# microcosmAI/MuJoCo-RL-Environment-Wrapper

Measured on NVIDIA B200. Metric: agent-steps/sec, higher is better.
Workload: dtype f32

## Files before the change

include/mjb.h:

```cpp
#ifndef MJB_H_
#define MJB_H_

#include <stdint.h>

#include "mjb_blob.h"

#ifdef __cplusplus
extern "C" {
#endif

#define MJB_OK 0
#define MJB_ERR_PARSE -1
#define MJB_ERR_ARG -2
#define MJB_ERR_CUDA -3
#define MJB_ERR_LIMIT -4

typedef struct mjb_model mjb_model;
typedef struct mjb_batch mjb_batch;

typedef struct mjb_dims {
  int32_t nq, nv, nu, nbody, njnt, ngeom, nsite, nsensor, nsensordata, npair;
  int32_t integrator;
  int32_t ncam;
  double timestep;
} mjb_dims;

int mjb_model_create(const char* mjcf_text, mjb_model** out);
void mjb_model_destroy(mjb_model* m);
int mjb_model_dims(const mjb_model* m, mjb_dims* out);
const void* mjb_model_blob(const mjb_model* m, int64_t* nbytes);
int mjb_name2id(const mjb_model* m, int objtype, const char* name);
const char* mjb_id2name(const mjb_model* m, int objtype, int id);
const char* mjb_last_error(void);
const char* mjb_version(void);
typedef struct mjb_param_offsets {
  int32_t body_mass, body_inertia, geom_friction, actuator_gear, dof_damping;
  int32_t n_params;
} mjb_param_offsets;
int mjb_param_layout(const mjb_model* m, mjb_param_offsets* out);
int mjb_model_set_field(mjb_model* m, const char* name, const double* values, int32_t count);

enum {
  MJB_DYN_LANGUAGE = 1,
  MJB_DYN_PICKUP = 2
};
enum {
  MJB_REW_TAG_DISTANCE = 1,
  MJB_REW_ANT = 2
};
enum { MJB_DONE_DISTANCE_LE = 1  };

#define MJB_MAX_AGENTS 8
#define MJB_MAX_PLUGINS 4
#define MJB_MAX_TARGETS 16
#define MJB_MAX_EXTRA_PROBES 48

typedef struct mjb_plugin {
  int32_t kind;
  int32_t act_lo;
  int32_t act_hi;
  int32_t n_obs;
  float param[4];
} mjb_plugin;

typedef struct mjb_env_spec {
  int32_t n_agents;
  int32_t free_joint;
  int32_t skip_frames;
  int32_t max_steps;
  int32_t n_phys_act;
  int32_t act_dim;
  int32_t obs_dim[MJB_MAX_AGENTS];
  int32_t agent_body[MJB_MAX_AGENTS];
  const int32_t* act_index;
  const int32_t* obs_index;
  int32_t obs_adr[MJB_MAX_AGENTS + 1];
  int32_t n_dynamics, n_rewards, n_dones;
  mjb_plugin dynamics[MJB_MAX_PLUGINS];
  mjb_plugin rewards[MJB_MAX_PLUGINS];
  mjb_plugin dones[MJB_MAX_PLUGINS];
  int32_t n_targets;
  int32_t target_objtype[MJB_MAX_TARGETS];
  int32_t target_objid[MJB_MAX_TARGETS];
  uint64_t seed;
  int32_t solver_iterations;
  int32_t ls_iterations;
  int32_t flags;
  float reset_noise;
  int32_t n_extra_probes;
  int32_t extra_objtype[MJB_MAX_EXTRA_PROBES];
  int32_t extra_objid[MJB_MAX_EXTRA_PROBES];
  float act_low[64], act_high[64];
  float* final_obs;
  const float* start_qpos;
  const float* start_qvel;
  int32_t n_start;
  float* params;
  float param_lo[4], param_hi[4];
} mjb_env_spec;

enum {
  MJB_SPEC_NO_PACK = 1,
  MJB_SPEC_AUTORESET = 2,
  MJB_SPEC_RANDOMIZE = 4
};


typedef struct mjb_layout {
  int32_t num_envs;
  int32_t qpos_stride, qvel_stride, ctrl_stride, sensor_stride;
  int32_t act_stride;
  int32_t obs_stride;
  int32_t probe_count;
  int32_t maxcon;
  int32_t store_i32, store_f32;
} mjb_layout;

typedef struct mjb_buffers {
  float* qpos;
  float* qvel;
  float* ctrl;
  float* warmstart;
  float* sensordata;
  float* probe;
  float* actions;
  float* obs;
  float* reward;
  uint8_t* term;
  uint8_t* trunc;
  int32_t* timestep;
  int32_t* store_i;
  float* store_f;
  int32_t* ncon;
  int32_t* contact_geom;
  float* contact_dist;
  int32_t* niter;
  int32_t* nreset;
  float* probe_quat;
  int32_t* ncon_dropped;
} mjb_buffers;

enum { MJB_STORE_I_UTTERANCE = 0, MJB_STORE_I_HAS_UTTERANCE = 1, MJB_STORE_I_TARGET = 2, MJB_STORE_I_INVENTORY = 3,
       MJB_STORE_I_HAS_XPOS = 4, MJB_STORE_I_DRAWS = 5, MJB_STORE_I_COUNT = 8 };
enum { MJB_STORE_F_DISTANCE = 0, MJB_STORE_F_XPOS_BEFORE = 1, MJB_STORE_F_DISTANCE64 = 2, MJB_STORE_F_COUNT = 4 };

int mjb_batch_layout(const mjb_model* m, const mjb_env_spec* spec, int32_t num_envs, mjb_layout* out);
int mjb_batch_create(const mjb_model* m, const mjb_env_spec* spec, int32_t num_envs, int32_t device, void* stream,
                     const mjb_buffers* buffers, mjb_batch** out);
void mjb_batch_destroy(mjb_batch* b);
int mjb_reset(mjb_batch* b, const uint8_t* mask_dev);
int mjb_reset_rows(mjb_batch* b, const uint8_t* mask_dev);
int mjb_step(mjb_batch* b);
int mjb_physics(mjb_batch* b, int32_t skip_frames);
int mjb_forward(mjb_batch* b);
int mjb_sync(mjb_batch* b);
int mjb_step_host(mjb_batch* b, const float* actions, float* obs, float* reward, uint8_t* term, uint8_t* trunc);
int64_t mjb_launch_count(const mjb_batch* b);
int mjb_set_timing(mjb_batch* b, int32_t enable);
int mjb_kernel_time_ms(mjb_batch* b, double* total_ms, int64_t* launches);
int mjb_set_env_subset(mjb_batch* b, const int32_t* env_ids_dev, int32_t count);
int mjb_render(mjb_batch* b, const int32_t* cam_ids, int32_t ncams, int32_t width, int32_t height, uint8_t* rgb_dev);
int mjb_batch_geometry(const mjb_batch* b, int32_t* grid, int32_t* warps_per_cta, int64_t* smem_bytes);
int mjb_phase_cycles(uint64_t* out, int32_t n);
uint32_t mjb_draw_u32(uint64_t seed, uint32_t env, uint32_t agent, uint32_t counter);
float mjb_reset_action(uint64_t seed, uint32_t env, uint32_t agent, uint32_t dim, uint32_t ep, float low, float high);
uint32_t mjb_start_index(uint64_t seed, uint32_t env, uint32_t ep, int32_t n_start);
float mjb_param_scale(uint64_t seed, uint32_t env, int32_t family, uint32_t index, uint32_t ep, float lo, float hi);

#ifdef __cplusplus
}
#endif
#endif
```

include/mjb_blob.h:

```cpp
#ifndef MJB_BLOB_H_
#define MJB_BLOB_H_

#include <stdint.h>
#include <string.h>

#ifdef __cplusplus
extern "C" {
#endif

#define MJB_BLOB_MAGIC "MJBLOB1"
#define MJB_FIELD_NAME_LEN 32

enum { MJB_DTYPE_I32 = 0, MJB_DTYPE_F64 = 1 };

typedef struct mjb_blob_header {
  char magic[8];
  int32_t nfields;
  int32_t reserved;
  int64_t total_bytes;
} mjb_blob_header;

typedef struct mjb_blob_field {
  char name[MJB_FIELD_NAME_LEN];
  int32_t dtype;
  int32_t count;
  int64_t offset;
} mjb_blob_field;

enum { MJB_GEOM_PLANE = 0, MJB_GEOM_SPHERE = 2, MJB_GEOM_CAPSULE = 3, MJB_GEOM_BOX = 6 };
enum { MJB_JNT_FREE = 0, MJB_JNT_SLIDE = 2, MJB_JNT_HINGE = 3 };
enum { MJB_SENS_TOUCH = 0, MJB_SENS_ACCELEROMETER = 1, MJB_SENS_VELOCIMETER = 2, MJB_SENS_GYRO = 3,
       MJB_SENS_RANGEFINDER = 7, MJB_SENS_JOINTPOS = 9, MJB_SENS_JOINTVEL = 10, MJB_SENS_FRAMEPOS = 26,
       MJB_SENS_FRAMEQUAT = 27, MJB_SENS_FRAMEXAXIS = 28, MJB_SENS_FRAMEYAXIS = 29, MJB_SENS_FRAMEZAXIS = 30,
       MJB_SENS_FRAMELINVEL = 31, MJB_SENS_FRAMEANGVEL = 32 };
enum { MJB_DATA_REAL = 0, MJB_DATA_POSITIVE = 1, MJB_DATA_AXIS = 2, MJB_DATA_QUATERNION = 3 };
enum { MJB_OBJ_BODY = 1, MJB_OBJ_XBODY = 2, MJB_OBJ_JOINT = 3, MJB_OBJ_GEOM = 5, MJB_OBJ_SITE = 6, MJB_OBJ_CAMERA = 7,
       MJB_OBJ_ACTUATOR = 19, MJB_OBJ_SENSOR = 20 };
enum { MJB_INT_EULER = 0, MJB_INT_RK4 = 1 };

static inline const mjb_blob_field* mjb_blob_find(const void* blob, const char* name) {
  const mjb_blob_header* h = (const mjb_blob_header*)blob;
  const mjb_blob_field* f = (const mjb_blob_field*)((const char*)blob + sizeof(mjb_blob_header));
  for (int i = 0; i < h->nfields; i++)
    if (strncmp(f[i].name, name, MJB_FIELD_NAME_LEN) == 0) return &f[i];
  return 0;
}
static inline const int32_t* mjb_blob_i32(const void* blob, const char* name, int* count) {
  const mjb_blob_field* f = mjb_blob_find(blob, name);
  if (!f || f->dtype != MJB_DTYPE_I32) { if (count) *count = -1; return 0; }
  if (count) *count = f->count;
  return (const int32_t*)((const char*)blob + f->offset);
}
static inline const double* mjb_blob_f64(const void* blob, const char* name, int* count) {
  const mjb_blob_field* f = mjb_blob_find(blob, name);
  if (!f || f->dtype != MJB_DTYPE_F64) { if (count) *count = -1; return 0; }
  if (count) *count = f->count;
  return (const double*)((const char*)blob + f->offset);
}

#ifdef __cplusplus
}
#endif
#endif
```

mujoco_rl_environment_wrapper_b200/_lib.py:

```python
import ctypes
import os
import struct

import numpy as np

_HERE = os.path.dirname(os.path.abspath(__file__))
LIB_PATH = os.environ.get("MJB_LIB") or os.path.join(_HERE, "libmjb.so")

MAX_AGENTS, MAX_PLUGINS, MAX_TARGETS, MAX_EXTRA_PROBES = 8, 4, 16, 48
SPEC_NO_PACK, SPEC_AUTORESET, SPEC_RANDOMIZE = 1, 2, 4
PARAM_FIELDS = ("body_mass", "body_inertia", "geom_friction", "actuator_gear", "dof_damping")
PARAM_FAMILIES = ("body_mass", "geom_friction", "actuator_gear", "dof_damping")
OBJ_BODY, OBJ_XBODY, OBJ_JOINT, OBJ_GEOM, OBJ_SITE, OBJ_CAMERA, OBJ_ACTUATOR, OBJ_SENSOR = 1, 2, 3, 5, 6, 7, 19, 20
SENSOR_TYPE = {"touch": 0, "accelerometer": 1, "velocimeter": 2, "gyro": 3, "rangefinder": 7, "jointpos": 9, "jointvel": 10,
               "framepos": 26, "framequat": 27, "framexaxis": 28, "frameyaxis": 29, "framezaxis": 30, "framelinvel": 31,
               "frameangvel": 32}
DATA_REAL, DATA_POSITIVE, DATA_AXIS, DATA_QUATERNION = 0, 1, 2, 3
DYN_LANGUAGE, DYN_PICKUP = 1, 2
REW_TAG_DISTANCE, REW_ANT = 1, 2
DONE_DISTANCE_LE = 1
STORE_I = {"utterance": 0, "has_utterance": 1, "current_target": 2, "inventory": 3, "has_xpos": 4, "draws": 5}
STORE_I_COUNT = 8
STORE_F = {"distance": 0, "xpos_before": 1}
STORE_F_COUNT = 4
JNT_FREE, JNT_SLIDE, JNT_HINGE = 0, 2, 3


class Dims(ctypes.Structure):
    _fields_ = [(n, ctypes.c_int32) for n in
                ("nq", "nv", "nu", "nbody", "njnt", "ngeom", "nsite", "nsensor", "nsensordata", "npair",
                 "integrator", "ncam")] + [("timestep", ctypes.c_double)]


class Plugin(ctypes.Structure):
    _fields_ = [("kind", ctypes.c_int32), ("act_lo", ctypes.c_int32), ("act_hi", ctypes.c_int32),
                ("n_obs", ctypes.c_int32), ("param", ctypes.c_float * 4)]


class EnvSpec(ctypes.Structure):
    _fields_ = [
        ("n_agents", ctypes.c_int32), ("free_joint", ctypes.c_int32), ("skip_frames", ctypes.c_int32),
        ("max_steps", ctypes.c_int32), ("n_phys_act", ctypes.c_int32), ("act_dim", ctypes.c_int32),
        ("obs_dim", ctypes.c_int32 * MAX_AGENTS), ("agent_body", ctypes.c_int32 * MAX_AGENTS),
        ("act_index", ctypes.POINTER(ctypes.c_int32)), ("obs_index", ctypes.POINTER(ctypes.c_int32)),
        ("obs_adr", ctypes.c_int32 * (MAX_AGENTS + 1)),
        ("n_dynamics", ctypes.c_int32), ("n_rewards", ctypes.c_int32), ("n_dones", ctypes.c_int32),
        ("dynamics", Plugin * MAX_PLUGINS), ("rewards", Plugin * MAX_PLUGINS), ("dones", Plugin * MAX_PLUGINS),
        ("n_targets", ctypes.c_int32),
        ("target_objtype", ctypes.c_int32 * MAX_TARGETS), ("target_objid", ctypes.c_int32 * MAX_TARGETS),
        ("seed", ctypes.c_uint64),
        ("solver_iterations", ctypes.c_int32), ("ls_iterations", ctypes.c_int32), ("flags", ctypes.c_int32), ("reset_noise", ctypes.c_float),
        ("n_extra_probes", ctypes.c_int32), ("extra_objtype", ctypes.c_int32 * MAX_EXTRA_PROBES), ("extra_objid", ctypes.c_int32 * MAX_EXTRA_PROBES),
        ("act_low", ctypes.c_float * 64), ("act_high", ctypes.c_float * 64), ("final_obs", ctypes.c_void_p),
        ("start_qpos", ctypes.c_void_p), ("start_qvel", ctypes.c_void_p), ("n_start", ctypes.c_int32),
        ("params", ctypes.c_void_p), ("param_lo", ctypes.c_float * 4), ("param_hi", ctypes.c_float * 4),
    ]


class ParamOffsets(ctypes.Structure):
    _fields_ = [(n, ctypes.c_int32) for n in PARAM_FIELDS + ("n_params",)]


class Layout(ctypes.Structure):
    _fields_ = [(n, ctypes.c_int32) for n in
                ("num_envs", "qpos_stride", "qvel_stride", "ctrl_stride", "sensor_stride", "act_stride",
                 "obs_stride", "probe_count", "maxcon", "store_i32", "store_f32")]


class Buffers(ctypes.Structure):
    _fields_ = [(n, ctypes.c_void_p) for n in
                ("qpos", "qvel", "ctrl", "warmstart", "sensordata", "probe", "actions", "obs", "reward", "term",
                 "trunc", "timestep", "store_i", "store_f", "ncon", "contact_geom", "contact_dist", "niter", "nreset", "probe_quat", "ncon_dropped")]


_LIB = None


def load(build_if_missing=True):
    global _LIB
    if _LIB is not None:
        return _LIB
    if build_if_missing and not os.environ.get("MJB_LIB"):
        from . import build as _build
        try:
            if _build.needs_build():
                _build.build()
        except Exception:
            if not os.path.exists(LIB_PATH):
                raise
    if not os.path.exists(LIB_PATH):
        raise RuntimeError(f"{LIB_PATH} is missing: run `python -m mujoco_rl_environment_wrapper_b200.build` "
                           "(there is no CPU fallback for the step path)")
    lib = ctypes.CDLL(LIB_PATH)
    vp, i32, i64 = ctypes.c_void_p, ctypes.c_int32, ctypes.c_int64
    lib.mjb_last_error.restype = ctypes.c_char_p
    lib.mjb_version.restype = ctypes.c_char_p
    lib.mjb_model_create.argtypes = [ctypes.c_char_p, ctypes.POINTER(vp)]
    lib.mjb_model_destroy.argtypes = [vp]
    lib.mjb_model_destroy.restype = None
    lib.mjb_model_dims.argtypes = [vp, ctypes.POINTER(Dims)]
    lib.mjb_model_blob.restype = vp
    lib.mjb_model_blob.argtypes = [vp, ctypes.POINTER(i64)]
    lib.mjb_name2id.argtypes = [vp, ctypes.c_int, ctypes.c_char_p]
    lib.mjb_id2name.restype = ctypes.c_char_p
    lib.mjb_id2name.argtypes = [vp, ctypes.c_int, ctypes.c_int]
    lib.mjb_batch_layout.argtypes = [vp, ctypes.POINTER(EnvSpec), i32, ctypes.POINTER(Layout)]
    lib.mjb_batch_create.argtypes = [vp, ctypes.POINTER(EnvSpec), i32, i32, vp, ctypes.POINTER(Buffers),
                                     ctypes.POINTER(vp)]
    lib.mjb_batch_destroy.argtypes = [vp]
    lib.mjb_batch_destroy.restype = None
    lib.mjb_reset.argtypes = [vp, vp]
    lib.mjb_reset_rows.argtypes = [vp, vp]
    lib.mjb_step.argtypes = [vp]
    lib.mjb_physics.argtypes = [vp, i32]
    lib.mjb_forward.argtypes = [vp]
    lib.mjb_sync.argtypes = [vp]
    lib.mjb_step_host.argtypes = [vp, vp, vp, vp, vp, vp]
    lib.mjb_launch_count.restype = i64
    lib.mjb_launch_count.argtypes = [vp]
    lib.mjb_set_timing.argtypes = [vp, i32]
    lib.mjb_kernel_time_ms.argtypes = [vp, ctypes.POINTER(ctypes.c_double), ctypes.POINTER(i64)]
    lib.mjb_set_env_subset.argtypes = [vp, vp, ctypes.c_int32]
    lib.mjb_render.argtypes = [vp, ctypes.POINTER(ctypes.c_int32), ctypes.c_int32, ctypes.c_int32, ctypes.c_int32, vp]
    lib.mjb_batch_geometry.argtypes = [vp, ctypes.POINTER(i32), ctypes.POINTER(i32), ctypes.POINTER(i64)]
    lib.mjb_phase_cycles.argtypes = [ctypes.POINTER(ctypes.c_uint64), i32]
    lib.mjb_draw_u32.restype = ctypes.c_uint32
    lib.mjb_draw_u32.argtypes = [ctypes.c_uint64, ctypes.c_uint32, ctypes.c_uint32, ctypes.c_uint32]
    lib.mjb_reset_action.restype = ctypes.c_float
    lib.mjb_reset_action.argtypes = [ctypes.c_uint64, ctypes.c_uint32, ctypes.c_uint32, ctypes.c_uint32, ctypes.c_uint32,
                                     ctypes.c_float, ctypes.c_float]
    lib.mjb_start_index.restype = ctypes.c_uint32
    lib.mjb_start_index.argtypes = [ctypes.c_uint64, ctypes.c_uint32, ctypes.c_uint32, ctypes.c_int32]
    lib.mjb_param_layout.argtypes = [vp, ctypes.POINTER(ParamOffsets)]
    lib.mjb_model_set_field.argtypes = [vp, ctypes.c_char_p, ctypes.POINTER(ctypes.c_double), i32]
    lib.mjb_param_scale.restype = ctypes.c_float
    lib.mjb_param_scale.argtypes = [ctypes.c_uint64, ctypes.c_uint32, ctypes.c_int32, ctypes.c_uint32, ctypes.c_uint32,
                                    ctypes.c_float, ctypes.c_float]
    _LIB = lib
    return lib


def check(rc, what=""):
    if rc != 0:
        msg = load().mjb_last_error().decode(errors="replace")
        raise Exception(f"{what}: {msg}" if what else msg)


def parse_blob(raw: bytes):
    magic, nf, _, _tot = struct.unpack_from("8siiq", raw, 0)
    if not magic.startswith(b"MJBLOB1"):
        raise ValueError("bad model blob")
    out = {}
    for i in range(nf):
        name, dt, cnt, off = struct.unpack_from("32siiq", raw, 24 + i * 48)
        name = name.split(b"\0")[0].decode()
        out[name] = np.frombuffer(raw, dtype=np.int32 if dt == 0 else np.float64, count=cnt, offset=off).copy()
    return out


class Model:

    def __init__(self, xml_text: str):
        self._lib = load()
        h = ctypes.c_void_p()
        check(self._lib.mjb_model_create(xml_text.encode(), ctypes.byref(h)), "MJCF compile")
        self._h = h
        d = Dims()
        check(self._lib.mjb_model_dims(h, ctypes.byref(d)))
        self.dims = d
        self._read_blob()
        for k in ("nq", "nv", "nu", "nbody", "njnt", "ngeom", "nsite", "nsensor", "nsensordata", "npair", "ncam"):
            setattr(self, k, getattr(d, k))
        self.timestep = d.timestep

    def _read_blob(self):
        n = ctypes.c_int64()
        p = self._lib.mjb_model_blob(self._h, ctypes.byref(n))
        self.blob = bytes((ctypes.c_char * n.value).from_address(p))
        self.fields = parse_blob(self.blob)

    def set_field(self, name, values):
        v = np.ascontiguousarray(np.asarray(values, dtype=np.float64).reshape(-1))
        check(self._lib.mjb_model_set_field(self._h, name.encode(), v.ctypes.data_as(ctypes.POINTER(ctypes.c_double)), v.size),
              "set_field")
        self._read_blob()

    def param_layout(self):
        out = ParamOffsets()
        check(self._lib.mjb_param_layout(self._h, ctypes.byref(out)), "param layout")
        return out

    def nominal_params(self):
        lay, f = self.param_layout(), self.fields
        row = np.zeros(lay.n_params, np.float32)
        vals = {"body_mass": f["body_mass"], "body_inertia": f["body_inertia"], "geom_friction": f["geom_friction"][0::3],
                "actuator_gear": f["actuator_gear"], "dof_damping": f["dof_damping"]}
        for k, v in vals.items():
            o = getattr(lay, k)
            row[o:o + v.size] = v
        return row

    @classmethod
    def from_xml_path(cls, path):
        with open(path, "r") as f:
            return cls(f.read())

    def __del__(self):
        try:
            if getattr(self, "_h", None):
                self._lib.mjb_model_destroy(self._h)
                self._h = None
        except Exception:
            pass

    def name2id(self, objtype, name):
        return self._lib.mjb_name2id(self._h, objtype, name.encode())

    def id2name(self, objtype, idx):
        r = self._lib.mjb_id2name(self._h, objtype, idx)
        return None if r is None else r.decode()
```

mujoco_rl_environment_wrapper_b200/batch.py:

```python
import ctypes

import numpy as np
import torch

from . import _lib as L


class Batch:
    def __init__(self, model: "L.Model", spec: "L.EnvSpec", num_envs: int, device=None, keepalive=(), share=None, probe_quat=False,
                 start_states=None, params=False, param_ranges=None):
        self._lib = L.load()
        if not torch.cuda.is_available():
            raise RuntimeError("mujoco_rl_environment_wrapper_b200: no CUDA device — the step path is CUDA-only "
                               "(sm_100a); there is no CPU fallback")
        self.model, self.spec, self.num_envs = model, spec, int(num_envs)
        self._keep = keepalive
        self.device = torch.device("cuda", torch.cuda.current_device()) if device is None else torch.device(device)
        lay = L.Layout()
        L.check(self._lib.mjb_batch_layout(model._h, ctypes.byref(spec), self.num_envs, ctypes.byref(lay)), "batch layout")
        self.layout = lay
        if share is not None:
            same = all(getattr(lay, f) == getattr(share.layout, f) for f, _ in L.Layout._fields_)
            if not same or share.num_envs != self.num_envs or share.device != self.device:
                raise Exception("level variants must share one buffer layout (same sizes, sensors, agents and plugins)")
# ... 60 lines not shown
            if getattr(self, "_h", None):
                self._lib.mjb_batch_destroy(self._h)
                self._h = None
        except Exception:
            pass

    def __getattr__(self, k):
        buf = self.__dict__.get("buf")
        if buf is not None and k in buf:
            return buf[k]
        raise AttributeError(k)

    def _mask_ptr(self, mask):
        if mask is None:
            return None
        self._mask = mask.to(device=self.device, dtype=torch.uint8).contiguous()
        return ctypes.c_void_p(self._mask.data_ptr())

    def reset(self, mask=None):
        L.check(self._lib.mjb_reset(self._h, self._mask_ptr(mask)), "reset")

    def reset_rows(self, mask=None):
        L.check(self._lib.mjb_reset_rows(self._h, self._mask_ptr(mask)), "reset_rows")

    def step(self):
        L.check(self._lib.mjb_step(self._h), "step")

    def set_subset(self, env_ids=None):
        if env_ids is None:
            self._subset = None
            L.check(self._lib.mjb_set_env_subset(self._h, None, 0), "env subset")
            return
        ids = env_ids.to(device=self.device, dtype=torch.int32).contiguous()
        count = int(ids.numel())
        if count == 0:
            ids = torch.zeros(1, dtype=torch.int32, device=self.device)
        self._subset = ids
        L.check(self._lib.mjb_set_env_subset(self._h, ctypes.c_void_p(self._subset.data_ptr()), count), "env subset")

    def render(self, cam_ids, width=64, height=64, out=None):
        n = len(cam_ids)
        if out is None:
            out = torch.empty((self.num_envs, n, height, width, 3), dtype=torch.uint8, device=self.device)
        ids = (ctypes.c_int32 * n)(*cam_ids)
        L.check(self._lib.mjb_render(self._h, ids, n, int(width), int(height), ctypes.c_void_p(out.data_ptr())), "render")
        return out

    def physics(self, skip_frames=1):
        L.check(self._lib.mjb_physics(self._h, skip_frames), "physics")

    def forward(self):
        L.check(self._lib.mjb_forward(self._h), "forward")

    def sync(self):
        L.check(self._lib.mjb_sync(self._h), "sync")

    def step_host(self, actions: np.ndarray, obs: np.ndarray, reward: np.ndarray, term: np.ndarray, trunc: np.ndarray):
        L.check(self._lib.mjb_step_host(self._h, actions.ctypes.data, obs.ctypes.data, reward.ctypes.data,
                                        term.ctypes.data, trunc.ctypes.data), "step_host")

    def host_arrays(self, pinned=True):
        lay, A, N = self.layout, self.spec.n_agents, self.num_envs
        z = lambda shape, dt: torch.zeros(shape, dtype=dt, pin_memory=pinned)
        f32, u8 = torch.float32, torch.uint8
        self._host_keep = [z((N, A, lay.act_stride), f32), z((N, A, lay.obs_stride), f32), z((N, A), f32),
                           z((N, A + 1), u8), z((N, A + 1), u8)]
        return tuple(t.numpy() for t in self._host_keep)

    @property
    def launch_count(self):
        return int(self._lib.mjb_launch_count(self._h))

    def set_timing(self, enable=True):
        L.check(self._lib.mjb_set_timing(self._h, 1 if enable else 0))

    def kernel_time_ms(self):
        t, n = ctypes.c_double(), ctypes.c_int64()
        L.check(self._lib.mjb_kernel_time_ms(self._h, ctypes.byref(t), ctypes.byref(n)))
        return t.value, n.value

    def geometry(self):
        g, w, s = ctypes.c_int32(), ctypes.c_int32(), ctypes.c_int64()
        self._lib.mjb_batch_geometry(self._h, ctypes.byref(g), ctypes.byref(w), ctypes.byref(s))
        return {"grid": g.value, "warps_per_cta": w.value, "smem_bytes": s.value}
```

mujoco_rl_environment_wrapper_b200/build.py:

```python
import os
import subprocess
import sys

_HERE = os.path.dirname(os.path.abspath(__file__))
CSRC = os.path.join(_HERE, "csrc")
LIB_PATH = os.path.join(_HERE, "libmjb.so")
SOURCES = ["mjcf_compile.cpp", "mjb_model.cpp", "mjb_batch.cu"]
NVCC_FLAGS = [
    "-gencode", "arch=compute_100a,code=sm_100a", "-lineinfo", "-O3", "-std=c++17",
    "--use_fast_math",
    "-Xcompiler", "-fPIC", "-Xcompiler", "-Wall", "-shared",
]


def _nvcc():
    for cand in (os.environ.get("NVCC"), "/usr/local/cuda/bin/nvcc", "nvcc"):
        if cand and (os.path.isabs(cand) and os.path.exists(cand) or not os.path.isabs(cand)):
            return cand
    raise RuntimeError("nvcc not found")


def _deps():
    out = []
    for root in (CSRC, os.path.join(_HERE, "..", "include")):
        for f in os.listdir(root):
            if f.endswith((".h", ".cuh", ".cu", ".cpp")):
                out.append(os.path.join(root, f))
    return out


def needs_build():
    if not os.path.exists(LIB_PATH):
        return True
    t = os.path.getmtime(LIB_PATH)
    return any(os.path.getmtime(f) > t for f in _deps())


def build(force=False, verbose=False):
    if not force and not needs_build():
        return LIB_PATH
    cmd = [_nvcc()] + NVCC_FLAGS + os.environ.get("MJB_NVCC_FLAGS", "").split() + (["-Xptxas", "-v"] if verbose else []) + ["-o", LIB_PATH] + \
          [os.path.join(CSRC, s) for s in SOURCES]
    res = subprocess.run(cmd, capture_output=True, text=True)
    if verbose or res.returncode != 0:
        sys.stderr.write(res.stdout + res.stderr)
    if res.returncode != 0:
        raise RuntimeError("nvcc failed building libmjb.so")
    return LIB_PATH


if __name__ == "__main__":
    build(force="--force" in sys.argv, verbose="-v" in sys.argv)
    print(LIB_PATH)
```

mujoco_rl_environment_wrapper_b200/csrc/dev_model.h:

```cpp
#pragma once
#include <stdint.h>

#ifndef MJB_HD
#if defined(__CUDACC__)
#define MJB_HD __host__ __device__ __forceinline__
#else
#define MJB_HD inline
#endif
#endif

namespace mjb {

#define MJB_IMAGE_FIELDS(X)                                                                         \
  X(level_adr)       \
  X(mb_parent)       \
  X(mb_root)         \
  X(mb_jntadr)       \
  X(mb_jntnum)       \
  X(mb_dofadr)       \
  X(mb_dofnum)       \
  X(mb_childadr)     \
  X(mb_child)        \
  X(mb_dofmask)      \
  X(mb_pos)          \
  X(mb_quat)         \
  X(mb_ipos)         \
  X(mb_iquat)        \
  X(mb_mass)         \
  X(mb_inertia)      \
  X(mb_invweight)    \
  X(jnt_type)        \
  X(jnt_qposadr)     \
  X(jnt_dofadr)      \
  X(jnt_pos)         \
  X(jnt_axis)        \
  X(jnt_qpos0)       \
  X(lim_dof)         \
  X(lim_qposadr)     \
  X(lim_param)       \
  X(dof_mb)          \
  X(dof_parent)      \
  X(dof_kind)        \
  X(dof_t0)          \
  X(dof_t1)          \
  X(dof_lim)         \
  X(dof_armature)    \
  X(dof_damping)     \
  X(geom_type)       \
  X(geom_mb)         \
  X(geom_slot)       \
  X(geom_size)       \
  X(geom_rbound)     \
  X(geom_pos)        \
  X(geom_mat)        \
  X(geom_quat)       \
  X(geom_ray)        \
  X(pair_pack)       \
  X(pclass)          \
  X(bp_block)        \
  X(bp_passmask)     \
  X(site_mb)         \
  X(site_type)       \
  X(site_pos)        \
  X(site_quat)       \
  X(site_size)       \
  X(sensor_type)     \
  X(sensor_site)     \
  X(sensor_adr)      \
  X(sensor_dim)      \
  X(sensor_dtype)    \
  X(sensor_cutoff)   \
  X(act_dof)         \
  X(act_param)       \
  X(dof_actadr)      \
  X(dof_actnum)      \
  X(act_list)        \
  X(probe_kind)      \
  X(probe_id)        \
  X(probe_const)     \
  X(act_index)       \
  X(obs_index)       \
  X(tri_lut)         \
  X(qpos0)

enum ImageField {
#define X(n) IF_##n,
  MJB_IMAGE_FIELDS(X)
#undef X
      IF_COUNT
};

#define MJB_SMEM_FIELDS(X)                                                                          \
  X(qpos) X(qvel) X(qacc) X(ctrl) X(qfrc)  \
  X(xpos) X(xquat) X(xmat) X(xipos)        \
  X(cdof) X(cinert) X(crb) X(cvel) X(cacc)  \
  X(gpos) X(gmat) X(spos) X(smat)          \
  X(M) X(H)                                \
  X(cand)                                  \
  X(con)                                   \
  X(J)                                     \
  X(efcD) X(efcAref) X(efcJar) X(efcJv)    \
  X(vecA) X(vecB) X(vecC) X(vecD)          \
  X(rk)                                    \
  X(sens)

enum SmemField {
#define X(n) SF_##n,
  MJB_SMEM_FIELDS(X)
#undef X
      SF_COUNT
};

struct DevPlugin {
  int kind, act_lo, act_hi, n_obs;
  float param[4];
};

struct DevModel {
  int nq, nv, nu, nmb, njnt, nlim, ngeom, ngdyn, nsite, nsensor, nsensordata, npair, nclass, nlevel, nprobe;
  int maxcon, maxcand, maxefc, ldj, maxtree, nblock;
  int pack, a1, t1, nq1, nv1, nu1, ns1, np1, ngeom1, maxcon1;
  int integrator, has_damping, need_acc_sensors;
  float timestep, gravity[3];
  double timestep_d;
  int solver_iterations, ls_iterations;
  float solver_tol;
  float reset_noise;
  int njnt1;
  int n_agents, free_joint, skip_frames, max_steps, n_phys_act, act_dim;
  int obs_dim[8], obs_adr[9], agent_probe[8];
  int n_dynamics, n_rewards, n_dones, n_targets;
  DevPlugin dynamics[4], rewards[4], dones[4];
  int target_probe[16];
  unsigned long long seed;
  int off[IF_COUNT];
  int image_words;
  int soff[SF_COUNT];
  int env_words;
  int qpos_stride, qvel_stride, ctrl_stride, sensor_stride, act_stride, obs_stride, store_i32, store_f32;
  float* final_obs;
  int autoreset;
  float dyn_act_low[4], dyn_act_high[4];
  const float* start_qpos;
  const float* start_qvel;
  int n_start;
  int start_pad[3];
  float* params;
  int n_params, prm_n;
  int randomize, prm_soff, off_prm_map, off_prm_nominal;
  float prm_lo[4], prm_hi[4];
  int ext_sensors, off_sens_obj, ext_pad[2];
};
enum { SO_MB = 0, SO_POS = 1, SO_QUAT = 4, SO_STRIDE = 8 };
enum { KSENS_OBJ_AXIS = 64 };
MJB_HD int prm_inertia(const DevModel& dm) { return dm.nmb; }
MJB_HD int prm_damping(const DevModel& dm) { return 4 * dm.nmb; }
MJB_HD int prm_gear(const DevModel& dm) { return 4 * dm.nmb + dm.nv; }
MJB_HD int prm_friction(const DevModel& dm) { return 4 * dm.nmb + dm.nv + dm.nu; }

enum { CAM_MB = 0, CAM_MODE = 1, CAM_POS = 2, CAM_QUAT = 5, CAM_TANHALF = 9, CAM_STRIDE = 12 };
struct RenderHdr {
  int ncam, ngeom;
  int off_cam, off_rgba;
  int words;
};
enum { GL_POS = 0, GL_MAT = 3, GL_SIZE = 12, GL_TYPE = 15, GL_RBOUND = 16, GL_RGB = 17, GL_STRIDE = 20 };

enum { CON_DIST = 0, CON_POS = 1, CON_FRAME = 4, CON_PAIR = 13, CON_MU = 14, CON_MASK = 15, CON_DOFS = 16, CON_STRIDE = 20 };
enum { LIM_LO = 0, LIM_HI, LIM_MARGIN, LIM_K, LIM_B, LIM_INVW, LIM_SOLIMP, LIM_STRIDE = 12 };
enum { PC_MARGIN = 0, PC_INCMARGIN, PC_MU, PC_K, PC_B, PC_SOLIMP, PC_CONDIM = 10, PC_STRIDE = 12 };
enum { DOF_AXIS = 0, DOF_FREE_TRANS = 1, DOF_FREE_ROT = 2 };
enum { PROBE_BODY = 0, PROBE_GEOM = 1, PROBE_CONST = 2 };
enum { BP_ROOT_A = 0, BP_PARTNER = 1, BP_REACH = 2, BP_MARGIN = 3, BP_STRIDE = 4, BP_ALWAYS = 0x7fffffff };

}
```

mujoco_rl_environment_wrapper_b200/csrc/env_kernel.cuh:

```cuda
#pragma once
#include "step_kernel.cuh"
#if defined(MJB_HOST_EMU)
#define MJB_IMG_WAIT(c) ((void)0)
#else
#include "tma_prims.cuh"
#define MJB_IMG_WAIT(c) do { if ((c).img_bar) mbar_wait((c).img_bar, 0); } while (0)
#endif

namespace mjb {

enum { MODE_STEP = 0, MODE_PHYSICS = 1, MODE_FORWARD = 2, MODE_RESET = 3, MODE_RESET_ROWS = 4 };

#if defined(MJB_HOST_EMU)
#define MJB_AGENT_LOOP
#else
#define MJB_AGENT_LOOP _Pragma("unroll (AMAX <= 2 ? 2 : 1)")
#endif

MJB_HD uint32_t draw_u32(unsigned long long seed, uint32_t env, uint32_t agent, uint32_t counter) {
  unsigned long long z = seed + 0x9E3779B97F4A7C15ull * (1ull + env) + 0xBF58476D1CE4E5B9ull * agent +
                         0x94D049BB133111EBull * counter;
  z = (z ^ (z >> 30)) * 0xBF58476D1CE4E5B9ull;
  z = (z ^ (z >> 27)) * 0x94D049BB133111EBull;
  z ^= z >> 31;
  return (uint32_t)(z >> 32);
}

MJB_HD float reset_action(unsigned long long seed, uint32_t env, uint32_t agent, uint32_t dim, uint32_t ep, float low, float high) {
  const float u = (float)(draw_u32(seed ^ 0x5eedc0deULL, env, 0xC000u + agent * 64u + dim, ep) >> 8) * (1.f / 16777216.f);
#if defined(__CUDA_ARCH__)
  return __fadd_rn(low, __fmul_rn(u, high - low));
#else
  volatile float span = u * (high - low);
  return low + span;
#endif
}

MJB_HD uint32_t start_index(unsigned long long seed, uint32_t env, uint32_t ep, int n_start) {
  return n_start < 1 ? 0u : (uint32_t)(((unsigned long long)draw_u32(seed ^ 0x5eedc0deULL, env, 0xD000u, ep) * (uint32_t)n_start) >> 32);
}

MJB_HD float param_scale(unsigned long long seed, uint32_t env, uint32_t family, uint32_t index, uint32_t ep, float lo, float hi) {
  const float u = (float)(draw_u32(seed ^ 0x5eedc0deULL, env, 0x10000u + 0x1000u * family + index, ep) >> 8) * (1.f / 16777216.f);
#if defined(__CUDA_ARCH__)
  return __fadd_rn(lo, __fmul_rn(u, hi - lo));
#else
  volatile float span = u * (hi - lo);
  return lo + span;
#endif
}

MJB_DEV double probe_dist(const float* probe, int a, int b) {
  const double dx = (double)probe[4 * a] - (double)probe[4 * b], dy = (double)probe[4 * a + 1] - (double)probe[4 * b + 1],
               dz = (double)probe[4 * a + 2] - (double)probe[4 * b + 2];
#if defined(MJB_HOST_EMU)
  volatile double xx = dx * dx, yy = dy * dy, zz = dz * dz;
  return sqrt((xx + yy) + zz);
#else
  return sqrt(__dadd_rn(__dadd_rn(__dmul_rn(dx, dx), __dmul_rn(dy, dy)), __dmul_rn(dz, dz)));
#endif
}
MJB_DEV double ld_dist(const float* sfa) {
  union { double d; float f[2]; } u;
  u.f[0] = sfa[MJB_STORE_F_DISTANCE64]; u.f[1] = sfa[MJB_STORE_F_DISTANCE64 + 1];
  return u.d;
}
MJB_DEV void st_dist(float* sfa, double d) {
  union { double d; float f[2]; } u;
  u.d = d;
  sfa[MJB_STORE_F_DISTANCE64] = u.f[0]; sfa[MJB_STORE_F_DISTANCE64 + 1] = u.f[1];
  sfa[MJB_STORE_F_DISTANCE] = (float)d;
}

template <int AMAX>
MJB_DEV bool run_plugins(const DevModel& dm, const float* ctrl, float* obs, float* rew, uint8_t* term, uint8_t* trunc, int env, int copy,
                         bool is_reset, const float* probe, int* si, float* sf, const float* act, int* ts_io, const double* dtab = nullptr,
                         bool keep_flags = false) {
  const int A = dm.a1, ab = copy * dm.a1, tb = copy * dm.t1, n_targets = dm.t1;
  auto pdist = [&](int a, int t) { return dtab ? dtab[a * n_targets + t] : probe_dist(probe, dm.agent_probe[ab + a], dm.target_probe[tb + t]); };
  double reward[AMAX];
  bool done[AMAX];
  int opos[AMAX];
  if (is_reset)
    MJB_AGENT_LOOP
    for (int a = 0; a < AMAX; a++) if (a < A) {
      MJB_NOUNROLL
      for (int k = 0; k < dm.store_i32; k++) if (k != MJB_STORE_I_DRAWS) si[a * dm.store_i32 + k] = 0;
      MJB_NOUNROLL
      for (int k = 0; k < dm.store_f32; k++) sf[a * dm.store_f32 + k] = 0.f;
    }
  MJB_AGENT_LOOP
  for (int a = 0; a < AMAX; a++) if (a < A) { reward[a] = 0.0; done[a] = false; opos[a] = dm.obs_adr[ab + a + 1] - dm.obs_adr[ab + a]; }
  MJB_NOUNROLL
  for (int p = 0; p < dm.n_dynamics; p++) {
    const DevPlugin& dyn = dm.dynamics[p];
    MJB_AGENT_LOOP
    for (int a = 0; a < AMAX; a++) if (a < A) {
      int* sia = si + a * dm.store_i32;
      float* sfa = sf + a * dm.store_f32;
      float* oa = obs + a * dm.obs_stride;
      if (dyn.kind == MJB_DYN_LANGUAGE) {
        int utt = (int)act[a * dm.act_stride + dyn.act_lo];
        sia[MJB_STORE_I_UTTERANCE] = utt; sia[MJB_STORE_I_HAS_UTTERANCE] = 1;
        int other = a == 0 ? 1 : 0;
        float val = 0.f;
        if (other < A && si[other * dm.store_i32 + MJB_STORE_I_HAS_UTTERANCE]) val = (float)si[other * dm.store_i32 + MJB_STORE_I_UTTERANCE];
        oa[opos[a]++] = val;
      } else if (dyn.kind == MJB_DYN_PICKUP) {
        int tgt = sia[MJB_STORE_I_TARGET];
        if (tgt == 0 && n_targets > 0) {
          tgt = 1 + (int)(draw_u32(dm.seed, env, a, sia[MJB_STORE_I_DRAWS]++) % (uint32_t)n_targets);
          sia[MJB_STORE_I_TARGET] = tgt;
        }
        if (tgt > 0) {
          const double d = pdist(a, tgt - 1);
          if (d < (double)dyn.param[0]) {
            sia[MJB_STORE_I_INVENTORY] ^= 1;
            reward[a] += 1.0;
            tgt = 1 + (int)(draw_u32(dm.seed, env, a, sia[MJB_STORE_I_DRAWS]++) % (uint32_t)n_targets);
            sia[MJB_STORE_I_TARGET] = tgt;
            st_dist(sfa, pdist(a, tgt - 1));
          }
          const float* tp = probe + 4 * dm.target_probe[tb + tgt - 1];
          oa[opos[a]] = tp[0]; oa[opos[a] + 1] = tp[1]; oa[opos[a] + 2] = tp[2];
        } else {
          oa[opos[a]] = 0.f; oa[opos[a] + 1] = 0.f; oa[opos[a] + 2] = 0.f;
        }
        oa[opos[a] + 3] = (float)sia[MJB_STORE_I_INVENTORY];
        opos[a] += 4;
      }
    }
  }
  if (is_reset) {
    MJB_AGENT_LOOP
    for (int a = 0; a < AMAX; a++) if (a < A) {
      MJB_NOUNROLL
      for (int k = 0; k < dm.store_i32; k++) if (k != MJB_STORE_I_DRAWS) si[a * dm.store_i32 + k] = 0;
      MJB_NOUNROLL
      for (int k = 0; k < dm.store_f32; k++) sf[a * dm.store_f32 + k] = 0.f;
      if (!keep_flags) { rew[a] = 0.f; term[a] = 0; trunc[a] = 0; }
    }
    if (!keep_flags) { term[A] = 0; trunc[A] = 0; }
    *ts_io = 0;
    return false;
  }
  MJB_NOUNROLL
  for (int p = 0; p < dm.n_rewards; p++) {
    const DevPlugin& rf = dm.rewards[p];
    MJB_AGENT_LOOP
    for (int a = 0; a < AMAX; a++) if (a < A) {
      int* sia = si + a * dm.store_i32;
      float* sfa = sf + a * dm.store_f32;
      if (rf.kind == MJB_REW_TAG_DISTANCE) {
        int tgt = sia[MJB_STORE_I_TARGET];
        if (n_targets <= 0) continue;
        if (tgt == 0) {
          tgt = 1 + (int)(draw_u32(dm.seed, env, a, sia[MJB_STORE_I_DRAWS]++) % (uint32_t)n_targets);
          sia[MJB_STORE_I_TARGET] = tgt;
          st_dist(sfa, pdist(a, tgt - 1));
        } else {
          const double d = pdist(a, tgt - 1);
          reward[a] += (ld_dist(sfa) - d) * (double)rf.param[0];
          st_dist(sfa, d);
        }
      } else if (rf.kind == MJB_REW_ANT) {
        float x_after = probe[4 * dm.agent_probe[ab + a]];
        if (!sia[MJB_STORE_I_HAS_XPOS]) {
          sia[MJB_STORE_I_HAS_XPOS] = 1;
        } else {
          double cc = 0.0;
          MJB_NOUNROLL
          for (int u = 0; u < dm.nu1; u++) cc += (double)ctrl[u] * (double)ctrl[u];
          reward[a] += ((double)x_after - (double)sfa[MJB_STORE_F_XPOS_BEFORE]) / dm.timestep_d - 0.5 * cc;
        }
        sfa[MJB_STORE_F_XPOS_BEFORE] = x_after;
      }
    }
  }
  int ts = *ts_io;
  uint8_t tr = ts >= dm.max_steps ? 1 : 0;
  MJB_NOUNROLL
  for (int a = 0; a <= A; a++) trunc[a] = tr;
  bool all = false;
  MJB_NOUNROLL
  for (int p = 0; p < dm.n_dones && !all; p++) {
    const DevPlugin& df = dm.dones[p];
    MJB_AGENT_LOOP
    for (int a = 0; a < AMAX; a++) if (a < A)
      if (df.kind == MJB_DONE_DISTANCE_LE) done[a] = done[a] || (ld_dist(sf + a * dm.store_f32) <= (double)df.param[0]);
    MJB_AGENT_LOOP
    for (int a = 0; a < AMAX; a++) if (a < A) all = all || done[a];
  }
  MJB_AGENT_LOOP
  for (int a = 0; a < AMAX; a++) if (a < A) { rew[a] = (float)reward[a]; term[a] = done[a] ? 1 : 0; }
  term[A] = all ? 1 : 0;
  *ts_io = ts + 1;
  return all || tr;
}

MJB_DEV void split_copy(int i, int n1, int K, int& k, int& j) {
  if (K == 1) { k = 0; j = i; }
  else { k = i / n1; j = i - k * n1; }
}

template <bool PHYS, bool PACKED, bool EXT = true, bool PRM = false>
MJB_DEV void run_env(const Ctx& c_in, const mjb_buffers& B, int venv, int num_envs, int mode_in, int skip_frames,
                     const uint8_t* reset_mask) {
  uint32_t fin = 0;
pass:
  const bool auto_pass = fin != 0;
  const bool own_rows = EXT && mode_in == MODE_RESET_ROWS;
  const int mode = (auto_pass || own_rows) ? (int)MODE_RESET : mode_in;
  Ctx c = c_in;
  float* probe = c.probe;
  const DevModel& dm = *c.dm;
  const int lane = c.lane, K = PACKED ? dm.pack : 1, e0 = venv * K;
  c.probe_quat = (!PACKED && B.probe_quat) ? B.probe_quat + (size_t)e0 * dm.np1 * 4 : nullptr;
  uint32_t live = 0, upd = 0;
  for (int k = 0; k < K; k++)
    if (e0 + k < num_envs) {
      live |= 1u << k;
      if (!(mode == MODE_RESET && reset_mask && !reset_mask[e0 + k])) upd |= 1u << k;
    }
  if (auto_pass) {
    upd = fin;
    c.cta_threads = 0;
  }
  if (!upd) return;
  if (mode == MODE_RESET || live != (K >= 32 ? 0xffffffffu : (1u << K) - 1u)) MJB_IMG_WAIT(c);
  float *qpos = SF(qpos), *qvel = SF(qvel), *qacc = SF(qacc), *ctrl = SF(ctrl), *sens = SF(sens);
  auto fresh = [&](int k) { return mode == MODE_RESET && ((upd >> k) & 1u); };
  auto has = [&](int k) { return ((live >> k) & 1u) != 0; };
  auto reset_key = [&](uint32_t env) {
    return (uint32_t)B.timestep[env] ^ MJB_F2U(B.qpos[(size_t)env * dm.qpos_stride]) ^ (MJB_F2U(B.qvel[(size_t)env * dm.qvel_stride]) << 13);
  };
  const bool pool = EXT && mode == MODE_RESET && !own_rows && dm.n_start > 0, from_start = own_rows || pool;
  uint32_t pr[MJB_MAX_PACK] = {0, 0, 0, 0};
  if (pool) {
#pragma unroll
    for (int k = 0; k < MJB_MAX_PACK; k++)
      if (k < K && fresh(k)) pr[k] = start_index(dm.seed, (uint32_t)(e0 + k), reset_key((uint32_t)(e0 + k)), dm.n_start);
  }
  auto pool_row = [&](const float* base, int n1, int k) {
    return base + (size_t)(K == 1 || k == 0 ? pr[0] : k == 1 ? pr[1] : k == 2 ? pr[2] : pr[3]) * n1;
  };
  MJB_NOUNROLL
  for (int i = lane; i < dm.nq; i += 32) {
    int k, j;
    split_copy(i, dm.nq1, K, k, j);
    if (from_start && fresh(k)) MJB_G2S(&qpos[i], pool ? pool_row(dm.start_qpos, dm.nq1, k) + j : &B.qpos[(size_t)(e0 + k) * dm.qpos_stride + j]);
    else if (fresh(k) || !has(k)) qpos[i] = CF(qpos0)[i];
    else MJB_G2S(&qpos[i], &B.qpos[(size_t)(e0 + k) * dm.qpos_stride + j]);
  }
  MJB_NOUNROLL
  for (int i = lane; i < dm.nv; i += 32) {
    int k, j;
    split_copy(i, dm.nv1, K, k, j);
    bool z = fresh(k) || !has(k);
    if (from_start && fresh(k)) {
      MJB_G2S(&qvel[i], pool ? pool_row(dm.start_qvel, dm.nv1, k) + j : &B.qvel[(size_t)(e0 + k) * dm.qvel_stride + j]);
      qacc[i] = 0.f;
    } else if (z) { qvel[i] = 0.f; qacc[i] = 0.f; }
    else {
      MJB_G2S(&qvel[i], &B.qvel[(size_t)(e0 + k) * dm.qvel_stride + j]);
      MJB_G2S(&qacc[i], &B.warmstart[(size_t)(e0 + k) * dm.qvel_stride + j]);
    }
  }
  MJB_NOUNROLL
  for (int i = lane; i < dm.nu; i += 32) {
    int k, j;
    split_copy(i, dm.nu1, K, k, j);
    if (fresh(k) || !has(k)) ctrl[i] = 0.f;
    else MJB_G2S(&ctrl[i], &B.ctrl[(size_t)(e0 + k) * dm.ctrl_stride + j]);
  }
  MJB_NOUNROLL
  for (int i = lane; i < dm.nsensordata; i += 32) {
    int k, j;
    split_copy(i, dm.ns1, K, k, j);
    if (fresh(k) || !has(k)) sens[i] = 0.f;
    else MJB_G2S(&sens[i], &B.sensordata[(size_t)(e0 + k) * dm.sensor_stride + j]);
  }
  auto probe_slot = [&](int p, int& k, int& p1) {
    if (K == 1) { k = 0; p1 = p; }
    else if (p < K * dm.a1) { k = p / dm.a1; p1 = p - k * dm.a1; }
    else { int q = p - K * dm.a1; k = q / dm.t1; p1 = dm.a1 + (q - k * dm.t1); }
  };
  MJB_NOUNROLL
  for (int i = lane; i < 4 * dm.nprobe; i += 32) {
    int k, p1;
    probe_slot(i >> 2, k, p1);
    if (has(k)) MJB_G2S(&probe[i], &B.probe[((size_t)(e0 + k) * dm.np1 + p1) * 4 + (i & 3)]);
    else probe[i] = 0.f;
  }
  const bool epi = (mode == MODE_STEP || mode == MODE_RESET);
  int pre_si[2] = {0, 0}, pre_ts = 0;
  float pre_sf = 0.f, pre_act[2] = {0.f, 0.f};
  if (epi && K == 1) {
    const int* gsi = B.store_i + (size_t)e0 * dm.a1 * dm.store_i32;
// ... 200 lines not shown
    for (int i = lane; i < n; i += 32) {
      int e = CI(obs_index)[dm.obs_adr[av] + i], kind = e >> 24, adr = e & 0xffffff;
      oa[i] = kind == 0 ? sens[adr] : (kind == 1 ? qpos[adr] : qvel[adr]);
    }
  }
  MJB_PH(c, PH_EPI_OBS);
  int* s_si = (int*)SF(J);
  float* s_sf = SF(J) + MJB_MAX_AGENTS * MJB_STORE_I_COUNT;
  float* s_act = s_sf + MJB_MAX_AGENTS * MJB_STORE_F_COUNT;
  int* s_ts = (int*)(s_act + 64);
  double* s_dtab = (double*)(s_ts + 4);
  MJB_NOUNROLL
  for (int k = 0; k < K; k++) {
    if (!writes(k)) continue;
    const int env = e0 + k, A1 = dm.a1;
    int* gsi = B.store_i + (size_t)env * A1 * dm.store_i32;
    float* gsf = B.store_f + (size_t)env * A1 * dm.store_f32;
    const float* gact = B.actions + (size_t)env * A1 * dm.act_stride;
    MJB_SYNC();
    if (K == 1) {
      for (int r = 0; r < 2; r++) {
        int i = lane + 32 * r;
        if (i < A1 * dm.store_i32) s_si[i] = pre_si[r];
        if (i < A1 * dm.act_stride) s_act[i] = pre_act[r];
      }
      if (lane < A1 * dm.store_f32) s_sf[lane] = pre_sf;
      if (lane == 0) *s_ts = pre_ts;
    } else {
      for (int i = lane; i < A1 * dm.store_i32; i += 32) s_si[i] = gsi[i];
      for (int i = lane; i < A1 * dm.act_stride; i += 32) s_act[i] = gact[i];
      if (lane < A1 * dm.store_f32) s_sf[lane] = gsf[lane];
      if (lane == 0) *s_ts = B.timestep[env];
    }
    MJB_NOUNROLL
    for (int i = lane; i < A1 * dm.t1; i += 32) {
      const int a = i / dm.t1, t = i - a * dm.t1;
      s_dtab[i] = probe_dist(probe, dm.agent_probe[k * A1 + a], dm.target_probe[k * dm.t1 + t]);
    }
    MJB_SYNC();
    MJB_PH(c, PH_EPI_STAGE);
    const uint32_t ep = auto_pass ? MJB_SHFL(ep_k, k) : 0u;
    bool last_step = false;
    if (lane == 0) {
      if (auto_pass) {
        MJB_NOUNROLL
        for (int a = 0; a < A1; a++) {
          MJB_NOUNROLL
          for (int p = 0; p < dm.n_dynamics; p++) {
            const DevPlugin& dyn = dm.dynamics[p];
            if (dyn.act_hi > dyn.act_lo)
              s_act[a * dm.act_stride + dyn.act_lo] = reset_action(dm.seed, (uint32_t)env, (uint32_t)a, (uint32_t)dyn.act_lo, ep,
                                                                   dm.dyn_act_low[p], dm.dyn_act_high[p]);
          }
        }
      }
      if (MJB_LIKELY(A1 <= 2))
        last_step = run_plugins<2>(dm, SF(ctrl) + k * dm.nu1, B.obs + (size_t)env * A1 * dm.obs_stride, B.reward + (size_t)env * A1, B.term + (size_t)env * (A1 + 1),
                                   B.trunc + (size_t)env * (A1 + 1), env, k, mode == MODE_RESET, probe, s_si, s_sf, s_act, s_ts, s_dtab, auto_pass);
      else
        last_step = run_plugins<MJB_MAX_AGENTS>(dm, SF(ctrl) + k * dm.nu1, B.obs + (size_t)env * A1 * dm.obs_stride, B.reward + (size_t)env * A1,
                                                B.term + (size_t)env * (A1 + 1), B.trunc + (size_t)env * (A1 + 1), env, k, mode == MODE_RESET, probe, s_si,
                                                s_sf, s_act, s_ts, s_dtab, auto_pass);
    }
    MJB_SYNC();
    MJB_PH(c, PH_EPI_PLUG);
    for (int i = lane; i < A1 * dm.store_i32; i += 32) gsi[i] = s_si[i];
    if (lane < A1 * dm.store_f32) gsf[lane] = s_sf[lane];
    if (lane == 0) B.timestep[env] = *s_ts;
    if (EXT && PHYS && mode == MODE_STEP && dm.autoreset && MJB_SHFL((int)last_step, 0)) {
      ended |= 1u << k;
      const size_t o = (size_t)env * A1 * dm.obs_stride;
      MJB_NOUNROLL
      for (int i = lane; i < A1 * dm.obs_stride; i += 32) dm.final_obs[o + i] = B.obs[o + i];
    }
  }
  MJB_PH(c, PH_EPILOGUE);
  if (MJB_UNLIKELY(ended)) {
    MJB_SYNC();
    fin = ended;
    goto pass;
  }
}

}
```

mujoco_rl_environment_wrapper_b200/csrc/mjb_batch.cu:

```cuda
#include <cuda_runtime.h>

#include <cmath>
#include <cstdio>
#include <cstring>
#include <map>
#include <mutex>
#include <string>
#include <vector>

#include "../../include/mjb.h"
#include "dev_model_build.h"
#include "env_kernel.cuh"
#include "render_kernel.cuh"
#include "tma_prims.cuh"
#include "lite_kernel.cuh"
#include "mjb_internal.h"

#ifndef MJB_MAX_THREADS
#define MJB_MAX_THREADS 512
#endif

namespace mjb {

template <bool PHYS, bool PACKED, bool EXT = false, bool PRM = false>
__global__ void __launch_bounds__(PHYS ? MJB_MAX_THREADS : 512, PHYS ? 1 : 4) k_env(const __grid_constant__ DevModel dm, const uint32_t* __restrict__ image, const mjb_buffers B,
                      int num_envs, int mode, int skip_frames, const uint8_t* __restrict__ mask,
                      const int* __restrict__ env_ids, int active, int env_base) {
  extern __shared__ __align__(128) uint32_t smem[];
  uint64_t* bar = reinterpret_cast<uint64_t*>(smem);
  uint32_t* img = smem + 4;
  const int warps = blockDim.x >> 5, warp = threadIdx.x >> 5, lane = threadIdx.x & 31;
  if (threadIdx.x == 0) {
    mbar_init(bar, 1);
    mbar_fence_init();
  }
  __syncthreads();
  if (threadIdx.x == 0) {
    uint32_t bytes = (uint32_t)dm.image_words * 4u;
    mbar_expect_tx(bar, bytes);
    bulk_g2s(img, image, bytes, bar);
  }
  float* scratch = reinterpret_cast<float*>(img + dm.image_words) + (size_t)warp * (dm.env_words + 4 * ((dm.nprobe + 3) & ~3));
  float* probe = scratch + dm.env_words;
  Ctx c{&dm, img, scratch, lane, probe, 0};
#if defined(MJB_PHASE_PROF)
  long long t_last = clock64();
  c.t_last = &t_last;
#endif
  const int stride = gridDim.x * warps;
  const int pack = PACKED ? dm.pack : 1;
  const int nvirt = (active + pack - 1) / pack;
  const int rounds = (nvirt - blockIdx.x * warps + stride - 1) / stride;
  int env = blockIdx.x * warps + warp;
  for (int r = 0; r < rounds; r++) {
    if (PHYS) {
      int busy = nvirt - (blockIdx.x * warps + r * stride);
      c.cta_threads = (mask == nullptr ? 32 : 0) * (busy > warps ? warps : (busy < 0 ? 0 : busy));
    }
    c.img_bar = r == 0 ? bar : nullptr;
    if (env < nvirt) run_env<PHYS, PACKED, EXT, PRM>(c, B, env_ids ? env_ids[env] : env + env_base, num_envs, mode, skip_frames, mask);
    if (r == 0) mbar_wait(bar, 0);
    if (!PHYS) __syncthreads();
    MJB_PH(c, PH_BARRIER);
    env += stride;
  }
}

}

struct mjb_batch {
  mjb::PackedModel packed;
  mjb::DevImage img;
  mjb::DevImage lite;
  bool has_lite = false;
  int lite_warps = 0, lite_grid = 0;
  size_t lite_smem = 0;
  mjb::LiteLayout tile{};
  int tile_grid = 0;
  size_t tile_smem = 0;
  int* d_lite_tab = nullptr;
  mjb::DevModel* d_lite_dm = nullptr;
  mjb_buffers B;
  int num_envs = 0, device = 0, warps = 0, grid = 0;
  size_t smem_bytes = 0;
  cudaStream_t stream = nullptr;
  cudaStream_t stream2 = nullptr;
  cudaEvent_t ev_fork = nullptr, ev_join = nullptr;
  uint32_t* d_image = nullptr;
  mjb::DevImage rimg;
  uint32_t *d_rimage = nullptr, *d_rtab = nullptr;
  const int* subset = nullptr;
  int subset_count = -1;
  int64_t launches = 0;
  bool timing = false;
  std::vector<std::pair<cudaEvent_t, cudaEvent_t>> events;
  float *h_act = nullptr, *h_obs = nullptr, *h_rew = nullptr;
  uint8_t *h_term = nullptr, *h_trunc = nullptr;
  const void* pin_cache[5] = {nullptr, nullptr, nullptr, nullptr, nullptr};
};

namespace {
#define CUDA_TRY(expr)                                                                      \
  do {                                                                                      \
    cudaError_t e_ = (expr);                                                                \
    if (e_ != cudaSuccess) {                                                                \
      mjb::set_error(std::string(#expr) + ": " + cudaGetErrorString(e_));                   \
      return MJB_ERR_CUDA;                                                                  \
    }                                                                                       \
  } while (0)

int launch(mjb_batch* b, int mode, int skip_frames, const uint8_t* mask, cudaStream_t stream = nullptr, int base = 0, int count = -1,
           const mjb_buffers* out_buffers = nullptr) {
  if (b->subset && b->subset_count == 0) return MJB_OK;
  if (!stream) stream = b->stream;
  const int active = b->subset ? b->subset_count : (count >= 0 ? count : b->num_envs);
  const mjb_buffers& B = out_buffers ? *out_buffers : b->B;
  cudaEvent_t e0 = nullptr, e1 = nullptr;
  if (b->timing) {
    CUDA_TRY(cudaEventCreate(&e0));
    CUDA_TRY(cudaEventCreate(&e1));
    CUDA_TRY(cudaEventRecord(e0, stream));
  }
  if (mode == mjb::MODE_STEP && b->has_lite && !b->subset) {
    const int ntiles = (active + b->tile.tile - 1) / b->tile.tile;
    const mjb::LiteLayout& T = b->tile;
    mjb::LiteIssue I{};
    int k = 0;
    auto row = [&](const void* basep, int words, int off_words) {
      if (words <= 0) return;
      I.c[k].base = (const char*)basep; I.c[k].row_bytes = 4u * words; I.c[k].fixed = 0; I.c[k].dst_off = 4u * off_words; k++;
      I.sum_row_bytes += 4u * words;
    };
    auto fixed = [&](const void* basep, int bytes, int off_words) {
      I.c[k].base = (const char*)basep; I.c[k].row_bytes = 0; I.c[k].fixed = bytes; I.c[k].dst_off = 4u * off_words; k++;
      I.first_bytes += bytes;
    };
    row(B.qpos, T.qs, T.o_qpos); row(B.qvel, T.vs, T.o_qvel); row(B.actions, T.as, T.o_act);
    row(B.store_i, T.sis, T.o_si); row(B.store_f, T.sfs, T.o_sf);
    if (T.use_ctrl) row(B.ctrl, T.cs, T.o_ctrl);
    if (T.use_sens) row(B.sensordata, T.ss, T.o_sens);
    if (T.use_probe) row(B.probe, T.ps, T.o_probe);
    fixed(b->d_lite_tab, 4 * T.table_words, T.o_gather);
    fixed(b->d_lite_dm, T.dm_bytes, T.o_dm);
    I.ncopy = k; I.tile = T.tile; I.active = active; I.env_base = base; I.profile = T.profile;
    mjb::k_lite<<<std::min(ntiles, b->tile_grid), LITE_THREADS, b->tile_smem, stream>>>(I, B, T);
  } else if (mode == mjb::MODE_STEP && b->has_lite) {
    mjb::k_env<false, false><<<b->lite_grid, b->lite_warps * 32, b->lite_smem, stream>>>(b->lite.dm, b->d_image, B, b->num_envs, mode,
                                                                                   skip_frames, mask, b->subset, active, base);
  } else {
    const bool ext = b->img.dm.autoreset || mode == mjb::MODE_RESET_ROWS || (mode == mjb::MODE_RESET && b->img.dm.n_start > 0);
    auto kern = b->img.dm.prm_n > 0 ? (b->img.dm.pack > 1 ? mjb::k_env<true, true, true, true> : mjb::k_env<true, false, true, true>)
              : ext ? (b->img.dm.pack > 1 ? mjb::k_env<true, true, true> : mjb::k_env<true, false, true>)
                    : (b->img.dm.pack > 1 ? mjb::k_env<true, true> : mjb::k_env<true, false>);
    const int pack = b->img.dm.pack;
    const int need = ((active + pack - 1) / pack + b->warps - 1) / b->warps;
    kern<<<std::min(b->grid, std::max(1, need)), b->warps * 32, b->smem_bytes, stream>>>(
        b->img.dm, b->d_image, B, b->num_envs, mode, skip_frames, mask, b->subset, active, base / pack);
  }
  CUDA_TRY(cudaGetLastError());
  if (b->timing) {
    CUDA_TRY(cudaEventRecord(e1, stream));
    b->events.emplace_back(e0, e1);
  }
  b->launches++;
  return MJB_OK;
}
}

extern "C" {

uint32_t mjb_draw_u32(uint64_t seed, uint32_t env, uint32_t agent, uint32_t counter) {
  return mjb::draw_u32(seed, env, agent, counter);
}

float mjb_reset_action(uint64_t seed, uint32_t env, uint32_t agent, uint32_t dim, uint32_t ep, float low, float high) {
  return mjb::reset_action(seed, env, agent, dim, ep, low, high);
}

uint32_t mjb_start_index(uint64_t seed, uint32_t env, uint32_t ep, int32_t n_start) {
  return mjb::start_index(seed, env, ep, n_start);
}

float mjb_param_scale(uint64_t seed, uint32_t env, int32_t family, uint32_t index, uint32_t ep, float lo, float hi) {
  return mjb::param_scale(seed, env, (uint32_t)family, index, ep, lo, hi);
}

int mjb_batch_layout(const mjb_model* m, const mjb_env_spec* spec, int32_t num_envs, mjb_layout* out) {
  if (!m || !spec || !out || num_envs < 1) { mjb::set_error("mjb_batch_layout: bad argument"); return MJB_ERR_ARG; }
  if (const char* e = mjb::param_spec_error(*spec)) { mjb::set_error(std::string("mjb_batch_layout: ") + e); return MJB_ERR_ARG; }
  try {
    mjb::ModelView mv(m->host.blob.data());
    mjb::DevImage img;
    mjb::build_dev_model(mv, *spec, img);
    mjb::fill_layout(img.dm, num_envs, *out);
    return MJB_OK;
  } catch (const std::exception& e) {
    mjb::set_error(e.what());
    return MJB_ERR_LIMIT;
  }
}

int mjb_batch_create(const mjb_model* m, const mjb_env_spec* spec, int32_t num_envs, int32_t device, void* stream,
                     const mjb_buffers* buffers, mjb_batch** out) {
  if (!m || !spec || !buffers || !out || num_envs < 1) { mjb::set_error("mjb_batch_create: bad argument"); return MJB_ERR_ARG; }
  *out = nullptr;
  if (spec->flags & MJB_SPEC_AUTORESET) {
    if (spec->skip_frames == 0) {
      mjb::set_error("mjb_batch_create: MJB_SPEC_AUTORESET needs skip_frames >= 1 (the physics-free step has no forward pass to reset with)");
      return MJB_ERR_ARG;
    }
    if (!spec->final_obs) { mjb::set_error("mjb_batch_create: MJB_SPEC_AUTORESET needs spec.final_obs"); return MJB_ERR_ARG; }
    for (int d = 0; d < spec->act_dim && d < 64; d++)
      if (!(spec->act_low[d] <= spec->act_high[d]) || !std::isfinite(spec->act_low[d]) || !std::isfinite(spec->act_high[d])) {
        mjb::set_error("mjb_batch_create: MJB_SPEC_AUTORESET needs finite act_low <= act_high");
        return MJB_ERR_ARG;
      }
  }
  if (spec->n_start < 0) { mjb::set_error("mjb_batch_create: spec.n_start < 0"); return MJB_ERR_ARG; }
  if (spec->n_start > 0 && (!spec->start_qpos || !spec->start_qvel)) {
    mjb::set_error("mjb_batch_create: spec.n_start > 0 needs spec.start_qpos and spec.start_qvel");
    return MJB_ERR_ARG;
  }
  if (const char* e = mjb::param_spec_error(*spec)) { mjb::set_error(std::string("mjb_batch_create: ") + e); return MJB_ERR_ARG; }
  int ndev = 0;
  if (cudaGetDeviceCount(&ndev) != cudaSuccess || ndev < 1) {
    mjb::set_error("mjb_batch_create: no CUDA device (the step path has no CPU fallback)");
    return MJB_ERR_CUDA;
  }
  mjb_batch* b = new mjb_batch();
  try {
    const int K = mjb::choose_pack(m->host, *spec, num_envs);
    mjb::make_packed(m->host, *spec, K, b->packed);
    mjb::ModelView mv(K > 1 ? b->packed.rep.blob.data() : m->host.blob.data());
    mjb::build_dev_model(mv, b->packed.vspec, b->img, false, K);
    mjb::ModelView mv1(m->host.blob.data());
    if (mv1.ncam > 0) mjb::build_dev_model(mv1, *spec, b->rimg, false, 1);
  } catch (const std::exception& e) {
    mjb::set_error(e.what());
    delete b;
    return MJB_ERR_LIMIT;
  }
  b->B = *buffers;
  b->num_envs = num_envs; b->device = device; b->stream = (cudaStream_t)stream;
  const mjb::DevModel& dm = b->img.dm;
  for (const void* p : {(const void*)b->B.qpos, (const void*)b->B.qvel, (const void*)b->B.ctrl, (const void*)b->B.warmstart,
                        (const void*)b->B.sensordata, (const void*)b->B.probe, (const void*)b->B.actions, (const void*)b->B.obs,
                        (const void*)b->B.reward, (const void*)b->B.term, (const void*)b->B.trunc, (const void*)b->B.timestep,
                        (const void*)b->B.store_i, (const void*)b->B.store_f})
    if (!p) { mjb::set_error("mjb_batch_create: a required buffer is NULL"); delete b; return MJB_ERR_ARG; }
  auto fail = [&](int rc) { mjb_batch_destroy(b); return rc; };
  if (cudaSetDevice(device) != cudaSuccess) { mjb::set_error("cudaSetDevice failed"); return fail(MJB_ERR_CUDA); }
  cudaDeviceProp prop;
  if (cudaGetDeviceProperties(&prop, device) != cudaSuccess) { mjb::set_error("cudaGetDeviceProperties failed"); return fail(MJB_ERR_CUDA); }
  size_t max_smem = prop.sharedMemPerBlockOptin;
  size_t fixed = 16 + (size_t)dm.image_words * 4;
  size_t per_env = ((size_t)dm.env_words + 4 * ((dm.nprobe + 3) & ~3)) * 4;
  size_t cta_budget = std::min(max_smem, prop.sharedMemPerMultiprocessor - 1024);
  int warps = cta_budget > fixed ? (int)((cta_budget - fixed) / per_env) : 0;
  int cap = std::min(MJB_MAX_THREADS / 32, mjb::env_int("MJB_WARPS", MJB_MAX_THREADS / 32));
  if (warps > cap) warps = cap;
  if (warps < 1) { mjb::set_error("model needs more shared memory per environment than one SM has"); return fail(MJB_ERR_LIMIT); }
  int sms = prop.multiProcessorCount;
  const int nvirt = (num_envs + dm.pack - 1) / dm.pack;
  int rounds = (nvirt + sms * warps - 1) / (sms * warps);
  int even = (nvirt + sms * rounds - 1) / (sms * rounds);
  if (even < warps) warps = even < 1 ? 1 : even;
  b->warps = warps;
  b->grid = (nvirt + warps - 1) / warps;
  if (b->grid > sms) b->grid = sms;
  b->smem_bytes = fixed + per_env * warps;
  static std::mutex smem_attr_mu;
  static std::map<int, size_t> smem_attr;
  std::lock_guard<std::mutex> smem_attr_lock(smem_attr_mu);
  if (b->smem_bytes > smem_attr[device] && (cudaFuncSetAttribute(mjb::k_env<true, false>, cudaFuncAttributeMaxDynamicSharedMemorySize, (int)b->smem_bytes) != cudaSuccess ||
      cudaFuncSetAttribute(mjb::k_env<true, true>, cudaFuncAttributeMaxDynamicSharedMemorySize, (int)b->smem_bytes) != cudaSuccess ||
      cudaFuncSetAttribute(mjb::k_env<true, false, true>, cudaFuncAttributeMaxDynamicSharedMemorySize, (int)b->smem_bytes) != cudaSuccess ||
      cudaFuncSetAttribute(mjb::k_env<true, true, true>, cudaFuncAttributeMaxDynamicSharedMemorySize, (int)b->smem_bytes) != cudaSuccess ||
      cudaFuncSetAttribute(mjb::k_env<true, false, true, true>, cudaFuncAttributeMaxDynamicSharedMemorySize, (int)b->smem_bytes) != cudaSuccess ||
      cudaFuncSetAttribute(mjb::k_env<true, true, true, true>, cudaFuncAttributeMaxDynamicSharedMemorySize, (int)b->smem_bytes) != cudaSuccess)) {
    mjb::set_error(std::string("cudaFuncSetAttribute(max dynamic smem) failed: ") + cudaGetErrorString(cudaGetLastError()));
    return fail(MJB_ERR_CUDA);
  }
  smem_attr[device] = std::max(smem_attr[device], b->smem_bytes);
  if (spec->skip_frames == 0) {
    try {
      mjb::ModelView mv(m->host.blob.data());
      mjb::build_dev_model(mv, *spec, b->lite, true);
    } catch (const std::exception& e) { mjb::set_error(e.what()); return fail(MJB_ERR_LIMIT); }
    size_t lite_env = ((size_t)b->lite.dm.env_words + 4 * ((b->lite.dm.nprobe + 3) & ~3)) * 4;
    b->lite_warps = 16;
    b->lite_smem = fixed + lite_env * b->lite_warps;
    int per_sm = 1;
    if (cudaFuncSetAttribute(mjb::k_env<false, false>, cudaFuncAttributeMaxDynamicSharedMemorySize, (int)b->lite_smem) != cudaSuccess ||
        cudaOccupancyMaxActiveBlocksPerMultiprocessor(&per_sm, mjb::k_env<false, false>, b->lite_warps * 32, b->lite_smem) != cudaSuccess || per_sm < 1) {
      mjb::set_error("lite step kernel configuration failed");
      return fail(MJB_ERR_CUDA);
    }
    b->lite_grid = std::min((num_envs + b->lite_warps - 1) / b->lite_warps, prop.multiProcessorCount * per_sm);
    b->has_lite = true;
    int tile = std::max(16, mjb::env_int("MJB_LITE_TILE", 64) / 16 * 16);
    for (;;) {
      b->tile = mjb::make_lite_layout(b->lite.dm, tile);
      b->tile.profile = mjb::env_int("MJB_LITE_PROFILE", 0);
      b->tile_smem = 16 + (size_t)b->tile.words * 4;
      if (b->tile_smem <= 48 * 1024 || tile <= 16) break;
      tile /= 2;
    }
    int tile_per_sm = 1;
    if (b->tile_smem > max_smem || cudaFuncSetAttribute(mjb::k_lite, cudaFuncAttributeMaxDynamicSharedMemorySize, (int)b->tile_smem) != cudaSuccess ||
        cudaOccupancyMaxActiveBlocksPerMultiprocessor(&tile_per_sm, mjb::k_lite, LITE_THREADS, b->tile_smem) != cudaSuccess || tile_per_sm < 1) {
      mjb::set_error("tile step kernel configuration failed (rows of one env too large for shared memory)");
      return fail(MJB_ERR_CUDA);
    }
    b->tile_grid = prop.multiProcessorCount * tile_per_sm;
    {
      std::vector<int> tab = mjb::lite_tables(b->lite.dm, b->tile, b->img.words.data());
      std::vector<char> hdr(b->tile.dm_bytes, 0);
      memcpy(hdr.data(), &b->lite.dm, sizeof(mjb::DevModel));
      if (cudaMalloc(&b->d_lite_tab, tab.size() * 4) != cudaSuccess ||
          cudaMemcpy(b->d_lite_tab, tab.data(), tab.size() * 4, cudaMemcpyHostToDevice) != cudaSuccess ||
          cudaMalloc(&b->d_lite_dm, hdr.size()) != cudaSuccess ||
          cudaMemcpy(b->d_lite_dm, hdr.data(), hdr.size(), cudaMemcpyHostToDevice) != cudaSuccess) {
        mjb::set_error("tile kernel table upload failed");
        return fail(MJB_ERR_CUDA);
      }
    }
  }
  if (cudaMalloc(&b->d_image, (size_t)dm.image_words * 4) != cudaSuccess ||
      cudaMemcpy(b->d_image, b->img.words.data(), (size_t)dm.image_words * 4, cudaMemcpyHostToDevice) != cudaSuccess) {
    mjb::set_error("device image upload failed");
    return fail(MJB_ERR_CUDA);
  }
  if (cudaStreamCreateWithFlags(&b->stream2, cudaStreamNonBlocking) != cudaSuccess ||
      cudaEventCreateWithFlags(&b->ev_fork, cudaEventDisableTiming) != cudaSuccess ||
      cudaEventCreateWithFlags(&b->ev_join, cudaEventDisableTiming) != cudaSuccess) {
    mjb::set_error("mjb_batch_create: stream / event creation failed");
    return fail(MJB_ERR_CUDA);
  }
  const int A = dm.a1;
  if (cudaMallocHost(&b->h_act, sizeof(float) * (size_t)num_envs * A * dm.act_stride + 16) != cudaSuccess ||
      cudaMallocHost(&b->h_obs, sizeof(float) * (size_t)num_envs * A * dm.obs_stride + 16) != cudaSuccess ||
      cudaMallocHost(&b->h_rew, sizeof(float) * (size_t)num_envs * A + 16) != cudaSuccess ||
      cudaMallocHost(&b->h_term, (size_t)num_envs * (A + 1) + 16) != cudaSuccess ||
      cudaMallocHost(&b->h_trunc, (size_t)num_envs * (A + 1) + 16) != cudaSuccess) {
    mjb::set_error("pinned staging allocation failed");
    return fail(MJB_ERR_CUDA);
  }
  *out = b;
  return MJB_OK;
}

void mjb_batch_destroy(mjb_batch* b) {
  if (!b) return;
  for (auto& ev : b->events) { cudaEventDestroy(ev.first); cudaEventDestroy(ev.second); }
  if (b->d_image) cudaFree(b->d_image);
  if (b->stream2) cudaStreamDestroy(b->stream2);
  for (cudaEvent_t e : {b->ev_fork, b->ev_join}) if (e) cudaEventDestroy(e);
  if (b->d_rimage) cudaFree(b->d_rimage);
  if (b->d_rtab) cudaFree(b->d_rtab);
  if (b->d_lite_tab) cudaFree(b->d_lite_tab);
  if (b->d_lite_dm) cudaFree(b->d_lite_dm);
  if (b->h_act) cudaFreeHost(b->h_act);
  if (b->h_obs) cudaFreeHost(b->h_obs);
  if (b->h_rew) cudaFreeHost(b->h_rew);
  if (b->h_term) cudaFreeHost(b->h_term);
  if (b->h_trunc) cudaFreeHost(b->h_trunc);
// ... 106 lines not shown
  if (!b || !total_ms || !launches) { mjb::set_error("mjb_kernel_time_ms: null argument"); return MJB_ERR_ARG; }
  CUDA_TRY(cudaStreamSynchronize(b->stream));
  double tot = 0;
  for (auto& ev : b->events) {
    float ms = 0;
    CUDA_TRY(cudaEventElapsedTime(&ms, ev.first, ev.second));
    tot += ms;
    cudaEventDestroy(ev.first); cudaEventDestroy(ev.second);
  }
  *total_ms = tot; *launches = (int64_t)b->events.size();
  b->events.clear();
  return MJB_OK;
}

int mjb_render(mjb_batch* b, const int32_t* cam_ids, int32_t ncams, int32_t width, int32_t height, uint8_t* rgb_dev) {
  if (!b || !cam_ids || !rgb_dev) { mjb::set_error("mjb_render: null argument"); return MJB_ERR_ARG; }
  const mjb::RenderHdr& rh = b->rimg.rhdr;
  if (rh.ncam == 0) { mjb::set_error("mjb_render: the model has no <camera>"); return MJB_ERR_ARG; }
  if (ncams < 1 || ncams > RENDER_MAX_CAMS || width < 1 || height < 1 || width > 4096 || height > 4096) {
    mjb::set_error("mjb_render: 1.." + std::to_string(RENDER_MAX_CAMS) + " cameras, 1..4096 pixels per side");
    return MJB_ERR_ARG;
  }
  mjb::RenderCams cams{};
  cams.n = ncams;
  for (int k = 0; k < ncams; k++) {
    if (cam_ids[k] < 0 || cam_ids[k] >= rh.ncam) { mjb::set_error("mjb_render: camera id out of range"); return MJB_ERR_ARG; }
    if (b->rimg.render[rh.off_cam + cam_ids[k] * mjb::CAM_STRIDE + mjb::CAM_MODE] != 0) {
      mjb::set_error("mjb_render: only mode=\"fixed\" cameras can be rendered");
      return MJB_ERR_ARG;
    }
    cams.id[k] = cam_ids[k];
  }
  CUDA_TRY(cudaSetDevice(b->device));
  const mjb::DevModel& dm = b->rimg.dm;
  const size_t smem = ((size_t)dm.image_words + dm.env_words + rh.words + (size_t)dm.ngeom * mjb::GL_STRIDE + 12 * RENDER_MAX_CAMS) * 4 +
                      (size_t)RENDER_TILE_BATCH * ((dm.ngeom + 2) & ~1) * 2;
  if (!b->d_rimage) {
    CUDA_TRY(cudaMalloc(&b->d_rimage, b->rimg.words.size() * 4));
    CUDA_TRY(cudaMalloc(&b->d_rtab, b->rimg.render.size() * 4));
    CUDA_TRY(cudaMemcpy(b->d_rimage, b->rimg.words.data(), b->rimg.words.size() * 4, cudaMemcpyHostToDevice));
    CUDA_TRY(cudaMemcpy(b->d_rtab, b->rimg.render.data(), b->rimg.render.size() * 4, cudaMemcpyHostToDevice));
    CUDA_TRY(cudaFuncSetAttribute(mjb::k_render, cudaFuncAttributeMaxDynamicSharedMemorySize, (int)smem));
  }
  int sms = 148;
  cudaDeviceGetAttribute(&sms, cudaDevAttrMultiProcessorCount, b->device);
  const int per_sm = (int)std::max<size_t>(1, std::min<size_t>(8, (200 * 1024) / (smem + 1024)));
  const int grid = std::min(b->num_envs, sms * per_sm);
  mjb::k_render<<<grid, 256, smem, b->stream>>>(dm, b->d_rimage, rh, b->d_rtab, b->B.qpos, b->num_envs, cams, width, height, rgb_dev);
  CUDA_TRY(cudaGetLastError());
  b->launches++;
  return MJB_OK;
}

int mjb_set_env_subset(mjb_batch* b, const int32_t* env_ids_dev, int32_t count) {
  if (!b) { mjb::set_error("mjb_set_env_subset: null batch"); return MJB_ERR_ARG; }
  if (b->img.dm.autoreset) {
    mjb::set_error("mjb_set_env_subset: level variants cannot auto-reset (a reset draws the env's level on the host)");
    return MJB_ERR_ARG;
  }
  if (!env_ids_dev) { b->subset = nullptr; b->subset_count = -1; return MJB_OK; }
  if (count < 0 || count > b->num_envs) { mjb::set_error("mjb_set_env_subset: count out of range"); return MJB_ERR_ARG; }
  if (b->img.dm.pack != 1) {
    mjb::set_error("mjb_set_env_subset: the batch packs several envs per warp; create it with MJB_SPEC_NO_PACK");
    return MJB_ERR_ARG;
  }
  b->subset = env_ids_dev; b->subset_count = count;
  return MJB_OK;
}

int mjb_phase_cycles(uint64_t* out, int32_t n) {
#if defined(MJB_PHASE_PROF)
  unsigned long long h[32];
  if (cudaMemcpyFromSymbol(h, mjb::g_phase_cycles, sizeof(h)) != cudaSuccess) return -1;
  for (int i = 0; i < n && i < 32; i++) out[i] = h[i];
  memset(h, 0, sizeof(h));
  cudaMemcpyToSymbol(mjb::g_phase_cycles, h, sizeof(h));
  return mjb::PH_COUNT;
#else
  (void)out; (void)n;
  return 0;
#endif
}

int mjb_batch_geometry(const mjb_batch* b, int32_t* grid, int32_t* warps_per_cta, int64_t* smem_bytes) {
  if (!b) return MJB_ERR_ARG;
  if (grid) *grid = b->grid;
  if (warps_per_cta) *warps_per_cta = b->warps;
  if (smem_bytes) *smem_bytes = (int64_t)b->smem_bytes;
  return MJB_OK;
}

}
```

mujoco_rl_environment_wrapper_b200/csrc/step_kernel.cuh:

```cuda
#pragma once
#include "../../include/mjb.h"
#include "dev_model.h"
#include "warp_prims.cuh"

namespace mjb {

#define MJB_MINVAL 1e-15f
#define MJB_MAX_PACK 4
#define MJB_BIG 1e30f

struct f3 { float x, y, z; };
struct q4 { float w, x, y, z; };
MJB_DEV f3 mk3(float x, float y, float z) { f3 r; r.x = x; r.y = y; r.z = z; return r; }
MJB_DEV f3 operator+(f3 a, f3 b) { return mk3(a.x + b.x, a.y + b.y, a.z + b.z); }
MJB_DEV f3 operator-(f3 a, f3 b) { return mk3(a.x - b.x, a.y - b.y, a.z - b.z); }
MJB_DEV f3 operator*(f3 a, float s) { return mk3(a.x * s, a.y * s, a.z * s); }
MJB_DEV float dot(f3 a, f3 b) { return a.x * b.x + a.y * b.y + a.z * b.z; }
MJB_DEV f3 cross(f3 a, f3 b) { return mk3(a.y * b.z - a.z * b.y, a.z * b.x - a.x * b.z, a.x * b.y - a.y * b.x); }
MJB_DEV f3 ld3(const float* p) { return mk3(p[0], p[1], p[2]); }
MJB_DEV void st3(float* p, f3 v) { p[0] = v.x; p[1] = v.y; p[2] = v.z; }
MJB_DEV float comp(f3 v, int i) { return i == 0 ? v.x : (i == 1 ? v.y : v.z); }
MJB_DEV q4 ldq(const float* p) { q4 q; q.w = p[0]; q.x = p[1]; q.y = p[2]; q.z = p[3]; return q; }
MJB_DEV q4 qmul(q4 a, q4 b) {
  q4 r;
  r.w = a.w * b.w - a.x * b.x - a.y * b.y - a.z * b.z;
  r.x = a.w * b.x + a.x * b.w + a.y * b.z - a.z * b.y;
  r.y = a.w * b.y - a.x * b.z + a.y * b.w + a.z * b.x;
  r.z = a.w * b.z + a.x * b.y - a.y * b.x + a.z * b.w;
  return r;
}
MJB_DEV q4 qnorm(q4 q) {
  float n2 = q.w * q.w + q.x * q.x + q.y * q.y + q.z * q.z;
  if (n2 < 1e-30f) { q.w = 1; q.x = q.y = q.z = 0; return q; }
  float inv = 1.0f / sqrtf(n2);
  q.w *= inv; q.x *= inv; q.y *= inv; q.z *= inv;
  return q;
}
MJB_DEV void q2m(q4 q, float* m) {
  float ww = q.w * q.w, xx = q.x * q.x, yy = q.y * q.y, zz = q.z * q.z;
  m[0] = ww + xx - yy - zz; m[4] = ww - xx + yy - zz; m[8] = ww - xx - yy + zz;
  m[1] = 2 * (q.x * q.y - q.w * q.z); m[2] = 2 * (q.x * q.z + q.w * q.y);
  m[3] = 2 * (q.x * q.y + q.w * q.z); m[5] = 2 * (q.y * q.z - q.w * q.x);
  m[6] = 2 * (q.x * q.z - q.w * q.y); m[7] = 2 * (q.y * q.z + q.w * q.x);
}
MJB_DEV f3 mulv(const float* m, f3 v) {
  return mk3(m[0] * v.x + m[1] * v.y + m[2] * v.z, m[3] * v.x + m[4] * v.y + m[5] * v.z, m[6] * v.x + m[7] * v.y + m[8] * v.z);
}
MJB_DEV f3 mulTv(const float* m, f3 v) {
  return mk3(m[0] * v.x + m[3] * v.y + m[6] * v.z, m[1] * v.x + m[4] * v.y + m[7] * v.z, m[2] * v.x + m[5] * v.y + m[8] * v.z);
}
MJB_DEV f3 colv(const float* m, int c) { return mk3(m[c], m[3 + c], m[6 + c]); }
MJB_DEV f3 qrot(q4 q, f3 v) {
  f3 u = mk3(q.x, q.y, q.z);
  f3 t = cross(u, v) * 2.0f;
  return v + t * q.w + cross(u, t);
}
MJB_DEV q4 axisangle(f3 ax, float ang) {
  float s, c;
  sincosf(0.5f * ang, &s, &c);
  q4 q; q.w = c; q.x = ax.x * s; q.y = ax.y * s; q.z = ax.z * s;
  return q;
}

struct Ctx {
  const DevModel* dm;
  const uint32_t* img;
  float* s;
  int lane;
  float* probe;
  int cta_threads;
  float* probe_quat;
  uint64_t* img_bar;
#if defined(MJB_PHASE_PROF)
  long long* t_last;
#endif
};
enum { PH_LOAD, PH_FK, PH_CRB, PH_RNE, PH_COLLIDE, PH_SENS, PH_CONSTR, PH_NEWTON_INIT, PH_NEWTON_GRAD, PH_NEWTON_HESS, PH_NEWTON_FACTOR,
       PH_NEWTON_LS, PH_INTEGRATE, PH_STORE, PH_EPILOGUE, PH_BARRIER, PH_ALIGN, PH_LS_ROWSMUL, PH_LS_MV, PH_LS_LOOP, PH_EPI_OBS, PH_EPI_STAGE, PH_EPI_PLUG, PH_COUNT };
#if defined(MJB_PHASE_PROF) && !defined(MJB_HOST_EMU)
__device__ unsigned long long g_phase_cycles[32];
__device__ __forceinline__ void mjb_phase(long long* t_last, int lane, int id) {
  __syncwarp();
  if (lane == 0) { long long t = clock64(); atomicAdd(&g_phase_cycles[id], (unsigned long long)(t - *t_last)); *t_last = t; }
}
#define MJB_PH(c, id) mjb_phase((c).t_last, (c).lane, (id))
#define MJB_COUNT(c, slot, n) do { if ((c).lane == 0) atomicAdd(&g_phase_cycles[slot], (unsigned long long)(n)); } while (0)
#else
#define MJB_PH(c, id) ((void)0)
#define MJB_COUNT(c, slot, n) ((void)0)
#endif
#define CI(f) ((const int*)(c.img + c.dm->off[IF_##f]))
#define CU(f) ((const uint32_t*)(c.img + c.dm->off[IF_##f]))
#define CF(f) ((const float*)(c.img + c.dm->off[IF_##f]))
#define SF(f) (c.s + c.dm->soff[SF_##f])
#define SI(f) ((int*)(c.s + c.dm->soff[SF_##f]))
#define PF(f, blk) (PRM ? c.s + c.dm->prm_soff + (blk) : CF(f))

MJB_DEV int tri(int i, int j) { return ((i * (i + 1)) >> 1) + j; }

MJB_DEV void inertia_mul(const float* I, f3 w, f3 v, f3& n, f3& f) {
  f3 h = mk3(I[1], I[2], I[3]);
  f = v * I[0] + cross(w, h);
  f3 Iw = mk3(I[4] * w.x + I[7] * w.y + I[8] * w.z, I[7] * w.x + I[5] * w.y + I[9] * w.z, I[8] * w.x + I[9] * w.y + I[6] * w.z);
  n = Iw + cross(h, v);
}

MJB_DEV void fk(const Ctx& c) {
  const DevModel& dm = *c.dm;
  const int* level_adr = CI(level_adr);
  float* qpos = SF(qpos);
  float *xpos = SF(xpos), *xquat = SF(xquat), *xmat = SF(xmat), *xipos = SF(xipos), *cdof = SF(cdof);
  MJB_NOUNROLL
  for (int l = 0; l < dm.nlevel; l++) {
    MJB_NOUNROLL
    for (int b = level_adr[l] + c.lane; b < level_adr[l + 1]; b += 32) {
      int p = CI(mb_parent)[b], root = CI(mb_root)[b];
      f3 pos = ld3(CF(mb_pos) + 3 * b);
      q4 quat = ldq(CF(mb_quat) + 4 * b);
      if (p >= 0) {
        pos = ld3(xpos + 3 * p) + mulv(xmat + 9 * p, pos);
        quat = qmul(ldq(xquat + 4 * p), quat);
      }
      int ja = CI(mb_jntadr)[b], jn = CI(mb_jntnum)[b];
      MJB_NOUNROLL
      for (int j = ja; j < ja + jn; j++) {
        int type = CI(jnt_type)[j], qa = CI(jnt_qposadr)[j], da = CI(jnt_dofadr)[j];
        if (type == MJB_JNT_FREE) {
          pos = ld3(qpos + qa);
          quat = qnorm(ldq(qpos + qa + 3));
          qpos[qa + 3] = quat.w; qpos[qa + 4] = quat.x; qpos[qa + 5] = quat.y; qpos[qa + 6] = quat.z;
        } else {
          f3 jpos = ld3(CF(jnt_pos) + 3 * j), jax = ld3(CF(jnt_axis) + 3 * j);
          f3 anchor = pos + qrot(quat, jpos), axis = qrot(quat, jax);
          float q = qpos[qa] - CF(jnt_qpos0)[j];
          st3(cdof + 6 * da, axis); st3(cdof + 6 * da + 3, anchor);
          if (type == MJB_JNT_HINGE) {
            quat = qmul(quat, axisangle(jax, q));
            pos = anchor - qrot(quat, jpos);
          } else {
            pos = pos + axis * q;
          }
        }
      }
      quat = qnorm(quat);
      float R[9];
      q2m(quat, R);
      st3(xpos + 3 * b, pos);
      xquat[4 * b] = quat.w; xquat[4 * b + 1] = quat.x; xquat[4 * b + 2] = quat.y; xquat[4 * b + 3] = quat.z;
#pragma unroll
      for (int i = 0; i < 9; i++) xmat[9 * b + i] = R[i];
      st3(xipos + 3 * b, pos + mulv(R, ld3(CF(mb_ipos) + 3 * b)));
      f3 o = (root == b) ? pos : ld3(xpos + 3 * root);
      MJB_NOUNROLL
      for (int j = ja; j < ja + jn; j++) {
        int type = CI(jnt_type)[j], da = CI(jnt_dofadr)[j];
        if (type == MJB_JNT_FREE) {
          for (int i = 0; i < 3; i++) {
            st3(cdof + 6 * (da + i), mk3(0, 0, 0));
            st3(cdof + 6 * (da + i) + 3, mk3(i == 0, i == 1, i == 2));
            f3 ax = colv(R, i);
            st3(cdof + 6 * (da + 3 + i), ax);
            st3(cdof + 6 * (da + 3 + i) + 3, cross(ax, o - pos));
          }
        } else if (type == MJB_JNT_HINGE) {
          f3 axis = ld3(cdof + 6 * da), anchor = ld3(cdof + 6 * da + 3);
          st3(cdof + 6 * da + 3, cross(axis, o - anchor));
        } else {
          f3 axis = ld3(cdof + 6 * da);
          st3(cdof + 6 * da, mk3(0, 0, 0)); st3(cdof + 6 * da + 3, axis);
        }
      }
    }
    MJB_SYNC();
  }
  float* cinert = SF(cinert);
  MJB_NOUNROLL
  for (int b = c.lane; b < dm.nmb; b += 32) {
    float R[9];
    q2m(qmul(ldq(xquat + 4 * b), ldq(CF(mb_iquat) + 4 * b)), R);
    f3 I = ld3(CF(mb_inertia) + 3 * b);
    float m = CF(mb_mass)[b];
    f3 cc = ld3(xipos + 3 * b) - ld3(xpos + 3 * CI(mb_root)[b]);
    float* o = cinert + 10 * b;
    o[0] = m; o[1] = m * cc.x; o[2] = m * cc.y; o[3] = m * cc.z;
    o[4] = R[0] * R[0] * I.x + R[1] * R[1] * I.y + R[2] * R[2] * I.z + m * (cc.y * cc.y + cc.z * cc.z);
    o[5] = R[3] * R[3] * I.x + R[4] * R[4] * I.y + R[5] * R[5] * I.z + m * (cc.x * cc.x + cc.z * cc.z);
    o[6] = R[6] * R[6] * I.x + R[7] * R[7] * I.y + R[8] * R[8] * I.z + m * (cc.x * cc.x + cc.y * cc.y);
    o[7] = R[0] * R[3] * I.x + R[1] * R[4] * I.y + R[2] * R[5] * I.z - m * cc.x * cc.y;
    o[8] = R[0] * R[6] * I.x + R[1] * R[7] * I.y + R[2] * R[8] * I.z - m * cc.x * cc.z;
    o[9] = R[3] * R[6] * I.x + R[4] * R[7] * I.y + R[5] * R[8] * I.z - m * cc.y * cc.z;
  }
  float *gpos = SF(gpos), *gmat = SF(gmat);
  MJB_NOUNROLL
  for (int g = c.lane; g < dm.ngeom; g += 32) {
    int slot = CI(geom_slot)[g];
    if (slot < 0) continue;
    int b = CI(geom_mb)[g];
    st3(gpos + 3 * slot, ld3(xpos + 3 * b) + mulv(xmat + 9 * b, ld3(CF(geom_pos) + 3 * g)));
    q2m(qmul(ldq(xquat + 4 * b), ldq(CF(geom_quat) + 4 * g)), gmat + 9 * slot);
  }
  float *spos = SF(spos), *smat = SF(smat);
  MJB_NOUNROLL
  for (int t = c.lane; t < dm.nsite; t += 32) {
    int b = CI(site_mb)[t];
    f3 lp = ld3(CF(site_pos) + 3 * t);
    q4 lq = ldq(CF(site_quat) + 4 * t);
    if (b >= 0) { lp = ld3(xpos + 3 * b) + mulv(xmat + 9 * b, lp); lq = qmul(ldq(xquat + 4 * b), lq); }
    st3(spos + 3 * t, lp);
    q2m(lq, smat + 9 * t);
  }
  MJB_SYNC();
}

MJB_DEV void crb_mass(const Ctx& c) {
  const DevModel& dm = *c.dm;
  const int* level_adr = CI(level_adr);
  float *cinert = SF(cinert), *crb = SF(crb), *M = SF(M), *cdof = SF(cdof);
  MJB_NOUNROLL
  for (int i = c.lane; i < 10 * dm.nmb; i += 32) crb[i] = cinert[i];
  MJB_NOUNROLL
  for (int i = c.lane; i < (dm.nv * (dm.nv + 1)) / 2; i += 32) M[i] = 0.f;
  MJB_SYNC();
  MJB_NOUNROLL
  for (int l = dm.nlevel - 2; l >= 0; l--) {
    MJB_NOUNROLL
    for (int b = level_adr[l] + c.lane; b < level_adr[l + 1]; b += 32) {
      int ca = CI(mb_childadr)[b], ce = CI(mb_childadr)[b + 1];
      if (ce > ca) {
        float acc[10];
#pragma unroll
        for (int i = 0; i < 10; i++) acc[i] = crb[10 * b + i];
        MJB_NOUNROLL
        for (int k = ca; k < ce; k++) {
          int ch = CI(mb_child)[k];
#pragma unroll
          for (int i = 0; i < 10; i++) acc[i] += crb[10 * ch + i];
        }
#pragma unroll
        for (int i = 0; i < 10; i++) crb[10 * b + i] = acc[i];
      }
    }
    MJB_SYNC();
  }
  MJB_NOUNROLL
  for (int i = c.lane; i < dm.nv; i += 32) {
    int b = CI(dof_mb)[i];
    f3 n, f;
    inertia_mul(crb + 10 * b, ld3(cdof + 6 * i), ld3(cdof + 6 * i + 3), n, f);
    for (int j = i; j >= 0; j = CI(dof_parent)[j]) {
      float v = dot(ld3(cdof + 6 * j), n) + dot(ld3(cdof + 6 * j + 3), f);
      if (j == i) v += CF(dof_armature)[i];
      M[tri(i, j)] = v;
    }
  }
  MJB_SYNC();
}

MJB_DEV void rne_pass(const Ctx& c, bool with_acc) {
  const DevModel& dm = *c.dm;
  const int* level_adr = CI(level_adr);
  float *cdof = SF(cdof), *cvel = SF(cvel), *cacc = SF(cacc), *qvel = SF(qvel), *qacc = SF(qacc);
  float *cinert = SF(cinert), *cfrc = SF(crb);
  MJB_NOUNROLL
  for (int l = 0; l < dm.nlevel; l++) {
    MJB_NOUNROLL
    for (int b = level_adr[l] + c.lane; b < level_adr[l + 1]; b += 32) {
      int p = CI(mb_parent)[b];
      f3 w = mk3(0, 0, 0), v = mk3(0, 0, 0), aw = mk3(0, 0, 0);
      f3 av = mk3(-dm.gravity[0], -dm.gravity[1], -dm.gravity[2]);
      if (p >= 0) { w = ld3(cvel + 6 * p); v = ld3(cvel + 6 * p + 3); aw = ld3(cacc + 6 * p); av = ld3(cacc + 6 * p + 3); }
      int da = CI(mb_dofadr)[b], dn = CI(mb_dofnum)[b];
      f3 wb = w, vb = v;
      MJB_NOUNROLL
      for (int d = da; d < da + dn; d++) {
        int kind = CI(dof_kind)[d];
        f3 sw = ld3(cdof + 6 * d), sv = ld3(cdof + 6 * d + 3);
        float qd = qvel[d];
        if (kind == DOF_FREE_ROT && d == da + 3) { wb = w; vb = v; }
        if (kind != DOF_FREE_TRANS) {
          f3 uw = kind == DOF_FREE_ROT ? wb : w, uv = kind == DOF_FREE_ROT ? vb : v;
          aw = aw + cross(uw, sw) * qd;
          av = av + (cross(uw, sv) + cross(uv, sw)) * qd;
        }
        if (with_acc) { aw = aw + sw * qacc[d]; av = av + sv * qacc[d]; }
        w = w + sw * qd; v = v + sv * qd;
      }
      st3(cvel + 6 * b, w); st3(cvel + 6 * b + 3, v);
      st3(cacc + 6 * b, aw); st3(cacc + 6 * b + 3, av);
      if (!with_acc) {
        f3 n1, f1, n2, f2;
        inertia_mul(cinert + 10 * b, aw, av, n1, f1);
        inertia_mul(cinert + 10 * b, w, v, n2, f2);
        st3(cfrc + 10 * b, n1 + cross(w, n2) + cross(v, f2));
        st3(cfrc + 10 * b + 3, f1 + cross(w, f2));
      }
    }
    MJB_SYNC();
  }
  if (with_acc) return;
  MJB_NOUNROLL
  for (int l = dm.nlevel - 2; l >= 0; l--) {
    MJB_NOUNROLL
    for (int b = level_adr[l] + c.lane; b < level_adr[l + 1]; b += 32) {
      int ca = CI(mb_childadr)[b], ce = CI(mb_childadr)[b + 1];
      MJB_NOUNROLL
      for (int k = ca; k < ce; k++) {
        int ch = CI(mb_child)[k];
#pragma unroll
        for (int i = 0; i < 6; i++) cfrc[10 * b + i] += cfrc[10 * ch + i];
      }
    }
    MJB_SYNC();
  }
  float *qfrc = SF(qfrc), *ctrl = SF(ctrl);
  MJB_NOUNROLL
  for (int d = c.lane; d < dm.nv; d += 32) {
    int b = CI(dof_mb)[d];
    float bias = dot(ld3(cdof + 6 * d), ld3(cfrc + 10 * b)) + dot(ld3(cdof + 6 * d + 3), ld3(cfrc + 10 * b + 3));
    float f = -CF(dof_damping)[d] * qvel[d] - bias;
    MJB_NOUNROLL
    for (int k = CI(dof_actadr)[d]; k < CI(dof_actadr)[d] + CI(dof_actnum)[d]; k++) {
      int u = CI(act_list)[k];
      const float* ap = CF(act_param) + 4 * u;
      float cv = ctrl[u];
      if (ap[1] != 0.f) cv = fminf(ap[3], fmaxf(ap[2], cv));
      f += ap[0] * cv;
    }
    qfrc[d] = f;
  }
  MJB_SYNC();
}

template <bool PRM = false>
MJB_DEV void kin_forward(const Ctx& c) {
  const DevModel& dm = *c.dm;
  const int* level_adr = CI(level_adr);
  float *qpos = SF(qpos), *qvel = SF(qvel);
  float *xpos = SF(xpos), *xquat = SF(xquat), *xmat = SF(xmat), *xipos = SF(xipos), *cdof = SF(cdof);
  float *cinert = SF(cinert), *cfrc = SF(crb), *cvel = SF(cvel), *cacc = SF(cacc);
  MJB_NOUNROLL
  for (int l = 0; l < dm.nlevel; l++) {
    MJB_NOUNROLL
    for (int b = level_adr[l] + c.lane; b < level_adr[l + 1]; b += 32) {
      const int p = CI(mb_parent)[b], root = CI(mb_root)[b];
      f3 pos = ld3(CF(mb_pos) + 3 * b);
      q4 quat = ldq(CF(mb_quat) + 4 * b);
      if (p >= 0) {
        pos = ld3(xpos + 3 * p) + mulv(xmat + 9 * p, pos);
        quat = qmul(ldq(xquat + 4 * p), quat);
      }
      const int ja = CI(mb_jntadr)[b], jn = CI(mb_jntnum)[b];
      MJB_NOUNROLL
      for (int j = ja; j < ja + jn; j++) {
        int type = CI(jnt_type)[j], qa = CI(jnt_qposadr)[j], da = CI(jnt_dofadr)[j];
        if (type == MJB_JNT_FREE) {
          pos = ld3(qpos + qa);
          quat = qnorm(ldq(qpos + qa + 3));
          qpos[qa + 3] = quat.w; qpos[qa + 4] = quat.x; qpos[qa + 5] = quat.y; qpos[qa + 6] = quat.z;
        } else {
          f3 jpos = ld3(CF(jnt_pos) + 3 * j), jax = ld3(CF(jnt_axis) + 3 * j);
          f3 anchor = pos + qrot(quat, jpos), axis = qrot(quat, jax);
          float q = qpos[qa] - CF(jnt_qpos0)[j];
          st3(cdof + 6 * da, axis); st3(cdof + 6 * da + 3, anchor);
          if (type == MJB_JNT_HINGE) {
            quat = qmul(quat, axisangle(jax, q));
            pos = anchor - qrot(quat, jpos);
          } else {
            pos = pos + axis * q;
          }
        }
      }
      quat = qnorm(quat);
      float R[9];
      q2m(quat, R);
      st3(xpos + 3 * b, pos);
      xquat[4 * b] = quat.w; xquat[4 * b + 1] = quat.x; xquat[4 * b + 2] = quat.y; xquat[4 * b + 3] = quat.z;
#pragma unroll
      for (int i = 0; i < 9; i++) xmat[9 * b + i] = R[i];
      const f3 ipos = pos + mulv(R, ld3(CF(mb_ipos) + 3 * b));
      st3(xipos + 3 * b, ipos);
      const f3 o = (root == b) ? pos : ld3(xpos + 3 * root);
      MJB_NOUNROLL
      for (int j = ja; j < ja + jn; j++) {
        int type = CI(jnt_type)[j], da = CI(jnt_dofadr)[j];
        if (type == MJB_JNT_FREE) {
          for (int i = 0; i < 3; i++) {
            st3(cdof + 6 * (da + i), mk3(0, 0, 0));
            st3(cdof + 6 * (da + i) + 3, mk3(i == 0, i == 1, i == 2));
            f3 ax = colv(R, i);
            st3(cdof + 6 * (da + 3 + i), ax);
            st3(cdof + 6 * (da + 3 + i) + 3, cross(ax, o - pos));
          }
        } else if (type == MJB_JNT_HINGE) {
          f3 axis = ld3(cdof + 6 * da), anchor = ld3(cdof + 6 * da + 3);
          st3(cdof + 6 * da + 3, cross(axis, o - anchor));
        } else {
          f3 axis = ld3(cdof + 6 * da);
          st3(cdof + 6 * da, mk3(0, 0, 0)); st3(cdof + 6 * da + 3, axis);
        }
      }
      f3 w = mk3(0, 0, 0), v = mk3(0, 0, 0), aw = mk3(0, 0, 0);
      f3 av = mk3(-dm.gravity[0], -dm.gravity[1], -dm.gravity[2]);
      if (p >= 0) { w = ld3(cvel + 6 * p); v = ld3(cvel + 6 * p + 3); aw = ld3(cacc + 6 * p); av = ld3(cacc + 6 * p + 3); }
      const int da = CI(mb_dofadr)[b], dn = CI(mb_dofnum)[b];
      if (p < 0 && root == b && dn == 6 && CI(dof_kind)[da] == DOF_FREE_TRANS) {
        v = ld3(qvel + da);
        w = mulv(R, ld3(qvel + da + 3));
        av = av + cross(v, w);
      } else {
        f3 wb = w, vb = v;
        MJB_NOUNROLL
        for (int d = da; d < da + dn; d++) {
          const int kind = CI(dof_kind)[d];
          const f3 sw = ld3(cdof + 6 * d), sv = ld3(cdof + 6 * d + 3);
          const float qd = qvel[d];
          if (kind == DOF_FREE_ROT && d == da + 3) { wb = w; vb = v; }
          if (kind != DOF_FREE_TRANS) {
            const f3 uw = kind == DOF_FREE_ROT ? wb : w, uv = kind == DOF_FREE_ROT ? vb : v;
            aw = aw + cross(uw, sw) * qd;
            av = av + (cross(uw, sv) + cross(uv, sw)) * qd;
          }
          w = w + sw * qd; v = v + sv * qd;
        }
      }
      st3(cvel + 6 * b, w); st3(cvel + 6 * b + 3, v);
      st3(cacc + 6 * b, aw); st3(cacc + 6 * b + 3, av);
    }
    MJB_SYNC();
  }
  MJB_NOUNROLL
  for (int b = c.lane; b < level_adr[dm.nlevel]; b += 32) {
    const f3 ipos = ld3(xipos + 3 * b), o = ld3(xpos + 3 * CI(mb_root)[b]);
    float I[10];
    {
      float Ri[9];
      q2m(qmul(ldq(xquat + 4 * b), ldq(CF(mb_iquat) + 4 * b)), Ri);
      const f3 In = ld3(PF(mb_inertia, prm_inertia(dm)) + 3 * b);
      const float m = PF(mb_mass, 0)[b];
      const f3 cc = ipos - o;
      I[0] = m; I[1] = m * cc.x; I[2] = m * cc.y; I[3] = m * cc.z;
      I[4] = Ri[0] * Ri[0] * In.x + Ri[1] * Ri[1] * In.y + Ri[2] * Ri[2] * In.z + m * (cc.y * cc.y + cc.z * cc.z);
      I[5] = Ri[3] * Ri[3] * In.x + Ri[4] * Ri[4] * In.y + Ri[5] * Ri[5] * In.z + m * (cc.x * cc.x + cc.z * cc.z);
      I[6] = Ri[6] * Ri[6] * In.x + Ri[7] * Ri[7] * In.y + Ri[8] * Ri[8] * In.z + m * (cc.x * cc.x + cc.y * cc.y);
      I[7] = Ri[0] * Ri[3] * In.x + Ri[1] * Ri[4] * In.y + Ri[2] * Ri[5] * In.z - m * cc.x * cc.y;
      I[8] = Ri[0] * Ri[6] * In.x + Ri[1] * Ri[7] * In.y + Ri[2] * Ri[8] * In.z - m * cc.x * cc.z;
      I[9] = Ri[3] * Ri[6] * In.x + Ri[4] * Ri[7] * In.y + Ri[5] * Ri[8] * In.z - m * cc.y * cc.z;
#pragma unroll
      for (int i = 0; i < 10; i++) cinert[10 * b + i] = I[i];
    }
    const f3 w = ld3(cvel + 6 * b), v = ld3(cvel + 6 * b + 3), aw = ld3(cacc + 6 * b), av = ld3(cacc + 6 * b + 3);
    f3 n1, f1, n2, f2;
    inertia_mul(I, aw, av, n1, f1);
    inertia_mul(I, w, v, n2, f2);
    st3(cfrc + 10 * b, n1 + cross(w, n2) + cross(v, f2));
    st3(cfrc + 10 * b + 3, f1 + cross(w, f2));
  }
  float *gpos = SF(gpos), *gmat = SF(gmat);
  MJB_NOUNROLL
  for (int g = c.lane; g < dm.ngeom; g += 32) {
    int slot = CI(geom_slot)[g];
    if (slot < 0) continue;
    int b = CI(geom_mb)[g];
    st3(gpos + 3 * slot, ld3(xpos + 3 * b) + mulv(xmat + 9 * b, ld3(CF(geom_pos) + 3 * g)));
    q2m(qmul(ldq(xquat + 4 * b), ldq(CF(geom_quat) + 4 * g)), gmat + 9 * slot);
  }
  float *spos = SF(spos), *smat = SF(smat);
  MJB_NOUNROLL
  for (int t = c.lane; t < dm.nsite; t += 32) {
    int b = CI(site_mb)[t];
    f3 lp = ld3(CF(site_pos) + 3 * t);
    q4 lq = ldq(CF(site_quat) + 4 * t);
    if (b >= 0) { lp = ld3(xpos + 3 * b) + mulv(xmat + 9 * b, lp); lq = qmul(ldq(xquat + 4 * b), lq); }
    st3(spos + 3 * t, lp);
    q2m(lq, smat + 9 * t);
  }
  {
    struct alignas(16) W4 { float a, b, c, d; };
    W4* m4 = (W4*)SF(M);
    const W4 z = {0.f, 0.f, 0.f, 0.f};
    MJB_NOUNROLL
    for (int i = c.lane; i < ((dm.nv * (dm.nv + 1)) / 2 + 3) / 4; i += 32) m4[i] = z;
  }
  MJB_SYNC();
}

template <bool PRM = false>
MJB_DEV void dyn_backward(const Ctx& c) {
  const DevModel& dm = *c.dm;
  const int* level_adr = CI(level_adr);
  float *crb = SF(cinert), *cfrc = SF(crb), *M = SF(M), *cdof = SF(cdof), *qvel = SF(qvel);
  MJB_NOUNROLL
  for (int l = dm.nlevel - 2; l >= 0; l--) {
    MJB_NOUNROLL
    for (int b = level_adr[l] + c.lane; b < level_adr[l + 1]; b += 32) {
      const int ca = CI(mb_childadr)[b], ce = CI(mb_childadr)[b + 1];
      if (ce > ca) {
        float acc[16];
#pragma unroll
        for (int i = 0; i < 10; i++) acc[i] = crb[10 * b + i];
#pragma unroll
        for (int i = 0; i < 6; i++) acc[10 + i] = cfrc[10 * b + i];
        MJB_NOUNROLL
        for (int k = ca; k < ce; k++) {
          const int ch = CI(mb_child)[k];
#pragma unroll
          for (int i = 0; i < 10; i++) acc[i] += crb[10 * ch + i];
#pragma unroll
          for (int i = 0; i < 6; i++) acc[10 + i] += cfrc[10 * ch + i];
        }
#pragma unroll
        for (int i = 0; i < 10; i++) crb[10 * b + i] = acc[i];
#pragma unroll
        for (int i = 0; i < 6; i++) cfrc[10 * b + i] = acc[10 + i];
      }
    }
    MJB_SYNC();
  }
  float *qfrc = SF(qfrc), *ctrl = SF(ctrl);
  MJB_NOUNROLL
  for (int i = c.lane; i < dm.nv; i += 32) {
    const int b = CI(dof_mb)[i];
    const f3 sw = ld3(cdof + 6 * i), sv = ld3(cdof + 6 * i + 3);
    f3 n, f;
    inertia_mul(crb + 10 * b, sw, sv, n, f);
    MJB_NOUNROLL
    for (int j = i; j >= 0; j = CI(dof_parent)[j]) {
      float v = dot(ld3(cdof + 6 * j), n) + dot(ld3(cdof + 6 * j + 3), f);
      if (j == i) v += CF(dof_armature)[i];
      M[tri(i, j)] = v;
    }
    const float bias = dot(sw, ld3(cfrc + 10 * b)) + dot(sv, ld3(cfrc + 10 * b + 3));
    float fq = -PF(dof_damping, prm_damping(dm))[i] * qvel[i] - bias;
    MJB_NOUNROLL
    for (int k = CI(dof_actadr)[i]; k < CI(dof_actadr)[i] + CI(dof_actnum)[i]; k++) {
      int u = CI(act_list)[k];
      const float* ap = CF(act_param) + 4 * u;
      float cv = ctrl[u];
      if (ap[1] != 0.f) cv = fminf(ap[3], fmaxf(ap[2], cv));
      fq += (PRM ? c.s[dm.prm_soff + prm_gear(dm) + u] : ap[0]) * cv;
    }
    qfrc[i] = fq;
  }
  MJB_SYNC();
}

struct GeomW { f3 pos; const float* mat; const float* size; int type; };
MJB_DEV GeomW geom_world(const Ctx& c, int g) {
  GeomW r;
  int slot = CI(geom_slot)[g];
  r.type = CI(geom_type)[g];
  r.size = CF(geom_size) + 3 * g;
  if (slot >= 0) { r.pos = ld3(SF(gpos) + 3 * slot); r.mat = SF(gmat) + 9 * slot; }
  else { r.pos = ld3(CF(geom_pos) + 3 * g); r.mat = CF(geom_mat) + 9 * g; }
  return r;
}
struct ConOut { float dist; f3 pos, n, t; };

MJB_DEV int plane_sphere(f3 pp, f3 n, f3 cs, float r, float margin, ConOut& o) {
  float dist = dot(cs - pp, n) - r;
  if (dist > margin) return 0;
  o.dist = dist; o.pos = cs - n * (r + 0.5f * dist); o.n = n; o.t = mk3(0, 0, 0);
  return 1;
}
MJB_DEV int sphere_sphere(f3 c1, float r1, f3 c2, float r2, float margin, ConOut& o) {
  f3 d = c2 - c1;
  float cd = sqrtf(dot(d, d)), dist = cd - r1 - r2;
  if (dist > margin) return 0;
  f3 n = cd < MJB_MINVAL ? mk3(1, 0, 0) : d * (1.0f / cd);
  o.dist = dist; o.pos = c1 + n * (r1 + 0.5f * dist); o.n = n; o.t = mk3(0, 0, 0);
  return 1;
}
// ... 143 lines not shown
  }
  const bool ref1 = fax < 3;
  const int ri = ref1 ? fax : fax - 3;
  const GeomW& A = ref1 ? a : b;
  const GeomW& B = ref1 ? b : a;
  f3 nA = colv(A.mat, ri);
  if (dot(nA, B.pos - A.pos) < 0.f) nA = nA * -1.f;
  const f3 nb = mulTv(B.mat, nA);
  int bj = 0;
  if (fabsf(nb.y) > fabsf(nb.x)) bj = 1;
  if (fabsf(nb.z) > fabsf(comp(nb, bj))) bj = 2;
  const f3 mB = colv(B.mat, bj) * (comp(nb, bj) > 0.f ? -1.f : 1.f);
  const int bu = bj == 2 ? 0 : bj + 1, bw = bu == 2 ? 0 : bu + 1, au = ri == 2 ? 0 : ri + 1, aw = au == 2 ? 0 : au + 1;
  const f3 Bu = colv(B.mat, bu) * B.size[bu], Bw = colv(B.mat, bw) * B.size[bw], Au = colv(A.mat, au), Aw = colv(A.mat, aw);
  const f3 fc = B.pos + mB * B.size[bj];
  const float su = A.size[au], sw = A.size[aw];
  auto s0 = [](int q) { return (q == 0 || q == 3) ? 1.f : -1.f; };
  auto s1 = [](int q) { return q < 2 ? 1.f : -1.f; };
  bool hit = false;
  f3 x = mk3(0, 0, 0);
  if (lane < 4) {
    x = fc + Bu * s0(lane) + Bw * s1(lane);
    const f3 rel = x - A.pos;
    hit = fabsf(dot(rel, Au)) <= su && fabsf(dot(rel, Aw)) <= sw;
  } else if (lane < 8) {
    const int q = lane - 4;
    const float U = s0(q) * su, W = s1(q) * sw;
    int pos_ = 0, neg_ = 0;
#pragma unroll
    for (int e = 0; e < 4; e++) {
      const f3 p0 = fc + Bu * s0(e) + Bw * s1(e) - A.pos, p1 = fc + Bu * s0((e + 1) & 3) + Bw * s1((e + 1) & 3) - A.pos;
      const float u0 = dot(p0, Au), w0 = dot(p0, Aw), u1 = dot(p1, Au), w1 = dot(p1, Aw);
      const float cr = (u1 - u0) * (W - w0) - (w1 - w0) * (U - u0);
      pos_ += cr > 0.f; neg_ += cr < 0.f;
    }
    if (pos_ == 4 || neg_ == 4) {
      const f3 x0 = A.pos + nA * A.size[ri] + Au * U + Aw * W;
      const float t = dot(mB, fc - x0) / dot(mB, nA);
      x = x0 + nA * t;
      hit = true;
    }
  } else if (lane < 24) {
    const int e = (lane - 8) >> 2, side = (lane - 8) & 3;
    const f3 p0 = fc + Bu * s0(e) + Bw * s1(e), p1 = fc + Bu * s0((e + 1) & 3) + Bw * s1((e + 1) & 3);
    const f3 ax_ = side < 2 ? Au : Aw, ot_ = side < 2 ? Aw : Au;
    const float sg = (side & 1) ? -1.f : 1.f, lim_ = side < 2 ? su : sw, olim = side < 2 ? sw : su;
    const float f0 = sg * dot(p0 - A.pos, ax_) - lim_, f1 = sg * dot(p1 - A.pos, ax_) - lim_;
    if ((f0 < 0.f && f1 > 0.f) || (f0 > 0.f && f1 < 0.f)) {
      x = p0 + (p1 - p0) * (f0 / (f0 - f1));
      hit = fabsf(dot(x - A.pos, ot_)) <= olim;
    }
  }
  if (hit) {
    const float dist = dot(x - A.pos, nA) - A.size[ri];
    if (dist > margin) hit = false;
    o.dist = dist; o.pos = x - nA * (0.5f * dist); o.n = ref1 ? nA : nA * -1.f;
  }
  return hit;
}

MJB_DEV void make_frame(f3 n, f3 t, float* fr) {
  float nn = sqrtf(dot(n, n));
  n = n * (1.0f / nn);
  if (dot(t, t) < 0.25f) {
    t = mk3(0, 0, 0);
    if (n.y < 0.5f && n.y > -0.5f) t.y = 1; else t.z = 1;
  }
  t = t - n * dot(n, t);
  t = t * (1.0f / sqrtf(dot(t, t)));
  st3(fr, n); st3(fr + 3, t); st3(fr + 6, cross(n, t));
}

MJB_DEV void store_contact(const Ctx& c, int idx, const ConOut& o, int pair, float mu) {
  float* r = SF(con) + CON_STRIDE * idx;
  r[CON_DIST] = o.dist;
  st3(r + CON_POS, o.pos);
  make_frame(o.n, o.t, r + CON_FRAME);
  ((int*)r)[CON_PAIR] = pair;
  r[CON_MU] = mu;
}

template <bool PRM = false>
MJB_DEV int collide(const Ctx& c, int* tot) {
  const DevModel& dm = *c.dm;
  const uint32_t* pairs = CU(pair_pack);
  int* cand = SI(cand);
  int ncand = 0;
  uint32_t act_lo = 0xffffffffu, act_hi = 0xffffffffu;
  MJB_NOUNROLL
  for (int b0 = 0; b0 < dm.nblock; b0 += 32) {
    const int bi = b0 + c.lane;
    bool on = false;
    if (bi < dm.nblock) {
      const int* rec = CI(bp_block) + BP_STRIDE * bi;
      const int partner = rec[BP_PARTNER];
      if (partner == BP_ALWAYS) on = true;
      else {
        const float reach = CF(bp_block)[BP_STRIDE * bi + BP_REACH] + CF(bp_block)[BP_STRIDE * bi + BP_MARGIN];
        const f3 ca = ld3(SF(xpos) + 3 * rec[BP_ROOT_A]);
        if (partner >= 0) {
          f3 d = ld3(SF(xpos) + 3 * partner) - ca;
          on = dot(d, d) <= reach * reach;
        } else {
          const int g = -1 - partner;
          const f3 gp = ld3(CF(geom_pos) + 3 * g);
          const float* gm = CF(geom_mat) + 9 * g;
          const int type = CI(geom_type)[g];
          if (type == MJB_GEOM_PLANE) on = dot(ca - gp, colv(gm, 2)) <= reach;
          else if (type == MJB_GEOM_BOX) on = point_box_dist(mulTv(gm, ca - gp), CF(geom_size) + 3 * g) <= reach;
          else { f3 d = gp - ca; float rr = reach + CF(geom_rbound)[g]; on = dot(d, d) <= rr * rr; }
        }
      }
    }
    const uint32_t bal = MJB_BALLOT(on);
    if (b0 == 0) act_lo = bal; else act_hi = bal;
  }
  if (dm.nblock > 0 && dm.nblock <= 32) act_hi = 0;
  const int npass = (dm.npair + 31) >> 5;
  MJB_NOUNROLL
  for (int pb = 0; pb < npass; pb += 32) {
  uint32_t live = 0;
  {
    const int ps = pb + c.lane;
    bool on = false;
    if (ps < npass) { const uint32_t* pm = CU(bp_passmask) + 2 * ps; on = ((pm[0] & act_lo) | (pm[1] & act_hi)) != 0u; }
    live = MJB_BALLOT(on);
  }
  MJB_NOUNROLL
  while (live) {
    const int base = (pb + MJB_FFS(live) - 1) << 5;
    live &= live - 1u;
    int p = base + c.lane;
    bool keep = false;
    if (p < dm.npair) {
      uint32_t pk = pairs[p];
      int g1 = pk & 0xfff, g2 = (pk >> 12) & 0xfff;
      float margin = CF(pclass)[PC_STRIDE * (pk >> 24) + PC_MARGIN];
      GeomW a = geom_world(c, g1), b = geom_world(c, g2);
      float rb2 = CF(geom_rbound)[g2];
      if (a.type == MJB_GEOM_PLANE) keep = dot(b.pos - a.pos, colv(a.mat, 2)) <= rb2 + margin;
      else if (b.type == MJB_GEOM_BOX) {
        keep = point_box_dist(mulTv(b.mat, a.pos - b.pos), b.size) <= CF(geom_rbound)[g1] + margin;
      } else {
        float rr = CF(geom_rbound)[g1] + rb2 + margin;
        f3 d = b.pos - a.pos;
        keep = dot(d, d) <= rr * rr;
      }
    }
    uint32_t bal = MJB_BALLOT(keep);
    int idx = ncand + MJB_POPC(bal & ((1u << c.lane) - 1u));
    if (keep && idx < dm.maxcand) cand[idx] = p;
    ncand += MJB_POPC(bal);
  }
  }
  if (ncand > dm.maxcand) ncand = dm.maxcand;
  MJB_SYNC();
  int ncon = 0;
  MJB_NOUNROLL
  for (int base = 0; base < ncand; base += 32) {
    int i = base + c.lane;
    int n = 0, p = -1;
    ConOut o[2];
    float mu = 0.f;
    if (i < ncand) {
      p = cand[i];
      uint32_t pk = pairs[p];
      int g1 = pk & 0xfff, g2 = (pk >> 12) & 0xfff;
// ... 41 lines not shown
    }
  }
  MJB_NOUNROLL
  for (int cb = 0; cb < ncand; cb += 32) {
  uint32_t multi = 0;
  {
    const int i = cb + c.lane;
    bool is_multi = false;
    if (i < ncand) {
      const uint32_t pk = pairs[cand[i]];
      const int t1 = CI(geom_type)[pk & 0xfff], t2 = CI(geom_type)[(pk >> 12) & 0xfff];
      is_multi = t2 == MJB_GEOM_BOX && (t1 == MJB_GEOM_PLANE || t1 == MJB_GEOM_BOX);
    }
    multi = MJB_BALLOT(is_multi);
  }
  MJB_NOUNROLL
  while (multi) {
    const int i = cb + MJB_FFS(multi) - 1;
    multi &= multi - 1u;
    int p = cand[i];
    uint32_t pk = pairs[p];
    int g1 = pk & 0xfff, g2 = (pk >> 12) & 0xfff;
    int t1 = CI(geom_type)[g1];
    const float* pc = CF(pclass) + PC_STRIDE * (pk >> 24);
    float margin = pc[PC_MARGIN], mu = PRM ? fmaxf(c.s[dm.prm_soff + prm_friction(dm) + g1], c.s[dm.prm_soff + prm_friction(dm) + g2]) : pc[PC_MU];
    GeomW a = geom_world(c, g1), b = geom_world(c, g2);
    bool hit = false;
    ConOut o;
    o.t = mk3(0, 0, 0);
    int lim = 4;
    if (t1 == MJB_GEOM_PLANE) {
      if (c.lane < 8) {
        f3 nrm = colv(a.mat, 2);
        float dist0 = dot(b.pos - a.pos, nrm);
        f3 vec = mk3(b.size[0] * ((c.lane & 1) ? 1.f : -1.f), b.size[1] * ((c.lane & 2) ? 1.f : -1.f), b.size[2] * ((c.lane & 4) ? 1.f : -1.f));
        f3 corner = mulv(b.mat, vec);
        float ld = dot(nrm, corner);
        if (!(dist0 + ld > margin || ld > 0)) {
          hit = true; o.dist = dist0 + ld; o.pos = corner + b.pos - nrm * (0.5f * o.dist); o.n = nrm;
        }
      }
    } else {
      lim = 8;
      hit = box_box_lane(c.lane, a, b, margin, o);
    }
    uint32_t bal = MJB_BALLOT(hit);
    int rank = MJB_POPC(bal & ((1u << c.lane) - 1u));
    int add = MJB_POPC(bal);
    if (add > lim) add = lim;
    const int copy = dm.pack > 1 ? g1 / dm.ngeom1 : 0;
    int room = 0;
#pragma unroll
    for (int cp = 0; cp < MJB_MAX_PACK; cp++)
      if (cp == copy) { room = dm.maxcon1 - tot[cp]; tot[cp] += add; }
    if (room < 0) room = 0;
    if (add > room) add = room;
    if (hit && rank < add) store_contact(c, ncon + rank, o, p, mu);
    ncon += add;
  }
  }
  MJB_SYNC();
  return ncon;
}

MJB_DEV_NOINLINE float impedance_pow(float x, float mid, float power) {
  if (x <= mid) return powf(x, power) / powf(mid, power - 1.f);
  return 1.f - powf(1.f - x, power) / powf(1.f - mid, power - 1.f);
}
MJB_DEV float impedance(const float* solimp, float pos, float margin) {
  float dmin = solimp[0], dmax = solimp[1], width = solimp[2], mid = solimp[3], power = solimp[4];
  if (dmin == dmax || width <= MJB_MINVAL) return 0.5f * (dmin + dmax);
  float x = fabsf((pos - margin) / width);
  if (x >= 1.f) return dmax;
  if (x <= 0.f) return dmin;
  float y;
  if (power == 1.f) y = x;
  else if (power == 2.f) y = x <= mid ? x * x / mid : 1.f - (1.f - x) * (1.f - x) / (1.f - mid);
  else y = impedance_pow(x, mid, power);
  return dmin + y * (dmax - dmin);
}

template <bool PRM = false>
MJB_DEV void make_constraints(const Ctx& c, int ncon) {
  const DevModel& dm = *c.dm;
  float *efcD = SF(efcD), *efcAref = SF(efcAref), *qpos = SF(qpos), *qvel = SF(qvel);
  MJB_NOUNROLL
  for (int k = c.lane; k < dm.nlim; k += 32) {
    const float* lp = CF(lim_param) + LIM_STRIDE * k;
    float q = qpos[CI(lim_qposadr)[k]], v = qvel[CI(lim_dof)[k]];
#pragma unroll
    for (int side = 0; side < 2; side++) {
      float dist = side == 0 ? q - lp[LIM_LO] : lp[LIM_HI] - q;
      float D = 0.f, aref = 0.f;
      if (dist < lp[LIM_MARGIN]) {
        float imp = impedance(lp + LIM_SOLIMP, dist, lp[LIM_MARGIN]);
        float R = fmaxf(MJB_MINVAL, (1.f - imp) * lp[LIM_INVW] / imp);
        D = 1.f / R;
        float vel = side == 0 ? v : -v;
        aref = -lp[LIM_B] * vel - lp[LIM_K] * imp * (dist - lp[LIM_MARGIN]);
      }
      efcD[2 * k + side] = D; efcAref[2 * k + side] = aref;
    }
  }
  float *J = SF(J), *con = SF(con), *cdof = SF(cdof), *xpos = SF(xpos);
  const uint32_t* pairs = CU(pair_pack);
  MJB_NOUNROLL
  for (int k = c.lane; k < ncon; k += 32) {
    float* r = con + CON_STRIDE * k;
    uint32_t pk = pairs[((const int*)r)[CON_PAIR]];
    int b1 = CI(geom_mb)[pk & 0xfff], b2 = CI(geom_mb)[(pk >> 12) & 0xfff];
    uint32_t mask = (b1 >= 0 ? CU(mb_dofmask)[2 * b1] : 0u) ^ (b2 >= 0 ? CU(mb_dofmask)[2 * b2] : 0u);
    ((uint32_t*)r)[CON_MASK] = mask;
#pragma unroll
    for (int wi = 0; wi < 4; wi++) {
      uint32_t word = 0u;
#pragma unroll
      for (int bi = 0; bi < 4; bi++) {
        if (mask) { word |= (uint32_t)(MJB_FFS(mask) - 1) << (8 * bi); mask &= mask - 1; }
      }
      ((uint32_t*)r)[CON_DOFS + wi] = word;
    }
  }
  MJB_SYNC();
  MJB_NOUNROLL
  for (int d = c.lane; d < dm.nv; d += 32) {
    f3 sw = ld3(cdof + 6 * d), sv = ld3(cdof + 6 * d + 3);
    int root = CI(mb_root)[CI(dof_mb)[d]];
    f3 o = ld3(xpos + 3 * root);
    uint32_t bit = 1u << d;
    MJB_NOUNROLL
    for (int k = 0; k < ncon; k++) {
      const float* r = con + CON_STRIDE * k;
      uint32_t mask = ((const uint32_t*)r)[CON_MASK];
      if (!(mask & bit)) continue;
      uint32_t pk = pairs[((const int*)r)[CON_PAIR]];
      int b2 = CI(geom_mb)[(pk >> 12) & 0xfff];
      float sgn = (b2 >= 0 && (CU(mb_dofmask)[2 * b2] & bit)) ? 1.f : -1.f;
      f3 vel = (sv + cross(sw, ld3(r + CON_POS) - o)) * sgn;
      int idx = MJB_POPC(mask & (bit - 1u));
      J[(3 * k) * dm.ldj + idx] = dot(ld3(r + CON_FRAME), vel);
      J[(3 * k + 1) * dm.ldj + idx] = dot(ld3(r + CON_FRAME + 3), vel);
      J[(3 * k + 2) * dm.ldj + idx] = dot(ld3(r + CON_FRAME + 6), vel);
    }
  }
  MJB_SYNC();
  int base = 2 * dm.nlim;
  MJB_NOUNROLL
  for (int k = c.lane; k < ncon; k += 32) {
    const float* r = con + CON_STRIDE * k;
    uint32_t pk = pairs[((const int*)r)[CON_PAIR]];
    const float* pc = CF(pclass) + PC_STRIDE * (pk >> 24);
    int b1 = CI(geom_mb)[pk & 0xfff], b2 = CI(geom_mb)[(pk >> 12) & 0xfff];
    float tran = (b1 >= 0 ? CF(mb_invweight)[b1] : 0.f) + (b2 >= 0 ? CF(mb_invweight)[b2] : 0.f);
    float mu = PRM ? r[CON_MU] : pc[PC_MU], dist = r[CON_DIST], inc = pc[PC_INCMARGIN];
    float imp = impedance(pc + PC_SOLIMP, dist, inc);
    float vn = 0.f, v1 = 0.f, v2 = 0.f;
    {
      uint32_t mm = ((const uint32_t*)r)[CON_MASK];
      int m = 0;
      MJB_NOUNROLL
      while (mm) {
        float qd = qvel[MJB_FFS(mm) - 1];
        mm &= mm - 1;
        vn += J[(3 * k) * dm.ldj + m] * qd; v1 += J[(3 * k + 1) * dm.ldj + m] * qd; v2 += J[(3 * k + 2) * dm.ldj + m] * qd;
        m++;
      }
    }
// ... 120 lines not shown
  MJB_SYNC();
  const int nrow = t1 - t0, lq = own ? li : NBT;
  const float* lp = Lout + tri(t0 + NBT - 1, 0) + lane;
#pragma unroll
  for (int kk = NBT - 1; kk >= 1; kk--) {
    const int k = t0 + kk;
    const float xk = MJB_SHFL(x, k);
    const bool in = lq < kk && kk < nrow;
    const float lk = *(in ? lp : Lout);
    x = in ? x - lk * xk : x;
    lp -= k;
  }
  return x;
}
MJB_DEV float factor_solve_reg(const float* A, float* Lout, int lane, int t0, int t1, int nb, float diag_add, float b) {
  if (nb <= 6) return factor_solve_regT<6>(A, Lout, lane, t0, t1, diag_add, b);
  if (nb <= 14) return factor_solve_regT<14>(A, Lout, lane, t0, t1, diag_add, b);
  return factor_solve_regT<MJB_NB>(A, Lout, lane, t0, t1, diag_add, b);
}
template <int NBT>
MJB_DEV_NOINLINE float chol_solve_regT(const float* A, float* Lout, int lane, int n, float diag_add, float b) {
  float l[NBT];
  const bool own = lane < n;
  const int rowoff = own ? tri(lane, 0) : 0;
#pragma unroll
  for (int k = 0; k < NBT; k++) {
    float v = (own && k <= lane) ? A[rowoff + k] : 0.f;
    l[k] = (k == lane) ? v + diag_add : v;
  }
  float rinv = 1.f;
#pragma unroll
  for (int j = 0; j < NBT; j++) {
    float s0 = l[j], s1 = 0.f;
#pragma unroll
    for (int k = 0; k < j; k++) {
      const float ljk = MJB_SHFL(l[k], j);
      if (k & 1) s1 -= l[k] * ljk; else s0 -= l[k] * ljk;
    }
    const float s = s0 + s1;
    const float inv = MJB_RSQRT(fmaxf(MJB_SHFL(s, j), 1e-20f));
    l[j] = s * inv;
    if (lane == j) rinv = inv;
  }
  MJB_SYNC();
#pragma unroll
  for (int k = 0; k < NBT; k++)
    if (own && k <= lane) Lout[rowoff + k] = l[k];
  float x = b;
#pragma unroll
  for (int k = 0; k < NBT; k++) {
    const float yk = MJB_SHFL(x * rinv, k);
    x = lane > k ? x - l[k] * yk : x;
  }
  x *= rinv;
  MJB_SYNC();
#pragma unroll
  for (int k = NBT - 1; k >= 1; k--) {
    const float zk = MJB_SHFL(x * rinv, k);
    const bool in = lane < k && k < n;
    const float lk = Lout[in ? tri(k, 0) + lane : 0];
    x = in ? x - lk * zk : x;
  }
  return x * rinv;
}

MJB_DEV float factor_solve(const float* A, float* L, int lane, int t0, int t1, int nb, float diag_add, float b, int nv) {
  if (MJB_LIKELY(nb <= MJB_NB)) return factor_solve_reg(A, L, lane, t0, t1, nb, diag_add, b);
  if (nb == nv) {
    if (nv <= 28) return chol_solve_regT<28>(A, L, lane, nv, diag_add, b);
    return chol_solve_regT<32>(A, L, lane, nv, diag_add, b);
  }
  if (A != L) {
    MJB_NOUNROLL
    for (int i = lane; i < (nv * (nv + 1)) / 2; i += 32) L[i] = A[i];
    MJB_SYNC();
  }
  if (lane < t1 && diag_add != 0.f) L[tri(lane, lane)] += diag_add;
  MJB_SYNC();
  float invd = cholesky(L, lane, t0, t1, nb);
  return chol_solve(L, lane, t0, t1, nb, invd, b);
}

MJB_DEV void rows_mul(const Ctx& c, int ncon, const float* x, float* out, const float* sub) {
  const DevModel& dm = *c.dm;
  MJB_NOUNROLL
  for (int k = c.lane; k < dm.nlim; k += 32) {
    float v = x[CI(lim_dof)[k]];
    out[2 * k] = v - (sub ? sub[2 * k] : 0.f);
    out[2 * k + 1] = -v - (sub ? sub[2 * k + 1] : 0.f);
  }
  const float* J = SF(J);
  const float* con = SF(con);
  const int base = 2 * dm.nlim;
  MJB_NOUNROLL
  for (int k0 = 0; k0 < ncon; k0 += 4) {
    const int k = k0 + (c.lane >> 3), l8 = c.lane & 7;
    float sn = 0.f, s1 = 0.f, s2 = 0.f;
    if (k < ncon) {
      const uint32_t* rec = (const uint32_t*)(con + CON_STRIDE * k);
      const int nb = MJB_POPC(rec[CON_MASK]);
      const float *Jn = J + (3 * k) * dm.ldj, *J1 = Jn + dm.ldj, *J2 = J1 + dm.ldj;
      MJB_NOUNROLL
      for (int m = l8; m < nb; m += 8) {
        const float xv = x[(rec[CON_DOFS + (m >> 2)] >> (8 * (m & 3))) & 0xff];
        sn += Jn[m] * xv; s1 += J1[m] * xv; s2 += J2[m] * xv;
      }
    }
#pragma unroll
    for (int o = 4; o > 0; o >>= 1) { sn += MJB_SHFL_XOR(sn, o); s1 += MJB_SHFL_XOR(s1, o); s2 += MJB_SHFL_XOR(s2, o); }
    if (k < ncon && l8 < 4) {
      const float mu = con[CON_STRIDE * k + CON_MU];
      const float v = sn + ((l8 & 1) ? -mu : mu) * (l8 < 2 ? s1 : s2);
      out[base + 4 * k + l8] = v - (sub ? sub[base + 4 * k + l8] : 0.f);
    }
  }
  MJB_SYNC();
}

MJB_DEV float jt_mul(const Ctx& c, int ncon, int base, int mylim, const float* w) {
  const DevModel& dm = *c.dm;
  const float* J = SF(J);
  const float* con = SF(con);
  float out = mylim >= 0 ? w[2 * mylim] - w[2 * mylim + 1] : 0.f;
  MJB_NOUNROLL
  for (int k = 0; k < ncon; k++) {
    const uint32_t mask = ((const uint32_t*)(con + CON_STRIDE * k))[CON_MASK];
    if (!((mask >> c.lane) & 1u)) continue;
    const float mu = con[CON_STRIDE * k + CON_MU];
    const float w0 = w[base + 4 * k], w1 = w[base + 4 * k + 1], w2 = w[base + 4 * k + 2], w3 = w[base + 4 * k + 3];
    const int idx = MJB_POPC(mask & ((1u << c.lane) - 1u));
    out += J[(3 * k) * dm.ldj + idx] * ((w0 + w1) + (w2 + w3)) + J[(3 * k + 1) * dm.ldj + idx] * (mu * (w0 - w1)) +
           J[(3 * k + 2) * dm.ldj + idx] * (mu * (w2 - w3));
  }
  return out;
}
MJB_DEV void jt_mul2(const Ctx& c, int ncon, int base, int mylim, const float* w, const float* v, float& ow, float& ov) {
  const DevModel& dm = *c.dm;
  const float* J = SF(J);
  const float* con = SF(con);
  ow = mylim >= 0 ? w[2 * mylim] - w[2 * mylim + 1] : 0.f;
  ov = mylim >= 0 ? v[2 * mylim] - v[2 * mylim + 1] : 0.f;
  MJB_NOUNROLL
  for (int k = 0; k < ncon; k++) {
    const uint32_t mask = ((const uint32_t*)(con + CON_STRIDE * k))[CON_MASK];
    if (!((mask >> c.lane) & 1u)) continue;
    const float mu = con[CON_STRIDE * k + CON_MU];
    const float w0 = w[base + 4 * k], w1 = w[base + 4 * k + 1], w2 = w[base + 4 * k + 2], w3 = w[base + 4 * k + 3];
    const float v0 = v[base + 4 * k], v1 = v[base + 4 * k + 1], v2 = v[base + 4 * k + 2], v3 = v[base + 4 * k + 3];
    const int idx = MJB_POPC(mask & ((1u << c.lane) - 1u));
    const float jn = J[(3 * k) * dm.ldj + idx], j1 = J[(3 * k + 1) * dm.ldj + idx], j2 = J[(3 * k + 2) * dm.ldj + idx];
    ow += jn * ((w0 + w1) + (w2 + w3)) + j1 * (mu * (w0 - w1)) + j2 * (mu * (w2 - w3));
    ov += jn * ((v0 + v1) + (v2 + v3)) + j1 * (mu * (v0 - v1)) + j2 * (mu * (v2 - v3));
  }
}

MJB_DEV int newton(const Ctx& c, int ncon) {
  const DevModel& dm = *c.dm;
  const int nv = dm.nv, lane = c.lane;
  const int t0 = CI(dof_t0)[lane], t1 = CI(dof_t1)[lane];
  float *M = SF(M), *H = SF(H), *a = SF(qacc), *sv = SF(vecC);
  float *D = SF(efcD), *frc = SF(efcAref), *jar = SF(efcJar), *jv = SF(efcJv);
  const float* J = SF(J);
  const float* con = SF(con);
  const uint32_t* pairs = CU(pair_pack);
  const int base = 2 * dm.nlim, nrow = base + 4 * ncon;
  float *qfrc = SF(qfrc), *tot = SF(vecA);
  {
    float x = factor_solve(M, H, lane, t0, t1, dm.maxtree, 0.f, lane < nv ? qfrc[lane] : 0.f, nv);
    if (lane < nv) a[lane] = x;
    MJB_SYNC();
  }
  rows_mul(c, ncon, a, jar, frc);
  MJB_NOUNROLL
  for (int r = lane; r < nrow; r += 32) { const float x = jar[r]; frc[r] = x < 0.f ? -D[r] * x : 0.f; }
  MJB_SYNC();
  float g = 0.f;
  if (lane < nv) {
    const float q = jt_mul(c, ncon, base, CI(dof_lim)[lane], frc);
    g = -q;
    tot[lane] = qfrc[lane] + q;
  }
  MJB_PH(c, PH_NEWTON_INIT);
  int it = 0;
  float last_step = 0.f;
  MJB_NOUNROLL
  for (;;) {
    const float qf = lane < nv ? qfrc[lane] : 0.f, ma = lane < nv ? tot[lane] + g : 0.f;
    const float gn = wsum(g * g), fn = wsum(qf * qf + ma * ma);
    const float amax = wmax(lane < nv ? fabsf(a[lane]) : 0.f), smax = wmax(last_step);
    const bool stalled = it > 0 && smax <= 1e-7f * (1.f + amax);
    const bool done = gn <= dm.solver_tol * dm.solver_tol * (fn + 1e-12f) || it >= dm.solver_iterations || stalled;
    MJB_PH(c, PH_NEWTON_GRAD);
    if (done) break;
    it++;
    {
      struct alignas(16) W4 { float a, b, c, d; };
      const W4* src = (const W4*)M;
      W4* dst = (W4*)H;
      MJB_NOUNROLL
      for (int i = lane; i < ((nv * (nv + 1)) / 2 + 3) / 4; i += 32) dst[i] = src[i];
    }
    MJB_SYNC();
    float hdiag = 0.f;
    {
      const int mylim = CI(dof_lim)[lane];
      if (mylim >= 0) hdiag = (jar[2 * mylim] < 0 ? D[2 * mylim] : 0.f) + (jar[2 * mylim + 1] < 0 ? D[2 * mylim + 1] : 0.f);
    }
    bool coupled = false;
    MJB_NOUNROLL
    for (int k = 0; k < ncon; k++) {
      uint32_t pk = pairs[((const int*)(con + CON_STRIDE * k))[CON_PAIR]];
      int b1 = CI(geom_mb)[pk & 0xfff], b2 = CI(geom_mb)[(pk >> 12) & 0xfff];
      uint32_t mask = ((const uint32_t*)(con + CON_STRIDE * k))[CON_MASK];
      float mu = con[CON_STRIDE * k + CON_MU];
      float w0 = jar[base + 4 * k] < 0 ? D[base + 4 * k] : 0.f, w1 = jar[base + 4 * k + 1] < 0 ? D[base + 4 * k + 1] : 0.f;
      float w2 = jar[base + 4 * k + 2] < 0 ? D[base + 4 * k + 2] : 0.f, w3 = jar[base + 4 * k + 3] < 0 ? D[base + 4 * k + 3] : 0.f;
      float cnn = w0 + w1 + w2 + w3;
      if (cnn == 0.f) continue;
      if (b1 >= 0 && b2 >= 0 && CI(mb_root)[b1] != CI(mb_root)[b2]) coupled = true;
      float cn1 = mu * (w0 - w1), c11 = mu * mu * (w0 + w1), cn2 = mu * (w2 - w3), c22 = mu * mu * (w2 + w3);
      const int nb = MJB_POPC(mask), npairs = (nb * (nb + 1)) >> 1;
      const uint32_t* dofs = (const uint32_t*)(con + CON_STRIDE * k) + CON_DOFS;
      const float *Jn = J + (3 * k) * dm.ldj, *J1 = Jn + dm.ldj, *J2 = J1 + dm.ldj;
      MJB_NOUNROLL
      for (int p = lane; p < npairs; p += 32) {
        uint32_t rc = CU(tri_lut)[p];
        int mi = rc & 0xff, mj = rc >> 8;
        int di = (dofs[mi >> 2] >> (8 * (mi & 3))) & 0xff, dj = (dofs[mj >> 2] >> (8 * (mj & 3))) & 0xff;
        float ni = Jn[mi], ai = J1[mi], bi = J2[mi], nj = Jn[mj], aj = J1[mj], bj = J2[mj];
        H[tri(di, dj)] += ni * (cnn * nj + cn1 * aj + cn2 * bj) + ai * (cn1 * nj + c11 * aj) + bi * (cn2 * nj + c22 * bj);
      }
      MJB_SYNC();
    }
    MJB_SYNC();
    const int h0 = coupled ? 0 : t0, h1 = coupled ? (lane < nv ? nv : 0) : t1, hb = coupled ? nv : dm.maxtree;
    MJB_PH(c, PH_NEWTON_HESS);
    float s = factor_solve(H, H, lane, h0, h1, hb, hdiag, -g, nv);
    if (lane < nv) sv[lane] = s; else s = 0.f;
    MJB_SYNC();
    MJB_PH(c, PH_NEWTON_FACTOR);
// ... 43 lines not shown
#endif
    }
#if defined(MJB_PHASE_PROF) && !defined(MJB_HOST_EMU)
    if (lane == 0 && alpha == 1.f) atomicAdd(&g_phase_cycles[31], 1ull);
#endif
    MJB_SYNC();
    if (lane < nv) {
      float gu, q;
      jt_mul2(c, ncon, base, CI(dof_lim)[lane], jv, frc, gu, q);
      g = (1.f - alpha) * g - gu;
      tot[lane] = qfrc[lane] + q;
    }
    MJB_PH(c, PH_NEWTON_LS);
  }
  if (lane < nv) SF(vecB)[lane] = g;
  MJB_SYNC();
  return it;
}

MJB_DEV int quad_roots(float a, float b, float cc, float* x) {
  if (a < MJB_MINVAL) return 0;
  float det = b * b - a * cc;
  if (det < 0) return 0;
  float sq = sqrtf(det);
  x[0] = (-b - sq) / a; x[1] = (-b + sq) / a;
  return 2;
}
MJB_DEV float ray_geom(f3 pos, const float* R, const float* size, f3 pnt, f3 vec, int type) {
  if (type == MJB_GEOM_SPHERE) {
    f3 d = pnt - pos;
    float x[2];
    if (!quad_roots(dot(vec, vec), dot(vec, d), dot(d, d) - size[0] * size[0], x)) return -1.f;
    return x[0] >= 0 ? x[0] : (x[1] >= 0 ? x[1] : -1.f);
  }
  f3 lp = mulTv(R, pnt - pos), lv = mulTv(R, vec);
  if (type == MJB_GEOM_PLANE) {
    if (lv.z > -MJB_MINVAL) return -1.f;
    float x = -lp.z / lv.z;
    if (x < 0) return -1.f;
    float p0 = lp.x + x * lv.x, p1 = lp.y + x * lv.y;
    if ((size[0] <= 0 || fabsf(p0) <= size[0]) && (size[1] <= 0 || fabsf(p1) <= size[1])) return x;
    return -1.f;
  }
  float best = -1.f;
  if (type == MJB_GEOM_CAPSULE) {
    float r = size[0], h = size[1], x[2];
    if (quad_roots(lv.x * lv.x + lv.y * lv.y, lp.x * lv.x + lp.y * lv.y, lp.x * lp.x + lp.y * lp.y - r * r, x))
      for (int i = 0; i < 2; i++)
        if (fabsf(lp.z + x[i] * lv.z) <= h && x[i] >= 0 && (best < 0 || x[i] < best)) best = x[i];
    for (int sg = -1; sg <= 1; sg += 2) {
      f3 d = lp - mk3(0, 0, sg * h);
      if (quad_roots(dot(lv, lv), dot(lv, d), dot(d, d) - r * r, x))
        for (int i = 0; i < 2; i++)
          if (sg * (lp.z + x[i] * lv.z) >= h && x[i] >= 0 && (best < 0 || x[i] < best)) best = x[i];
    }
    return best;
  }
  float tn = -MJB_BIG, tf = MJB_BIG;
#pragma unroll
  for (int a = 0; a < 3; a++) {
    const float p = comp(lp, a), v = comp(lv, a), sz = size[a];
    if (fabsf(v) < MJB_MINVAL) {
      if (fabsf(p) > sz) return -1.f;
    } else {
      const float inv = 1.f / v, t1 = (-sz - p) * inv, t2 = (sz - p) * inv;
      tn = fmaxf(tn, fminf(t1, t2));
      tf = fminf(tf, fmaxf(t1, t2));
    }
  }
  if (tn > tf || tf < 0.f) return -1.f;
  return tn >= 0.f ? tn : tf;
}

MJB_DEV float cutoff(const Ctx& c, int i, float x) {
  float cut = CF(sensor_cutoff)[i];
  if (cut <= 0) return x;
  int dt = CI(sensor_dtype)[i];
  if (dt == 0) return fminf(cut, fmaxf(-cut, x));
  if (dt == 1) return fminf(cut, x);
  return x;
}

MJB_DEV void sensors_pos(const Ctx& c) {
  const DevModel& dm = *c.dm;
  float* sens = SF(sens);
  MJB_NOUNROLL
  for (int i = 0; i < dm.nsensor; i++) {
    int type = CI(sensor_type)[i], t = CI(sensor_site)[i], adr = CI(sensor_adr)[i];
    if (type == MJB_SENS_RANGEFINDER) {
      f3 pnt = ld3(SF(spos) + 3 * t), vec = colv(SF(smat) + 9 * t, 2);
      int bex = CI(site_mb)[t];
      float best = MJB_BIG;
      MJB_NOUNROLL
      for (int g = c.lane; g < dm.ngeom; g += 32) {
        int gb = CI(geom_mb)[g];
        if ((gb >= 0 && gb == bex) || !CI(geom_ray)[g]) continue;
        GeomW gw = geom_world(c, g);
        if (gw.type != MJB_GEOM_PLANE) {
          f3 mvec = gw.pos - pnt;
          float rb = CF(geom_rbound)[g], tca = dot(mvec, vec), mm = dot(mvec, mvec);
          if (mm - tca * tca > rb * rb || (tca < 0.f && mm > rb * rb)) continue;
        }
        float x = ray_geom(gw.pos, gw.mat, gw.size, pnt, vec, gw.type);
        if (x >= 0 && x < best) best = x;
      }
      best = wmin(best);
      if (c.lane == 0) sens[adr] = cutoff(c, i, best >= MJB_BIG ? -1.f : best);
    } else if (type >= MJB_SENS_FRAMEXAXIS && type <= MJB_SENS_FRAMEZAXIS) {
      if (c.lane < 3) sens[adr + c.lane] = cutoff(c, i, SF(smat)[9 * t + 3 * c.lane + (type - MJB_SENS_FRAMEXAXIS)]);
    }
  }
  MJB_SYNC();
}

MJB_DEV void sensors_acc(const Ctx& c, int ncon) {
  const DevModel& dm = *c.dm;
  if (!dm.need_acc_sensors) return;
  float* sens = SF(sens);
  bool did_rne = false;
  const uint32_t* pairs = CU(pair_pack);
  const int base = 2 * dm.nlim;
  MJB_NOUNROLL
  for (int i = 0; i < dm.nsensor; i++) {
    int type = CI(sensor_type)[i], t = CI(sensor_site)[i], adr = CI(sensor_adr)[i];
    if (type == MJB_SENS_TOUCH) {
      int body = CI(site_mb)[t];
      float total = 0.f;
      MJB_NOUNROLL
      for (int k = c.lane; k < ncon; k += 32) {
        const float* r = SF(con) + CON_STRIDE * k;
        uint32_t pk = pairs[((const int*)r)[CON_PAIR]];
        int b1 = CI(geom_mb)[pk & 0xfff], b2 = CI(geom_mb)[(pk >> 12) & 0xfff];
        if (body < 0 || (b1 != body && b2 != body)) continue;
        float fn = 0.f;
        for (int e = 0; e < 4; e++) {
          float x = SF(efcJar)[base + 4 * k + e];
          if (x < 0) fn -= SF(efcD)[base + 4 * k + e] * x;
        }
        if (fn <= MJB_MINVAL) continue;
        f3 ray = ld3(r + CON_FRAME);
        if (b2 == body) ray = ray * -1.f;
        if (ray_geom(ld3(SF(spos) + 3 * t), SF(smat) + 9 * t, CF(site_size) + 3 * t, ld3(r + CON_POS), ray, CI(site_type)[t]) >= 0)
          total += fn;
      }
      total = wsum(total);
      if (c.lane == 0) sens[adr] = cutoff(c, i, total);
    } else if (type == MJB_SENS_ACCELEROMETER) {
      if (!did_rne) { rne_pass(c, true); did_rne = true; }
      int b = CI(site_mb)[t];
      if (c.lane == 0) {
        f3 acc = mk3(-dm.gravity[0], -dm.gravity[1], -dm.gravity[2]);
        if (b >= 0) {
          f3 w = ld3(SF(cvel) + 6 * b), v = ld3(SF(cvel) + 6 * b + 3), aw = ld3(SF(cacc) + 6 * b), av = ld3(SF(cacc) + 6 * b + 3);
          f3 r = ld3(SF(spos) + 3 * t) - ld3(SF(xpos) + 3 * CI(mb_root)[b]);
          acc = av + cross(aw, r) + cross(w, v + cross(w, r));
        }
        f3 loc = mulTv(SF(smat) + 9 * t, acc);
        sens[adr] = cutoff(c, i, loc.x); sens[adr + 1] = cutoff(c, i, loc.y); sens[adr + 2] = cutoff(c, i, loc.z);
      }
    }
  }
  MJB_SYNC();
}

MJB_DEV void sensors_frame(const Ctx& c) {
  const DevModel& dm = *c.dm;
  float* sens = SF(sens);
  const float *xpos = SF(xpos), *xquat = SF(xquat), *xmat = SF(xmat), *cvel = SF(cvel);
  MJB_NOUNROLL
  for (int i = c.lane; i < dm.nsensor; i += 32) {
    const int type = CI(sensor_type)[i], adr = CI(sensor_adr)[i];
    if (type == MJB_SENS_JOINTPOS || type == MJB_SENS_JOINTVEL) {
      const int a = CI(sensor_site)[i];
      sens[adr] = cutoff(c, i, type == MJB_SENS_JOINTPOS ? SF(qpos)[a] : SF(qvel)[a]);
      continue;
    }
    const bool axis = type >= KSENS_OBJ_AXIS;
    if (!axis && type != MJB_SENS_VELOCIMETER && type != MJB_SENS_GYRO && type != MJB_SENS_FRAMEPOS && type != MJB_SENS_FRAMEQUAT &&
        type != MJB_SENS_FRAMELINVEL && type != MJB_SENS_FRAMEANGVEL)
      continue;
    const float* rec = (const float*)(c.img + dm.off_sens_obj + SO_STRIDE * i);
    const int b = ((const int*)rec)[SO_MB];
    f3 p = ld3(rec + SO_POS), w = mk3(0, 0, 0), v = mk3(0, 0, 0);
    q4 q = ldq(rec + SO_QUAT);
    if (b >= 0) {
      p = ld3(xpos + 3 * b) + mulv(xmat + 9 * b, p);
      q = qmul(ldq(xquat + 4 * b), q);
      w = ld3(cvel + 6 * b);
      v = ld3(cvel + 6 * b + 3) + cross(w, p - ld3(xpos + 3 * CI(mb_root)[b]));
    }
    if (type == MJB_SENS_FRAMEQUAT) {
      q = qnorm(q);
      sens[adr] = q.w; sens[adr + 1] = q.x; sens[adr + 2] = q.y; sens[adr + 3] = q.z;
      continue;
    }
    f3 r = type == MJB_SENS_FRAMEPOS ? p : (type == MJB_SENS_FRAMEANGVEL ? w : v);
    if (axis) {
      const int a = type - KSENS_OBJ_AXIS;
      r = qrot(q, mk3(a == 0, a == 1, a == 2));
    } else if (type == MJB_SENS_GYRO || type == MJB_SENS_VELOCIMETER) {
      q4 qc = q;
      qc.x = -q.x; qc.y = -q.y; qc.z = -q.z;
      r = qrot(qc, type == MJB_SENS_GYRO ? w : v);
    }
    sens[adr] = cutoff(c, i, r.x); sens[adr + 1] = cutoff(c, i, r.y); sens[adr + 2] = cutoff(c, i, r.z);
  }
  MJB_SYNC();
}

template <bool PRM = false>
MJB_DEV int forward(const Ctx& c, bool sensors, bool probes, int* iters_out, int* found) {
  MJB_PH(c, PH_INTEGRATE);
  kin_forward<PRM>(c);
  if (probes) {
    const DevModel& dm = *c.dm;
    MJB_NOUNROLL
    for (int p = c.lane; p < dm.nprobe; p += 32) {
      int kind = CI(probe_kind)[p], id = CI(probe_id)[p];
      f3 v = kind == PROBE_BODY ? ld3(SF(xipos) + 3 * id) : (kind == PROBE_GEOM ? ld3(SF(gpos) + 3 * id) : ld3(CF(probe_const) + 3 * p));
      c.probe[4 * p] = v.x; c.probe[4 * p + 1] = v.y; c.probe[4 * p + 2] = v.z; c.probe[4 * p + 3] = 0.f;
      if (c.probe_quat && kind != PROBE_CONST) {
        q4 q;
        if (kind == PROBE_BODY) q = ldq(SF(xquat) + 4 * id);
        else {
          int g = 0;
          MJB_NOUNROLL
          for (int k = 0; k < dm.ngeom; k++) if (CI(geom_slot)[k] == id) g = k;
          q = qnorm(qmul(ldq(SF(xquat) + 4 * CI(geom_mb)[g]), ldq(CF(geom_quat) + 4 * g)));
        }
        c.probe_quat[4 * p] = q.w; c.probe_quat[4 * p + 1] = q.x; c.probe_quat[4 * p + 2] = q.y; c.probe_quat[4 * p + 3] = q.z;
      }
    }
    MJB_SYNC();
  }
  MJB_PH(c, PH_FK);
  dyn_backward<PRM>(c);
  MJB_PH(c, PH_RNE);
  if (sensors && c.dm->ext_sensors) sensors_frame(c);
  int tot[MJB_MAX_PACK] = {0, 0, 0, 0};
  int ncon = collide<PRM>(c, tot);
  MJB_PH(c, PH_COLLIDE);
  if (found) {
#pragma unroll
    for (int cp = 0; cp < MJB_MAX_PACK; cp++) found[cp] += tot[cp] > c.dm->maxcon1 ? tot[cp] - c.dm->maxcon1 : 0;
  }
  if (sensors) sensors_pos(c);
  MJB_PH(c, PH_SENS);
  make_constraints<PRM>(c, ncon);
  MJB_PH(c, PH_CONSTR);
  int it = newton(c, ncon);
  MJB_CTA_SYNC(c.cta_threads);
  MJB_PH(c, PH_ALIGN);
  if (iters_out) *iters_out = it;
  if (sensors) sensors_acc(c, ncon);
  MJB_PH(c, PH_SENS);
  return ncon;
}

MJB_DEV void integrate_pos(const Ctx& c, float* qpos, const float* v, float h) {
  const DevModel& dm = *c.dm;
  MJB_NOUNROLL
  for (int j = c.lane; j < dm.njnt; j += 32) {
    int qa = CI(jnt_qposadr)[j], da = CI(jnt_dofadr)[j];
    if (CI(jnt_type)[j] == MJB_JNT_FREE) {
      for (int i = 0; i < 3; i++) qpos[qa + i] += h * v[da + i];
      f3 w = ld3(v + da + 3);
      float nw = sqrtf(dot(w, w)), ang = nw * h;
      if (ang > 0.f) {
        q4 q = qnorm(qmul(ldq(qpos + qa + 3), axisangle(w * (1.0f / nw), ang)));
        qpos[qa + 3] = q.w; qpos[qa + 4] = q.x; qpos[qa + 5] = q.y; qpos[qa + 6] = q.z;
      }
    } else {
      qpos[qa] += h * v[da];
    }
  }
}

template <bool PRM = false>
MJB_DEV int substep(const Ctx& c, bool sensors, bool integrate, int* iters_out, int* dropped) {
  const DevModel& dm = *c.dm;
  const int nv = dm.nv, lane = c.lane;
  float *qpos = SF(qpos), *qvel = SF(qvel), *qacc = SF(qacc);
  const float h = dm.timestep;
  const bool rk4 = integrate && dm.integrator == MJB_INT_RK4;
  const int nstage = rk4 ? 4 : 1;
  float* rk = SF(rk);
  float *q0 = rk, *v0 = rk + dm.nq, *dq = rk + dm.nq + nv, *dv = rk + dm.nq + 2 * nv;
  int ncon = 0;
  MJB_NOUNROLL
  for (int st = 0; st < nstage; st++) {
    if (st > 0) {
      const float A = st == 3 ? 1.0f : 0.5f;
      float vprev = lane < nv ? qvel[lane] : 0.f, aprev = lane < nv ? qacc[lane] : 0.f;
      MJB_SYNC();
      if (lane < nv) SF(vecC)[lane] = A * vprev;
      MJB_NOUNROLL
      for (int i = lane; i < dm.nq; i += 32) qpos[i] = q0[i];
      MJB_SYNC();
      integrate_pos(c, qpos, SF(vecC), h);
      if (lane < nv) qvel[lane] = v0[lane] + h * A * aprev;
      MJB_SYNC();
    }
    ncon = forward<PRM>(c, sensors && st == 0, sensors && st == nstage - 1, st == 0 ? iters_out : nullptr, dropped);
    if (rk4) {
      const float Bw = (st == 0 || st == 3) ? (1.f / 6) : (1.f / 3);
      if (st == 0) {
        MJB_NOUNROLL
        for (int i = lane; i < dm.nq; i += 32) q0[i] = qpos[i];
        if (lane < nv) { v0[lane] = qvel[lane]; dq[lane] = 0.f; dv[lane] = 0.f; }
      }
      if (lane < nv) { dq[lane] += Bw * qvel[lane]; dv[lane] += Bw * qacc[lane]; }
      MJB_SYNC();
    }
  }
  if (!integrate) return ncon;
  if (rk4) {
    if (lane < nv) qvel[lane] = v0[lane] + h * dv[lane];
    MJB_NOUNROLL
    for (int i = lane; i < dm.nq; i += 32) qpos[i] = q0[i];
    MJB_SYNC();
    integrate_pos(c, qpos, dq, h);
    MJB_SYNC();
    return ncon;
  }
  float acc = lane < nv ? qacc[lane] : 0.f;
  if (PRM || dm.has_damping) {
    float *M = SF(M), *H = SF(H);
    const int t0 = CI(dof_t0)[lane], t1 = CI(dof_t1)[lane];
    float rhs = lane < nv ? SF(vecA)[lane] : 0.f;
    MJB_SYNC();
    acc = factor_solve(M, H, lane, t0, t1, dm.maxtree, lane < nv ? h * PF(dof_damping, prm_damping(dm))[lane] : 0.f, rhs, nv);
  }
  if (lane < nv) qvel[lane] += h * acc;
  MJB_SYNC();
  integrate_pos(c, qpos, qvel, h);
  MJB_SYNC();
  return ncon;
}

}
```

mujoco_rl_environment_wrapper_b200/csrc/tma_prims.cuh:

```cuda
#pragma once
#include <stdint.h>

namespace mjb {

__device__ __forceinline__ uint32_t smem_u32(const void* p) { return (uint32_t)__cvta_generic_to_shared(p); }
__device__ __forceinline__ void mbar_init(uint64_t* bar, int count) {
  asm volatile("mbarrier.init.shared::cta.b64 [%0], %1;" ::"r"(smem_u32(bar)), "r"(count));
}
__device__ __forceinline__ void mbar_fence_init() { asm volatile("fence.mbarrier_init.release.cluster;" ::: "memory"); }
__device__ __forceinline__ void mbar_expect_tx(uint64_t* bar, uint32_t bytes) {
  asm volatile("mbarrier.arrive.expect_tx.shared::cta.b64 _, [%0], %1;" ::"r"(smem_u32(bar)), "r"(bytes) : "memory");
}
__device__ __forceinline__ void bulk_g2s(void* dst, const void* src, uint32_t bytes, uint64_t* bar) {
  asm volatile("cp.async.bulk.shared::cluster.global.mbarrier::complete_tx::bytes [%0], [%1], %2, [%3];" ::"r"(smem_u32(dst)),
               "l"(src), "r"(bytes), "r"(smem_u32(bar))
               : "memory");
}
__device__ __forceinline__ void mbar_wait(uint64_t* bar, uint32_t parity) {
  asm volatile(
      "{\n"
      ".reg .pred p;\n"
      "WAIT_LOOP:\n"
      "mbarrier.try_wait.parity.shared::cta.b64 p, [%0], %1;\n"
      "@p bra WAIT_DONE;\n"
      "bra WAIT_LOOP;\n"
      "WAIT_DONE:\n"
      "}\n" ::"r"(smem_u32(bar)),
      "r"(parity)
      : "memory");
}

}
```

mujoco_rl_environment_wrapper_b200/csrc/warp_prims.cuh:

```cuda
#pragma once
#include <math.h>
#include <stdint.h>
#include <string.h>

#if defined(MJB_HOST_EMU)
#include "../../tests/emu/simt_emu.h"
#define MJB_DEV inline
#define MJB_DEV_NOINLINE inline
#define MJB_NOUNROLL
#define MJB_LANE() (simt::lane())
#define MJB_SYNC() simt::barrier()
#define MJB_SHFL(v, src) simt::shfl((v), (src))
#define MJB_SHFL_XOR(v, m) simt::shfl_xor((v), (m))
#define MJB_BALLOT(p) simt::ballot(p)
#define MJB_POPC(x) __builtin_popcount(x)
#define MJB_FFS(x) __builtin_ffs(x)
#define MJB_RSQRT(x) (1.0f / sqrtf(x))
inline uint32_t mjb_f2u(float x) { uint32_t u; memcpy(&u, &x, 4); return u; }
#define MJB_F2U(x) mjb_f2u(x)
#define MJB_G2S(dst, src) (*(dst) = *(src))
#define MJB_G2S_WAIT() ((void)0)
#define MJB_CTA_SYNC(nthreads) ((void)0)
#else
#define MJB_DEV __device__ __forceinline__
#define MJB_DEV_NOINLINE __device__ __noinline__
#define MJB_NOUNROLL _Pragma("unroll 1")
#define MJB_LANE() ((int)(threadIdx.x & 31))
#define MJB_SYNC() __syncwarp()
#define MJB_SHFL(v, src) __shfl_sync(0xffffffffu, (v), (src))
#define MJB_SHFL_XOR(v, m) __shfl_xor_sync(0xffffffffu, (v), (m))
#define MJB_BALLOT(p) __ballot_sync(0xffffffffu, (p))
#define MJB_POPC(x) __popc(x)
#define MJB_FFS(x) __ffs(x)
#define MJB_RSQRT(x) rsqrtf(x)
#define MJB_F2U(x) __float_as_uint(x)
__device__ __forceinline__ void mjb_g2s4(float* dst, const float* src) {
  asm volatile("cp.async.ca.shared.global [%0], [%1], 4;" ::"r"((uint32_t)__cvta_generic_to_shared(dst)), "l"(src) : "memory");
}
#define MJB_G2S(dst, src) mjb_g2s4((dst), (src))
#define MJB_G2S_WAIT() asm volatile("cp.async.wait_all;" ::: "memory")
__device__ __forceinline__ void mjb_cta_sync(int nthreads) {
  if (nthreads > 32) asm volatile("bar.sync 1, %0;" ::"r"(nthreads) : "memory");
}
#define MJB_CTA_SYNC(nthreads) mjb_cta_sync(nthreads)
#endif

#define MJB_UNLIKELY(x) __builtin_expect(!!(x), 0)
#define MJB_LIKELY(x) __builtin_expect(!!(x), 1)

namespace mjb {

MJB_DEV float wsum(float v) {
#pragma unroll
  for (int o = 16; o > 0; o >>= 1) v += MJB_SHFL_XOR(v, o);
  return v;
}
MJB_DEV float wmin(float v) {
#pragma unroll
  for (int o = 16; o > 0; o >>= 1) v = fminf(v, MJB_SHFL_XOR(v, o));
  return v;
}
MJB_DEV float wmax(float v) {
#pragma unroll
  for (int o = 16; o > 0; o >>= 1) v = fmaxf(v, MJB_SHFL_XOR(v, o));
  return v;
}

}
```

Measured before the change: 56.45 million.

## JIT-compile a model-specialised env kernel with NVRTC and constant shape fields

Adds an NVRTC path that recompiles the environment kernel at batch creation, with the model's shape fields and image/scratch offsets baked in as compile-time constants (SpecModel). Loop bounds and buffer offsets that were read from the grid-constant DevModel become literals, so the compiler can unroll loops, fold addresses and free registers. The original generic kernel stays as a fallback when compilation fails or the GENERIC flag is set. This adds JIT compile time at startup, a dependency on libnvrtc, and more build complexity.

New measurement: 67.29 million, median of 6. 19.2% higher.

```diff
diff --git a/include/mjb.h b/include/mjb.h
--- a/include/mjb.h
+++ b/include/mjb.h
@@ -1,7 +1,9 @@
 #ifndef MJB_H_
 #define MJB_H_
 
+#if !defined(__CUDACC_RTC__)
 #include <stdint.h>
+#endif
 
 #include "mjb_blob.h"
 
@@ -102,7 +104,8 @@
 enum {
   MJB_SPEC_NO_PACK = 1,
   MJB_SPEC_AUTORESET = 2,
-  MJB_SPEC_RANDOMIZE = 4
+  MJB_SPEC_RANDOMIZE = 4,
+  MJB_SPEC_GENERIC = 8
 };
 
 
@@ -161,6 +164,8 @@
 int mjb_set_env_subset(mjb_batch* b, const int32_t* env_ids_dev, int32_t count);
 int mjb_render(mjb_batch* b, const int32_t* cam_ids, int32_t ncams, int32_t width, int32_t height, uint8_t* rgb_dev);
 int mjb_batch_geometry(const mjb_batch* b, int32_t* grid, int32_t* warps_per_cta, int64_t* smem_bytes);
+int mjb_batch_spec_info(const mjb_batch* b, int32_t* specialised, double* compile_ms, char* reason, int32_t reason_len);
+int mjb_spec_compile(const mjb_model* m, const mjb_env_spec* spec, int32_t num_envs, double* compile_ms, void* cubin, int64_t* cubin_bytes);
 int mjb_phase_cycles(uint64_t* out, int32_t n);
 uint32_t mjb_draw_u32(uint64_t seed, uint32_t env, uint32_t agent, uint32_t counter);
 float mjb_reset_action(uint64_t seed, uint32_t env, uint32_t agent, uint32_t dim, uint32_t ep, float low, float high);
diff --git a/include/mjb_blob.h b/include/mjb_blob.h
--- a/include/mjb_blob.h
+++ b/include/mjb_blob.h
@@ -1,8 +1,13 @@
 #ifndef MJB_BLOB_H_
 #define MJB_BLOB_H_
 
+#if defined(__CUDACC_RTC__)
+typedef signed char int8_t; typedef unsigned char uint8_t; typedef short int16_t; typedef unsigned short uint16_t;
+typedef int int32_t; typedef unsigned int uint32_t; typedef long long int64_t; typedef unsigned long long uint64_t;
+#else
 #include <stdint.h>
 #include <string.h>
+#endif
 
 #ifdef __cplusplus
 extern "C" {
@@ -38,6 +43,7 @@
        MJB_OBJ_ACTUATOR = 19, MJB_OBJ_SENSOR = 20 };
 enum { MJB_INT_EULER = 0, MJB_INT_RK4 = 1 };
 
+#if !defined(__CUDACC_RTC__)
 static inline const mjb_blob_field* mjb_blob_find(const void* blob, const char* name) {
   const mjb_blob_header* h = (const mjb_blob_header*)blob;
   const mjb_blob_field* f = (const mjb_blob_field*)((const char*)blob + sizeof(mjb_blob_header));
@@ -57,6 +63,7 @@
   if (count) *count = f->count;
   return (const double*)((const char*)blob + f->offset);
 }
+#endif
 
 #ifdef __cplusplus
 }
diff --git a/mujoco_rl_environment_wrapper_b200/_lib.py b/mujoco_rl_environment_wrapper_b200/_lib.py
--- a/mujoco_rl_environment_wrapper_b200/_lib.py
+++ b/mujoco_rl_environment_wrapper_b200/_lib.py
@@ -8,7 +8,7 @@
 LIB_PATH = os.environ.get("MJB_LIB") or os.path.join(_HERE, "libmjb.so")
 
 MAX_AGENTS, MAX_PLUGINS, MAX_TARGETS, MAX_EXTRA_PROBES = 8, 4, 16, 48
-SPEC_NO_PACK, SPEC_AUTORESET, SPEC_RANDOMIZE = 1, 2, 4
+SPEC_NO_PACK, SPEC_AUTORESET, SPEC_RANDOMIZE, SPEC_GENERIC = 1, 2, 4, 8
 PARAM_FIELDS = ("body_mass", "body_inertia", "geom_friction", "actuator_gear", "dof_damping")
 PARAM_FAMILIES = ("body_mass", "geom_friction", "actuator_gear", "dof_damping")
 OBJ_BODY, OBJ_XBODY, OBJ_JOINT, OBJ_GEOM, OBJ_SITE, OBJ_CAMERA, OBJ_ACTUATOR, OBJ_SENSOR = 1, 2, 3, 5, 6, 7, 19, 20
@@ -76,6 +76,22 @@
 _LIB = None
 
 
+def _preload_nvrtc():
+    if os.path.exists(os.path.join(os.environ.get("CUDA_HOME", "/usr/local/cuda"), "lib64", "libnvrtc.so.12")) or \
+            os.path.exists("/usr/local/cuda/lib64/libnvrtc.so.12"):
+        return
+    import importlib.util
+    spec = importlib.util.find_spec("nvidia.cuda_nvrtc")
+    for root in (spec.submodule_search_locations or []) if spec else []:
+        path = os.path.join(root, "lib", "libnvrtc.so.12")
+        if os.path.exists(path):
+            try:
+                ctypes.CDLL(path, mode=ctypes.RTLD_GLOBAL)
+            except OSError:
+                pass
+            return
+
+
 def load(build_if_missing=True):
     global _LIB
     if _LIB is not None:
@@ -91,6 +107,7 @@
     if not os.path.exists(LIB_PATH):
         raise RuntimeError(f"{LIB_PATH} is missing: run `python -m mujoco_rl_environment_wrapper_b200.build` "
                            "(there is no CPU fallback for the step path)")
+    _preload_nvrtc()
     lib = ctypes.CDLL(LIB_PATH)
     vp, i32, i64 = ctypes.c_void_p, ctypes.c_int32, ctypes.c_int64
     lib.mjb_last_error.restype = ctypes.c_char_p
@@ -123,6 +140,8 @@
     lib.mjb_set_env_subset.argtypes = [vp, vp, ctypes.c_int32]
     lib.mjb_render.argtypes = [vp, ctypes.POINTER(ctypes.c_int32), ctypes.c_int32, ctypes.c_int32, ctypes.c_int32, vp]
     lib.mjb_batch_geometry.argtypes = [vp, ctypes.POINTER(i32), ctypes.POINTER(i32), ctypes.POINTER(i64)]
+    lib.mjb_batch_spec_info.argtypes = [vp, ctypes.POINTER(i32), ctypes.POINTER(ctypes.c_double), ctypes.c_char_p, i32]
+    lib.mjb_spec_compile.argtypes = [vp, ctypes.POINTER(EnvSpec), i32, ctypes.POINTER(ctypes.c_double), vp, ctypes.POINTER(i64)]
     lib.mjb_phase_cycles.argtypes = [ctypes.POINTER(ctypes.c_uint64), i32]
     lib.mjb_draw_u32.restype = ctypes.c_uint32
     lib.mjb_draw_u32.argtypes = [ctypes.c_uint64, ctypes.c_uint32, ctypes.c_uint32, ctypes.c_uint32]
@@ -140,6 +159,15 @@
     return lib
 
 
+def spec_compile(model, spec, num_envs):
+    lib = load()
+    ms, n = ctypes.c_double(), ctypes.c_int64(0)
+    check(lib.mjb_spec_compile(model._h, ctypes.byref(spec), int(num_envs), ctypes.byref(ms), None, ctypes.byref(n)), "spec compile")
+    buf = ctypes.create_string_buffer(n.value)
+    check(lib.mjb_spec_compile(model._h, ctypes.byref(spec), int(num_envs), ctypes.byref(ms), buf, ctypes.byref(n)), "spec compile")
+    return buf.raw[:n.value], ms.value
+
+
 def check(rc, what=""):
     if rc != 0:
         msg = load().mjb_last_error().decode(errors="replace")
diff --git a/mujoco_rl_environment_wrapper_b200/batch.py b/mujoco_rl_environment_wrapper_b200/batch.py
--- a/mujoco_rl_environment_wrapper_b200/batch.py
+++ b/mujoco_rl_environment_wrapper_b200/batch.py
@@ -166,4 +166,7 @@
     def geometry(self):
         g, w, s = ctypes.c_int32(), ctypes.c_int32(), ctypes.c_int64()
         self._lib.mjb_batch_geometry(self._h, ctypes.byref(g), ctypes.byref(w), ctypes.byref(s))
-        return {"grid": g.value, "warps_per_cta": w.value, "smem_bytes": s.value}
+        spec, ms, why = ctypes.c_int32(), ctypes.c_double(), ctypes.create_string_buffer(4096)
+        self._lib.mjb_batch_spec_info(self._h, ctypes.byref(spec), ctypes.byref(ms), why, len(why))
+        return {"grid": g.value, "warps_per_cta": w.value, "smem_bytes": s.value, "specialised": bool(spec.value),
+                "spec_reason": why.value.decode(errors="replace"), "spec_compile_ms": ms.value}
diff --git a/mujoco_rl_environment_wrapper_b200/build.py b/mujoco_rl_environment_wrapper_b200/build.py
--- a/mujoco_rl_environment_wrapper_b200/build.py
+++ b/mujoco_rl_environment_wrapper_b200/build.py
@@ -11,6 +11,32 @@
     "--use_fast_math",
     "-Xcompiler", "-fPIC", "-Xcompiler", "-Wall", "-shared",
 ]
+
+
+SPEC_SOURCES = {
+    "env_kernel.cuh": os.path.join(CSRC, "env_kernel.cuh"), "step_kernel.cuh": os.path.join(CSRC, "step_kernel.cuh"),
+    "warp_prims.cuh": os.path.join(CSRC, "warp_prims.cuh"), "tma_prims.cuh": os.path.join(CSRC, "tma_prims.cuh"),
+    "dev_model.h": os.path.join(CSRC, "dev_model.h"), "../../include/mjb.h": os.path.join(_HERE, "..", "include", "mjb.h"),
+    "mjb_blob.h": os.path.join(_HERE, "..", "include", "mjb_blob.h"),
+}
+SPEC_INC = os.path.join(CSRC, "mjb_spec_sources.inc")
+
+
+def _write_spec_sources():
+    out = ["// generated by build.py from the files named below: do not edit", "struct SpecSource { const char* name; const char* text; };",
+           "static const SpecSource kSpecSources[] = {"]
+    for name, path in SPEC_SOURCES.items():
+        with open(path) as f:
+            text = f.read()
+        pieces = [text[i:i + 12000] for i in range(0, len(text), 12000)]
+        out.append('  {"%s",' % name)
+        out.extend('   R"mjb_src(%s)mjb_src"' % p for p in pieces)
+        out.append("  },")
+    out.append("};")
+    text = "\n".join(out) + "\n"
+    if not os.path.exists(SPEC_INC) or open(SPEC_INC).read() != text:
+        with open(SPEC_INC, "w") as f:
+            f.write(text)
 
 
 def _nvcc():
@@ -39,8 +65,9 @@
 def build(force=False, verbose=False):
     if not force and not needs_build():
         return LIB_PATH
+    _write_spec_sources()
     cmd = [_nvcc()] + NVCC_FLAGS + os.environ.get("MJB_NVCC_FLAGS", "").split() + (["-Xptxas", "-v"] if verbose else []) + ["-o", LIB_PATH] + \
-          [os.path.join(CSRC, s) for s in SOURCES]
+          [os.path.join(CSRC, s) for s in SOURCES] + ["-ldl"]
     res = subprocess.run(cmd, capture_output=True, text=True)
     if verbose or res.returncode != 0:
         sys.stderr.write(res.stdout + res.stderr)
diff --git a/mujoco_rl_environment_wrapper_b200/csrc/dev_model.h b/mujoco_rl_environment_wrapper_b200/csrc/dev_model.h
--- a/mujoco_rl_environment_wrapper_b200/csrc/dev_model.h
+++ b/mujoco_rl_environment_wrapper_b200/csrc/dev_model.h
@@ -1,5 +1,7 @@
 #pragma once
+#if !defined(__CUDACC_RTC__)
 #include <stdint.h>
+#endif
 
 #ifndef MJB_HD
 #if defined(__CUDACC__)
@@ -153,10 +155,29 @@
 };
 enum { SO_MB = 0, SO_POS = 1, SO_QUAT = 4, SO_STRIDE = 8 };
 enum { KSENS_OBJ_AXIS = 64 };
-MJB_HD int prm_inertia(const DevModel& dm) { return dm.nmb; }
-MJB_HD int prm_damping(const DevModel& dm) { return 4 * dm.nmb; }
-MJB_HD int prm_gear(const DevModel& dm) { return 4 * dm.nmb + dm.nv; }
-MJB_HD int prm_friction(const DevModel& dm) { return 4 * dm.nmb + dm.nv + dm.nu; }
+template <class M> MJB_HD int prm_inertia(const M& dm) { return dm.nmb; }
+template <class M> MJB_HD int prm_damping(const M& dm) { return 4 * dm.nmb; }
+template <class M> MJB_HD int prm_gear(const M& dm) { return 4 * dm.nmb + dm.nv; }
+template <class M> MJB_HD int prm_friction(const M& dm) { return 4 * dm.nmb + dm.nv + dm.nu; }
+
+#define MJB_SHAPE_FIELDS(X)                                                                                                  \
+  X(nq) X(nv) X(nu) X(nmb) X(njnt) X(nlim) X(ngeom) X(ngdyn) X(nsite) X(nsensor) X(nsensordata) X(npair) X(nclass)         \
+  X(nlevel) X(nprobe) X(maxcon) X(maxcand) X(maxefc) X(ldj) X(maxtree) X(nblock)                                           \
+  X(pack) X(a1) X(t1) X(nq1) X(nv1) X(nu1) X(ns1) X(np1) X(ngeom1) X(maxcon1) X(njnt1)                                     \
+  X(integrator) X(has_damping) X(need_acc_sensors) X(solver_iterations) X(ls_iterations)                                   \
+  X(n_agents) X(free_joint) X(n_phys_act) X(act_dim) X(n_dynamics) X(n_rewards) X(n_dones) X(n_targets)                   \
+  X(image_words) X(env_words) X(qpos_stride) X(qvel_stride) X(ctrl_stride) X(sensor_stride) X(act_stride) X(obs_stride)    \
+  X(store_i32) X(store_f32) X(autoreset) X(n_params) X(prm_n) X(prm_soff) X(off_prm_map) X(off_prm_nominal)                \
+  X(ext_sensors) X(off_sens_obj)
+
+#if defined(MJB_SPEC)
+}
+#include "mjb_spec_shape.h"
+namespace mjb {
+typedef SpecModel DM;
+#else
+typedef DevModel DM;
+#endif
 
 enum { CAM_MB = 0, CAM_MODE = 1, CAM_POS = 2, CAM_QUAT = 5, CAM_TANHALF = 9, CAM_STRIDE = 12 };
 struct RenderHdr {
diff --git a/mujoco_rl_environment_wrapper_b200/csrc/env_kernel.cuh b/mujoco_rl_environment_wrapper_b200/csrc/env_kernel.cuh
--- a/mujoco_rl_environment_wrapper_b200/csrc/env_kernel.cuh
+++ b/mujoco_rl_environment_wrapper_b200/csrc/env_kernel.cuh
@@ -73,7 +73,7 @@
 }
 
 template <int AMAX>
-MJB_DEV bool run_plugins(const DevModel& dm, const float* ctrl, float* obs, float* rew, uint8_t* term, uint8_t* trunc, int env, int copy,
+MJB_DEV bool run_plugins(const DM& dm, const float* ctrl, float* obs, float* rew, uint8_t* term, uint8_t* trunc, int env, int copy,
                          bool is_reset, const float* probe, int* si, float* sf, const float* act, int* ts_io, const double* dtab = nullptr,
                          bool keep_flags = false) {
   const int A = dm.a1, ab = copy * dm.a1, tb = copy * dm.t1, n_targets = dm.t1;
@@ -213,7 +213,7 @@
   const int mode = (auto_pass || own_rows) ? (int)MODE_RESET : mode_in;
   Ctx c = c_in;
   float* probe = c.probe;
-  const DevModel& dm = *c.dm;
+  const DM& dm = *c.dm;
   const int lane = c.lane, K = PACKED ? dm.pack : 1, e0 = venv * K;
   c.probe_quat = (!PACKED && B.probe_quat) ? B.probe_quat + (size_t)e0 * dm.np1 * 4 : nullptr;
   uint32_t live = 0, upd = 0;
@@ -580,4 +580,54 @@
   }
 }
 
-}
+#if !defined(MJB_HOST_EMU)
+#ifndef MJB_MAX_THREADS
+#define MJB_MAX_THREADS 512
+#endif
+
+template <bool PHYS, bool PACKED, bool EXT = false, bool PRM = false>
+__global__ void __launch_bounds__(PHYS ? MJB_MAX_THREADS : 512, PHYS ? 1 : 4) k_env(const __grid_constant__ DM dm, const uint32_t* __restrict__ image, const mjb_buffers B,
+                      int num_envs, int mode, int skip_frames, const uint8_t* __restrict__ mask,
+                      const int* __restrict__ env_ids, int active, int env_base) {
+  extern __shared__ __align__(128) uint32_t smem[];
+  uint64_t* bar = reinterpret_cast<uint64_t*>(smem);
+  uint32_t* img = smem + 4;
+  const int warps = blockDim.x >> 5, warp = threadIdx.x >> 5, lane = threadIdx.x & 31;
+  if (threadIdx.x == 0) {
+    mbar_init(bar, 1);
+    mbar_fence_init();
+  }
+  __syncthreads();
+  if (threadIdx.x == 0) {
+    uint32_t bytes = (uint32_t)dm.image_words * 4u;
+    mbar_expect_tx(bar, bytes);
+    bulk_g2s(img, image, bytes, bar);
+  }
+  float* scratch = reinterpret_cast<float*>(img + dm.image_words) + (size_t)warp * (dm.env_words + 4 * ((dm.nprobe + 3) & ~3));
+  float* probe = scratch + dm.env_words;
+  Ctx c{&dm, img, scratch, lane, probe, 0};
+#if defined(MJB_PHASE_PROF)
+  long long t_last = clock64();
+  c.t_last = &t_last;
+#endif
+  const int stride = gridDim.x * warps;
+  const int pack = PACKED ? dm.pack : 1;
+  const int nvirt = (active + pack - 1) / pack;
+  const int rounds = (nvirt - blockIdx.x * warps + stride - 1) / stride;
+  int env = blockIdx.x * warps + warp;
+  for (int r = 0; r < rounds; r++) {
+    if (PHYS) {
+      int busy = nvirt - (blockIdx.x * warps + r * stride);
+      c.cta_threads = (mask == nullptr ? 32 : 0) * (busy > warps ? warps : (busy < 0 ? 0 : busy));
+    }
+    c.img_bar = r == 0 ? bar : nullptr;
+    if (env < nvirt) run_env<PHYS, PACKED, EXT, PRM>(c, B, env_ids ? env_ids[env] : env + env_base, num_envs, mode, skip_frames, mask);
+    if (r == 0) mbar_wait(bar, 0);
+    if (!PHYS) __syncthreads();
+    MJB_PH(c, PH_BARRIER);
+    env += stride;
+  }
+}
+#endif
+
+}
diff --git a/mujoco_rl_environment_wrapper_b200/csrc/mjb_batch.cu b/mujoco_rl_environment_wrapper_b200/csrc/mjb_batch.cu
--- a/mujoco_rl_environment_wrapper_b200/csrc/mjb_batch.cu
+++ b/mujoco_rl_environment_wrapper_b200/csrc/mjb_batch.cu
@@ -15,58 +15,7 @@
 #include "tma_prims.cuh"
 #include "lite_kernel.cuh"
 #include "mjb_internal.h"
-
-#ifndef MJB_MAX_THREADS
-#define MJB_MAX_THREADS 512
-#endif
-
-namespace mjb {
-
-template <bool PHYS, bool PACKED, bool EXT = false, bool PRM = false>
-__global__ void __launch_bounds__(PHYS ? MJB_MAX_THREADS : 512, PHYS ? 1 : 4) k_env(const __grid_constant__ DevModel dm, const uint32_t* __restrict__ image, const mjb_buffers B,
-                      int num_envs, int mode, int skip_frames, const uint8_t* __restrict__ mask,
-                      const int* __restrict__ env_ids, int active, int env_base) {
-  extern __shared__ __align__(128) uint32_t smem[];
-  uint64_t* bar = reinterpret_cast<uint64_t*>(smem);
-  uint32_t* img = smem + 4;
-  const int warps = blockDim.x >> 5, warp = threadIdx.x >> 5, lane = threadIdx.x & 31;
-  if (threadIdx.x == 0) {
-    mbar_init(bar, 1);
-    mbar_fence_init();
-  }
-  __syncthreads();
-  if (threadIdx.x == 0) {
-    uint32_t bytes = (uint32_t)dm.image_words * 4u;
-    mbar_expect_tx(bar, bytes);
-    bulk_g2s(img, image, bytes, bar);
-  }
-  float* scratch = reinterpret_cast<float*>(img + dm.image_words) + (size_t)warp * (dm.env_words + 4 * ((dm.nprobe + 3) & ~3));
-  float* probe = scratch + dm.env_words;
-  Ctx c{&dm, img, scratch, lane, probe, 0};
-#if defined(MJB_PHASE_PROF)
-  long long t_last = clock64();
-  c.t_last = &t_last;
-#endif
-  const int stride = gridDim.x * warps;
-  const int pack = PACKED ? dm.pack : 1;
-  const int nvirt = (active + pack - 1) / pack;
-  const int rounds = (nvirt - blockIdx.x * warps + stride - 1) / stride;
-  int env = blockIdx.x * warps + warp;
-  for (int r = 0; r < rounds; r++) {
-    if (PHYS) {
-      int busy = nvirt - (blockIdx.x * warps + r * stride);
-      c.cta_threads = (mask == nullptr ? 32 : 0) * (busy > warps ? warps : (busy < 0 ? 0 : busy));
-    }
-    c.img_bar = r == 0 ? bar : nullptr;
-    if (env < nvirt) run_env<PHYS, PACKED, EXT, PRM>(c, B, env_ids ? env_ids[env] : env + env_base, num_envs, mode, skip_frames, mask);
-    if (r == 0) mbar_wait(bar, 0);
-    if (!PHYS) __syncthreads();
-    MJB_PH(c, PH_BARRIER);
-    env += stride;
-  }
-}
-
-}
+#include "spec_jit.h"
 
 struct mjb_batch {
   mjb::PackedModel packed;
@@ -81,6 +30,9 @@
   int* d_lite_tab = nullptr;
   mjb::DevModel* d_lite_dm = nullptr;
   mjb_buffers B;
+  cudaKernel_t spec_kern = nullptr;
+  std::string spec_why;
+  double spec_ms = 0;
   int num_envs = 0, device = 0, warps = 0, grid = 0;
   size_t smem_bytes = 0;
   cudaStream_t stream = nullptr;
@@ -154,8 +106,16 @@
                     : (b->img.dm.pack > 1 ? mjb::k_env<true, true> : mjb::k_env<true, false>);
     const int pack = b->img.dm.pack;
     const int need = ((active + pack - 1) / pack + b->warps - 1) / b->warps;
-    kern<<<std::min(b->grid, std::max(1, need)), b->warps * 32, b->smem_bytes, stream>>>(
-        b->img.dm, b->d_image, B, b->num_envs, mode, skip_frames, mask, b->subset, active, base / pack);
+    const int grid = std::min(b->grid, std::max(1, need)), env_base = base / pack;
+    if (mode == mjb::MODE_STEP && b->spec_kern) {
+      const int* env_ids = b->subset;
+      void* args[] = {(void*)&b->img.dm, (void*)&b->d_image, (void*)&B, (void*)&b->num_envs, (void*)&mode, (void*)&skip_frames,
+                      (void*)&mask, (void*)&env_ids, (void*)&active, (void*)&env_base};
+      CUDA_TRY(cudaLaunchKernel((const void*)b->spec_kern, dim3(grid), dim3(b->warps * 32), args, b->smem_bytes, stream));
+    } else {
+      kern<<<grid, b->warps * 32, b->smem_bytes, stream>>>(b->img.dm, b->d_image, B, b->num_envs, mode, skip_frames, mask, b->subset,
+                                                           active, env_base);
+    }
   }
   CUDA_TRY(cudaGetLastError());
   if (b->timing) {
@@ -282,6 +242,13 @@
     return fail(MJB_ERR_CUDA);
   }
   smem_attr[device] = std::max(smem_attr[device], b->smem_bytes);
+  if (spec->flags & MJB_SPEC_GENERIC) b->spec_why = "MJB_SPEC_GENERIC";
+  else if (spec->skip_frames == 0) b->spec_why = "skip_frames = 0 (the physics-free step)";
+  else {
+    mjb::SpecKernel* sk = mjb::spec_compile(dm);
+    b->spec_kern = mjb::spec_kernel(sk, device, b->smem_bytes, b->spec_why);
+    b->spec_ms = sk->compile_ms;
+  }
   if (spec->skip_frames == 0) {
     try {
       mjb::ModelView mv(m->host.blob.data());
@@ -554,6 +521,35 @@
 #endif
 }
 
+int mjb_batch_spec_info(const mjb_batch* b, int32_t* specialised, double* compile_ms, char* reason, int32_t reason_len) {
+  if (!b) return MJB_ERR_ARG;
+  if (specialised) *specialised = b->spec_kern ? 1 : 0;
+  if (compile_ms) *compile_ms = b->spec_ms;
+  if (reason && reason_len > 0) snprintf(reason, (size_t)reason_len, "%s", b->spec_why.c_str());
+  return MJB_OK;
+}
+
+int mjb_spec_compile(const mjb_model* m, const mjb_env_spec* spec, int32_t num_envs, double* compile_ms, void* cubin, int64_t* cubin_bytes) {
+  if (!m || !spec || num_envs < 1 || !cubin_bytes) { mjb::set_error("mjb_spec_compile: bad argument"); return MJB_ERR_ARG; }
+  mjb::DevImage img;
+  try {
+    mjb::PackedModel packed;
+    const int K = mjb::choose_pack(m->host, *spec, num_envs);
+    mjb::make_packed(m->host, *spec, K, packed);
+    mjb::ModelView mv(K > 1 ? packed.rep.blob.data() : m->host.blob.data());
+    mjb::build_dev_model(mv, packed.vspec, img, false, K);
+  } catch (const std::exception& e) {
+    mjb::set_error(e.what());
+    return MJB_ERR_LIMIT;
+  }
+  const mjb::SpecKernel* sk = mjb::spec_compile(img.dm);
+  if (!sk->why.empty()) { mjb::set_error("mjb_spec_compile: " + sk->why); return MJB_ERR_CUDA; }
+  if (compile_ms) *compile_ms = sk->compile_ms;
+  if (cubin && *cubin_bytes >= (int64_t)sk->cubin.size()) memcpy(cubin, sk->cubin.data(), sk->cubin.size());
+  *cubin_bytes = (int64_t)sk->cubin.size();
+  return MJB_OK;
+}
+
 int mjb_batch_geometry(const mjb_batch* b, int32_t* grid, int32_t* warps_per_cta, int64_t* smem_bytes) {
   if (!b) return MJB_ERR_ARG;
   if (grid) *grid = b->grid;
diff --git a/mujoco_rl_environment_wrapper_b200/csrc/spec_jit.h b/mujoco_rl_environment_wrapper_b200/csrc/spec_jit.h
--- /dev/null
+++ b/mujoco_rl_environment_wrapper_b200/csrc/spec_jit.h
@@ -0,0 +1,168 @@
+#pragma once
+#include <cuda.h>
+#include <cuda_runtime.h>
+#include <dlfcn.h>
+#include <nvrtc.h>
+
+#include <chrono>
+#include <cstdlib>
+#include <map>
+#include <memory>
+#include <mutex>
+#include <string>
+#include <vector>
+
+#include "dev_model.h"
+#include "mjb_spec_sources.inc"
+
+namespace mjb {
+
+inline std::string spec_shape_header(const DevModel& dm) {
+  std::string h = "// generated: the shape of one batch's model (mjb_batch_create)\n#pragma once\nnamespace mjb {\n";
+  h += "__device__ constexpr int spec_off[IF_COUNT] = {";
+  for (int i = 0; i < IF_COUNT; i++) h += std::to_string(dm.off[i]) + (i + 1 < IF_COUNT ? ", " : "};\n");
+  h += "__device__ constexpr int spec_soff[SF_COUNT] = {";
+  for (int i = 0; i < SF_COUNT; i++) h += std::to_string(dm.soff[i]) + (i + 1 < SF_COUNT ? ", " : "};\n");
+  h += "struct SpecModel : DevModel {\n";
+#define X(f) h += "  static constexpr int " #f " = " + std::to_string(dm.f) + ";\n";
+  MJB_SHAPE_FIELDS(X)
+#undef X
+  h += "};\n}  // namespace mjb\n";
+  return h;
+}
+
+inline std::string spec_kernel_name(const DevModel& dm) {
+  const char* packed = dm.pack > 1 ? "true" : "false";
+  if (dm.prm_n > 0) return std::string("mjb::k_env<true, ") + packed + ", true, true>";
+  return std::string("mjb::k_env<true, ") + packed + (dm.autoreset ? ", true, false>" : ", false, false>");
+}
+
+struct Nvrtc {
+  decltype(&nvrtcVersion) version;
+  decltype(&nvrtcCreateProgram) create;
+  decltype(&nvrtcAddNameExpression) add_name;
+  decltype(&nvrtcCompileProgram) compile;
+  decltype(&nvrtcGetProgramLogSize) log_size;
+  decltype(&nvrtcGetProgramLog) log;
+  decltype(&nvrtcGetCUBINSize) cubin_size;
+  decltype(&nvrtcGetCUBIN) cubin;
+  decltype(&nvrtcGetLoweredName) lowered;
+  decltype(&nvrtcDestroyProgram) destroy;
+  decltype(&nvrtcGetErrorString) error;
+};
+
+inline const Nvrtc* nvrtc_api(std::string& why) {
+  static std::once_flag once;
+  static Nvrtc api;
+  static bool ok = false;
+  static std::string err;
+  std::call_once(once, [] {
+    void* h = nullptr;
+    std::vector<std::string> cands;
+    if (const char* home = getenv("CUDA_HOME")) cands.push_back(std::string(home) + "/lib64/libnvrtc.so.12");
+    cands.push_back("/usr/local/cuda/lib64/libnvrtc.so.12");
+    cands.push_back("libnvrtc.so.12");
+    for (const std::string& c : cands)
+      if ((h = dlopen(c.c_str(), RTLD_NOW | RTLD_LOCAL))) break;
+    if (!h) { err = "libnvrtc.so.12 not found"; return; }
+#define SYM(field, name)                                                       \
+  if (!(api.field = (decltype(api.field))dlsym(h, #name))) {                   \
+    err = "libnvrtc.so.12 lacks " #name;                                        \
+    return;                                                                     \
+  }
+    SYM(version, nvrtcVersion) SYM(create, nvrtcCreateProgram) SYM(add_name, nvrtcAddNameExpression)
+    SYM(compile, nvrtcCompileProgram) SYM(log_size, nvrtcGetProgramLogSize) SYM(log, nvrtcGetProgramLog)
+    SYM(cubin_size, nvrtcGetCUBINSize) SYM(cubin, nvrtcGetCUBIN) SYM(lowered, nvrtcGetLoweredName)
+    SYM(destroy, nvrtcDestroyProgram) SYM(error, nvrtcGetErrorString)
+#undef SYM
+    int major = 0, minor = 0;
+    api.version(&major, &minor);
+    if (major != __CUDACC_VER_MAJOR__ || minor != __CUDACC_VER_MINOR__) {
+      err = "NVRTC " + std::to_string(major) + "." + std::to_string(minor) + " differs from the nvcc that built libmjb (" +
+            std::to_string(__CUDACC_VER_MAJOR__) + "." + std::to_string(__CUDACC_VER_MINOR__) + ")";
+      return;
+    }
+    ok = true;
+  });
+  why = err;
+  return ok ? &api : nullptr;
+}
+
+struct SpecKernel {
+  std::string why;
+  double compile_ms = 0;
+  std::vector<char> cubin;
+  std::string lowered;
+  cudaLibrary_t lib = nullptr;
+  cudaKernel_t kern = nullptr;
+  std::map<int, size_t> smem_attr;
+};
+
+inline SpecKernel* spec_compile(const DevModel& dm) {
+  static std::mutex mu;
+  static std::map<std::string, std::unique_ptr<SpecKernel>> cache;
+  const std::string shape = spec_shape_header(dm), name = spec_kernel_name(dm);
+  std::lock_guard<std::mutex> lock(mu);
+  std::unique_ptr<SpecKernel>& slot = cache[name + "\n" + shape];
+  if (slot) return slot.get();
+  slot.reset(new SpecKernel());
+  SpecKernel& sk = *slot;
+  const Nvrtc* api = nvrtc_api(sk.why);
+  if (!api) return &sk;
+  const auto t0 = std::chrono::steady_clock::now();
+  std::vector<const char*> hdr_text, hdr_name;
+  for (const auto& s : kSpecSources) { hdr_name.push_back(s.name); hdr_text.push_back(s.text); }
+  hdr_name.push_back("mjb_spec_shape.h");
+  hdr_text.push_back(shape.c_str());
+  nvrtcProgram prog = nullptr;
+  nvrtcResult rc = api->create(&prog, "#include \"env_kernel.cuh\"\n", "mjb_spec.cu", (int)hdr_text.size(), hdr_text.data(), hdr_name.data());
+  if (rc != NVRTC_SUCCESS) { sk.why = std::string("nvrtcCreateProgram: ") + api->error(rc); return &sk; }
+  api->add_name(prog, name.c_str());
+  const char* opts[] = {"--gpu-architecture=sm_100a", "-std=c++17", "--use_fast_math", "-lineinfo", "-DMJB_SPEC=1", "-default-device"};
+  rc = api->compile(prog, (int)(sizeof(opts) / sizeof(opts[0])), opts);
+  if (rc != NVRTC_SUCCESS) {
+    size_t n = 0;
+    api->log_size(prog, &n);
+    std::string log(n, '\0');
+    if (n) api->log(prog, &log[0]);
+    sk.why = std::string("NVRTC compile failed: ") + api->error(rc) + "\n" + log;
+    api->destroy(&prog);
+    return &sk;
+  }
+  size_t n = 0;
+  api->cubin_size(prog, &n);
+  sk.cubin.resize(n);
+  api->cubin(prog, sk.cubin.data());
+  const char* lowered = nullptr;
+  api->lowered(prog, name.c_str(), &lowered);
+  sk.lowered = lowered ? lowered : "";
+  api->destroy(&prog);
+  sk.compile_ms = std::chrono::duration<double, std::milli>(std::chrono::steady_clock::now() - t0).count();
+  if (sk.lowered.empty()) sk.why = "nvrtcGetLoweredName failed";
+  return &sk;
+}
+
+inline cudaKernel_t spec_kernel(SpecKernel* sk, int device, size_t smem, std::string& why) {
+  static std::mutex mu;
+  std::lock_guard<std::mutex> lock(mu);
+  if (!sk->why.empty()) { why = sk->why; return nullptr; }
+  cudaError_t e = cudaSuccess;
+  if (!sk->lib) {
+    if ((e = cudaLibraryLoadData(&sk->lib, sk->cubin.data(), nullptr, nullptr, 0, nullptr, nullptr, 0)) != cudaSuccess ||
+        (e = cudaLibraryGetKernel(&sk->kern, sk->lib, sk->lowered.c_str())) != cudaSuccess) {
+      sk->why = std::string("loading the specialised kernel: ") + cudaGetErrorString(e);
+      why = sk->why;
+      return nullptr;
+    }
+  }
+  if (smem > sk->smem_attr[device]) {
+    if ((e = cudaFuncSetAttribute((const void*)sk->kern, cudaFuncAttributeMaxDynamicSharedMemorySize, (int)smem)) != cudaSuccess) {
+      why = std::string("cudaFuncSetAttribute(specialised kernel): ") + cudaGetErrorString(e);
+      return nullptr;
+    }
+    sk->smem_attr[device] = smem;
+  }
+  return sk->kern;
+}
+
+}
diff --git a/mujoco_rl_environment_wrapper_b200/csrc/step_kernel.cuh b/mujoco_rl_environment_wrapper_b200/csrc/step_kernel.cuh
--- a/mujoco_rl_environment_wrapper_b200/csrc/step_kernel.cuh
+++ b/mujoco_rl_environment_wrapper_b200/csrc/step_kernel.cuh
@@ -63,7 +63,7 @@
 }
 
 struct Ctx {
-  const DevModel* dm;
+  const DM* dm;
   const uint32_t* img;
   float* s;
   int lane;
@@ -89,11 +89,18 @@
 #define MJB_PH(c, id) ((void)0)
 #define MJB_COUNT(c, slot, n) ((void)0)
 #endif
-#define CI(f) ((const int*)(c.img + c.dm->off[IF_##f]))
-#define CU(f) ((const uint32_t*)(c.img + c.dm->off[IF_##f]))
-#define CF(f) ((const float*)(c.img + c.dm->off[IF_##f]))
-#define SF(f) (c.s + c.dm->soff[SF_##f])
-#define SI(f) ((int*)(c.s + c.dm->soff[SF_##f]))
+#if defined(MJB_SPEC)
+#define MJB_OFF(f) spec_off[IF_##f]
+#define MJB_SOFF(f) spec_soff[SF_##f]
+#else
+#define MJB_OFF(f) c.dm->off[IF_##f]
+#define MJB_SOFF(f) c.dm->soff[SF_##f]
+#endif
+#define CI(f) ((const int*)(c.img + MJB_OFF(f)))
+#define CU(f) ((const uint32_t*)(c.img + MJB_OFF(f)))
+#define CF(f) ((const float*)(c.img + MJB_OFF(f)))
+#define SF(f) (c.s + MJB_SOFF(f))
+#define SI(f) ((int*)(c.s + MJB_SOFF(f)))
 #define PF(f, blk) (PRM ? c.s + c.dm->prm_soff + (blk) : CF(f))
 
 MJB_DEV int tri(int i, int j) { return ((i * (i + 1)) >> 1) + j; }
@@ -106,7 +113,7 @@
 }
 
 MJB_DEV void fk(const Ctx& c) {
-  const DevModel& dm = *c.dm;
+  const DM& dm = *c.dm;
   const int* level_adr = CI(level_adr);
   float* qpos = SF(qpos);
   float *xpos = SF(xpos), *xquat = SF(xquat), *xmat = SF(xmat), *xipos = SF(xipos), *cdof = SF(cdof);
@@ -213,7 +220,7 @@
 }
 
 MJB_DEV void crb_mass(const Ctx& c) {
-  const DevModel& dm = *c.dm;
+  const DM& dm = *c.dm;
   const int* level_adr = CI(level_adr);
   float *cinert = SF(cinert), *crb = SF(crb), *M = SF(M), *cdof = SF(cdof);
   MJB_NOUNROLL
@@ -257,7 +264,7 @@
 }
 
 MJB_DEV void rne_pass(const Ctx& c, bool with_acc) {
-  const DevModel& dm = *c.dm;
+  const DM& dm = *c.dm;
   const int* level_adr = CI(level_adr);
   float *cdof = SF(cdof), *cvel = SF(cvel), *cacc = SF(cacc), *qvel = SF(qvel), *qacc = SF(qacc);
   float *cinert = SF(cinert), *cfrc = SF(crb);
@@ -333,7 +340,7 @@
 
 template <bool PRM = false>
 MJB_DEV void kin_forward(const Ctx& c) {
-  const DevModel& dm = *c.dm;
+  const DM& dm = *c.dm;
   const int* level_adr = CI(level_adr);
   float *qpos = SF(qpos), *qvel = SF(qvel);
   float *xpos = SF(xpos), *xquat = SF(xquat), *xmat = SF(xmat), *xipos = SF(xipos), *cdof = SF(cdof);
@@ -486,7 +493,7 @@
 
 template <bool PRM = false>
 MJB_DEV void dyn_backward(const Ctx& c) {
-  const DevModel& dm = *c.dm;
+  const DM& dm = *c.dm;
   const int* level_adr = CI(level_adr);
   float *crb = SF(cinert), *cfrc = SF(crb), *M = SF(M), *cdof = SF(cdof), *qvel = SF(qvel);
   MJB_NOUNROLL
@@ -796,7 +803,7 @@
 
 template <bool PRM = false>
 MJB_DEV int collide(const Ctx& c, int* tot) {
-  const DevModel& dm = *c.dm;
+  const DM& dm = *c.dm;
   const uint32_t* pairs = CU(pair_pack);
   int* cand = SI(cand);
   int ncand = 0;
@@ -1004,7 +1011,7 @@
 
 template <bool PRM = false>
 MJB_DEV void make_constraints(const Ctx& c, int ncon) {
-  const DevModel& dm = *c.dm;
+  const DM& dm = *c.dm;
   float *efcD = SF(efcD), *efcAref = SF(efcAref), *qpos = SF(qpos), *qvel = SF(qvel);
   MJB_NOUNROLL
   for (int k = c.lane; k < dm.nlim; k += 32) {
@@ -1291,7 +1298,7 @@
 }
 
 MJB_DEV void rows_mul(const Ctx& c, int ncon, const float* x, float* out, const float* sub) {
-  const DevModel& dm = *c.dm;
+  const DM& dm = *c.dm;
   MJB_NOUNROLL
   for (int k = c.lane; k < dm.nlim; k += 32) {
     float v = x[CI(lim_dof)[k]];
@@ -1327,7 +1334,7 @@
 }
 
 MJB_DEV float jt_mul(const Ctx& c, int ncon, int base, int mylim, const float* w) {
-  const DevModel& dm = *c.dm;
+  const DM& dm = *c.dm;
   const float* J = SF(J);
   const float* con = SF(con);
   float out = mylim >= 0 ? w[2 * mylim] - w[2 * mylim + 1] : 0.f;
@@ -1344,7 +1351,7 @@
   return out;
 }
 MJB_DEV void jt_mul2(const Ctx& c, int ncon, int base, int mylim, const float* w, const float* v, float& ow, float& ov) {
-  const DevModel& dm = *c.dm;
+  const DM& dm = *c.dm;
   const float* J = SF(J);
   const float* con = SF(con);
   ow = mylim >= 0 ? w[2 * mylim] - w[2 * mylim + 1] : 0.f;
@@ -1364,7 +1371,7 @@
 }
 
 MJB_DEV int newton(const Ctx& c, int ncon) {
-  const DevModel& dm = *c.dm;
+  const DM& dm = *c.dm;
   const int nv = dm.nv, lane = c.lane;
   const int t0 = CI(dof_t0)[lane], t1 = CI(dof_t1)[lane];
   float *M = SF(M), *H = SF(H), *a = SF(qacc), *sv = SF(vecC);
@@ -1574,7 +1581,7 @@
 }
 
 MJB_DEV void sensors_pos(const Ctx& c) {
-  const DevModel& dm = *c.dm;
+  const DM& dm = *c.dm;
   float* sens = SF(sens);
   MJB_NOUNROLL
   for (int i = 0; i < dm.nsensor; i++) {
@@ -1606,7 +1613,7 @@
 }
 
 MJB_DEV void sensors_acc(const Ctx& c, int ncon) {
-  const DevModel& dm = *c.dm;
+  const DM& dm = *c.dm;
   if (!dm.need_acc_sensors) return;
   float* sens = SF(sens);
   bool did_rne = false;
@@ -1656,7 +1663,7 @@
 }
 
 MJB_DEV void sensors_frame(const Ctx& c) {
-  const DevModel& dm = *c.dm;
+  const DM& dm = *c.dm;
   float* sens = SF(sens);
   const float *xpos = SF(xpos), *xquat = SF(xquat), *xmat = SF(xmat), *cvel = SF(cvel);
   MJB_NOUNROLL
@@ -1705,7 +1712,7 @@
   MJB_PH(c, PH_INTEGRATE);
   kin_forward<PRM>(c);
   if (probes) {
-    const DevModel& dm = *c.dm;
+    const DM& dm = *c.dm;
     MJB_NOUNROLL
     for (int p = c.lane; p < dm.nprobe; p += 32) {
       int kind = CI(probe_kind)[p], id = CI(probe_id)[p];
@@ -1750,7 +1757,7 @@
 }
 
 MJB_DEV void integrate_pos(const Ctx& c, float* qpos, const float* v, float h) {
-  const DevModel& dm = *c.dm;
+  const DM& dm = *c.dm;
   MJB_NOUNROLL
   for (int j = c.lane; j < dm.njnt; j += 32) {
     int qa = CI(jnt_qposadr)[j], da = CI(jnt_dofadr)[j];
@@ -1770,7 +1777,7 @@
 
 template <bool PRM = false>
 MJB_DEV int substep(const Ctx& c, bool sensors, bool integrate, int* iters_out, int* dropped) {
-  const DevModel& dm = *c.dm;
+  const DM& dm = *c.dm;
   const int nv = dm.nv, lane = c.lane;
   float *qpos = SF(qpos), *qvel = SF(qvel), *qacc = SF(qacc);
   const float h = dm.timestep;
diff --git a/mujoco_rl_environment_wrapper_b200/csrc/tma_prims.cuh b/mujoco_rl_environment_wrapper_b200/csrc/tma_prims.cuh
--- a/mujoco_rl_environment_wrapper_b200/csrc/tma_prims.cuh
+++ b/mujoco_rl_environment_wrapper_b200/csrc/tma_prims.cuh
@@ -1,5 +1,7 @@
 #pragma once
+#if !defined(__CUDACC_RTC__)
 #include <stdint.h>
+#endif
 
 namespace mjb {
 
diff --git a/mujoco_rl_environment_wrapper_b200/csrc/warp_prims.cuh b/mujoco_rl_environment_wrapper_b200/csrc/warp_prims.cuh
--- a/mujoco_rl_environment_wrapper_b200/csrc/warp_prims.cuh
+++ b/mujoco_rl_environment_wrapper_b200/csrc/warp_prims.cuh
@@ -1,7 +1,9 @@
 #pragma once
+#if !defined(__CUDACC_RTC__)
 #include <math.h>
 #include <stdint.h>
 #include <string.h>
+#endif
 
 #if defined(MJB_HOST_EMU)
 #include "../../tests/emu/simt_emu.h"
```
